# pairlab/SlotFormer

Measured on AMD Instinct MI355X. Metric: rollout frames/sec at B=32, 128x128, 7 slots, 6+50 steps (SAVi-encode + SlotFormer rollout), higher is better.
Workload: dtype f32 storage; matmul/conv on split-bf16 MFMA (bf16x3: hi*hi+hi*lo+lo*hi, f32 accumulate)

## Files before the change

include/slotformer_hip.h:

```cpp
#ifndef SLOTFORMER_HIP_H
#define SLOTFORMER_HIP_H
#include <stddef.h>

#ifdef __cplusplus
extern "C" {
#endif

int sf_version(void);
const char* sf_last_error_string(void);

int sf_get_precision(void);
int sf_set_precision(int mode);

int sf_profile_enable(int class_mask);
int sf_set_seam_fused(int on);
int sf_get_seam_fused(void);
int sf_set_ffn_rows64(int on);
int sf_get_ffn_rows64(void);
int sf_profile_sample(int every);
int sf_profile_read(int kernel_class, double* total_ms, long long* launches, double* work);


int sf_linear_f32(const float* A, int lda, const float* W, const float* bias, const float* ln_gamma,
                  const float* ln_beta, float ln_eps, const float* residual, int ldr, float* C, int ldc,
// ... 137 lines not shown
int sf_slot_update_packed_f32(const float* part_num, const float* part_den, int P, const float* slots_prev,
                              const void* gru_ih_packed, const void* gru_hh_packed, const float* gru_b_ih,
                              const float* gru_b_hh, const float* ln_g, const float* ln_b, const void* mlp_w1_packed,
                              const float* mlp_b1, const void* mlp_w2_packed, const float* mlp_b2, float* slots_out,
                              const float* q_ln_g, const float* q_ln_b, const void* q_w_packed, float* q_out, int B, int N,
                              int D, int H, float ln_eps, void* stream);
int sf_slot_update_packed_next_f32(const float* part_num, const float* part_den, int P, const float* slots_prev,
                                   const void* gru_ih_packed, const void* gru_hh_packed, const float* gru_b_ih,
                                   const float* gru_b_hh, const float* ln_g, const float* ln_b, const void* mlp_w1_packed,
                                   const float* mlp_b1, const void* mlp_w2_packed, const float* mlp_b2, float* slots_out,
                                   const float* q_ln_g, const float* q_ln_b, const void* q_w_packed, float* q_out, int B, int N,
                                   int D, int H, float ln_eps, float* out2, long long out2_bs, int p_step, const float* pm_ln_g,
                                   const float* pm_ln_b, const void* pm_w0_packed, const float* pm_b0, const void* pm_w2_packed,
                                   const float* pm_b2, int norm_first, const void* kd_w_packed, const float* kd_b, const float* noise,
                                   long long noise_bs, float* kdist_out, long long kdist_bs, float* next_slots, void* stream);

int sf_mha_f32(const float* qkv, float* out, int B, int L, int Lq, int d_model, int num_heads, void* stream);

int sf_qkv_attention_f32(const float* x, const float* ln_gamma, const float* ln_beta, float ln_eps,
                         const float* in_proj_w, const float* in_proj_b, float* out, int B, int L, int Lq, int d_model,
                         int num_heads, void* stream);

int sf_lstm_pointwise_f32(const float* gates, const float* c_prev, float* h_out, float* c_out, int R, int H,
                          void* stream);

int sf_sample_dist_f32(const float* dist, const float* noise, float* out, int R, int D, void* stream);

int sf_bilinear_resize_f32(const float* in, float* out, long long R, int Hi, int Wi, int Ho, int Wo,
                           void* stream);

size_t sf_groupnorm1_workspace_bytes(int F);
int sf_groupnorm1_nhwc_f32(const float* x, const float* gamma, const float* beta, float* y, int F, int H, int W, int C,
                           float eps, int relu, int pixel_shuffle, void* ws, size_t ws_bytes, void* stream);
size_t sf_groupnorm1_bwd_workspace_bytes(int F, int H, int W, int C);
int sf_groupnorm1_nhwc_bwd_f32(const float* x, const float* gamma, const float* beta, const float* dy, float* dx, float* dgamma,
                               float* dbeta, int F, int H, int W, int C, float eps, int relu, int pixel_shuffle, void* ws,
                               size_t ws_bytes, void* stream);

int sf_slate_attention_f32(const float* q, const float* k, const float* v, float* out, int ldq, int ldk, int ldv, int ldo,
                           int B, int Lq, int Lk, int num_heads, int head_dim, int causal, void* stream);
size_t sf_slate_attention_bwd_workspace_bytes(int B, int Lq, int num_heads);
int sf_slate_attention_train_fwd_f32(const float* q, const float* k, const float* v, float* out, float* lse, int ldq, int ldk,
                                     int ldv, int ldo, long long q_bs, long long k_bs, long long v_bs, long long o_bs, int B,
                                     int Lq, int Lk, int num_heads, int head_dim, int causal, float dropout_p,
                                     unsigned long long seed, void* stream);
int sf_slate_attention_train_bwd_f32(const float* q, const float* k, const float* v, const float* out, const float* d_out,
                                     const float* lse, float* dq, float* dk, float* dv, int ldq, int ldk, int ldv, int ldo,
                                     long long q_bs, long long k_bs, long long v_bs, long long o_bs, int B, int Lq, int Lk,
                                     int num_heads, int head_dim, int causal, float dropout_p, unsigned long long seed, void* ws,
                                     size_t ws_bytes, void* stream);
int sf_slate_attention_bwd_f32(const float* q, const float* k, const float* v, const float* out, const float* d_out, float* dq,
                               float* dk, float* dv, int ldq, int ldk, int ldv, int ldo, long long q_bs, long long k_bs,
                               long long v_bs, long long o_bs, int B, int Lq, int Lk, int num_heads, int head_dim, int causal,
                               void* ws, size_t ws_bytes, void* stream);
int sf_slate_attention_strided_f32(const float* q, const float* k, const float* v, float* out, int ldq, int ldk, int ldv,
                                   int ldo, long long q_bs, long long k_bs, long long v_bs, long long o_bs, int B, int Lq,
                                   int Lk, int num_heads, int head_dim, int causal, void* stream);
int sf_embed_tokens_f32(const long long* idx, const float* tok_emb, const float* pos, float* out, int B, int L, int d,
                        void* stream);
int sf_argmax_rows_f32(const float* x, long long ld, long long* out, long long R, int V, void* stream);
int sf_cross_entropy_f32(const float* x, const long long* target, float* loss_rows, float* mean_out, long long R, int V,
                         void* stream);
int sf_softmax_rows_f32(const float* x, const float* add, float scale, float* y, long long R, int V, void* stream);
int sf_cross_entropy_bwd_f32(const float* x, const long long* target, const float* g, float* dx, long long R, int V, void* stream);
int sf_log_softmax_rows_f32(const float* x, float* y, long long R, int V, void* stream);
int sf_gumbel_softmax_rows_f32(const float* x, unsigned long long seed, float scale, float* y, long long R, int V, void* stream);
int sf_softmax_rows_bwd_f32(const float* y, const float* dy, float scale, float* dx, long long R, int V, void* stream);

typedef struct {
  const float *ln1_g, *ln1_b, *wqkv, *wo;
  const float *ln2_g, *ln2_b, *wq_c, *wkv_c, *wo_c;
  const float *ln3_g, *ln3_b, *w1, *b1, *w2, *b2;
  int is_first;
} sf_slate_block;

typedef struct {
  int d_model, num_heads, num_layers, vocab_size, num_slots, max_len;
  const float *in_proj_w, *in_proj_b, *tok_emb , *pos_emb , *lnf_g, *lnf_b, *head_w ;
  const sf_slate_block* blocks;
} sf_slate_decoder;

size_t sf_slate_generate_workspace_bytes(const sf_slate_decoder* m, int B, int steps);
int sf_slate_generate_f32(const sf_slate_decoder* m, const float* slots, int B, int steps, long long* tokens_out,
                          float* logits_out, void* ws, size_t ws_bytes, void* stream);

int sf_slate_step_ok(const sf_slate_decoder* m);
size_t sf_slate_generate_tok_workspace_bytes(const sf_slate_decoder* m, int B, int steps);
int sf_slate_generate_tok_f32(const sf_slate_decoder* m, const float* slots, int B, int steps, long long* tokens_out,
                              float* logits_out, int frames_per_wg, void* ws, size_t ws_bytes, void* stream,
                              int* frames_per_wg_ran);
int sf_gather_rows_f32(const float* table, const long long* ids, float* out, long long R, int d, long long table_rows,
                       void* stream);

int sf_dvae_tokens_ok(int V, int K, int C, int H, int W);
size_t sf_dvae_head_packed_bytes(int V, int K);
int sf_dvae_pack_head_weights(const float* w, void* packed, int V, int K, void* stream);
int sf_dvae_pack_head_weights_host(const float* w, void* packed, int V, int K);
int sf_dvae_patch_embed_f32(const float* img, const float* w, float* y, int F, int C, int H, int W, void* stream);
int sf_dvae_head_argmax_f32(const float* x, long long ld, const void* w_packed, const float* bias, long long* ids_i64, short* ids_i16, long long R,
                            int V, int K, void* stream);

int sf_head_ce_ok(int V, int K);
size_t sf_head_ce_packed_bytes(int V, int K);
size_t sf_head_ce_workspace_bytes(long long R);
int sf_head_ce_pack_weights(const float* w, void* packed, int V, int K, void* stream);
int sf_head_ce_pack_weights_host(const float* w, void* packed, int V, int K);
int sf_head_ce_fwd_f32(const float* x, long long ld, const void* w_packed, const long long* target_i64, const short* target_i16,
                       const float* group_w, int group, float* lse, float* loss_rows, double* stats, long long R, int V, int K, void* ws,
                       size_t ws_bytes, void* stream);
int sf_head_ce_bwd_f32(const float* x, long long ld, const void* w_packed, const long long* target_i64, const short* target_i16,
                       const float* group_w, int group, const float* lse, const float* g, float* dx, long long ldx, long long R, int V, int K,
                       void* stream);

int sf_physion_readout_ok(int N, int C, int F);
int sf_physion_readout_fwd_f32(const float* slots, long long stride_v, long long stride_t, int V, const int* video_index, const float* W1,
                               const float* b1, const float* w2, const float* b2, float* logits, int* t_star, float* step_logits,
                               unsigned char* pair_star, int K, int B, int T, int N, int C, int F, int agg, void* stream);
size_t sf_physion_readout_bwd_workspace_bytes(int B, int N, int F);
int sf_physion_readout_bwd_f32(const float* slots, long long stride_v, long long stride_t, int V, const int* video_index, const float* W1,
                               const float* b1, const float* w2, const float* g, const int* t_star, const unsigned char* pair_star, float* dW1,
                               float* db1, float* dw2, float* db2, int B, int T, int N, int C, int F, int agg, void* workspace,
                               size_t workspace_bytes, void* stream);
int sf_physion_readout_score_f32(const float* logits, const float* labels, const int* task_idx, const float* thresholds, int n_thresh, int n_tasks,
                                 float* loss, float* g, int* counts, int* task_counts, int K, int B, void* stream);


typedef struct {
  const float *norm1_g, *norm1_b, *in_proj_w, *in_proj_b, *out_proj_w, *out_proj_b;
  const float *norm2_g, *norm2_b, *lin1_w, *lin1_b, *lin2_w, *lin2_b;
  const void *lin1_packed, *lin2_packed;
  const void *attn_in_packed, *attn_out_packed;
  const void* tok_packed;
} sf_tfm_layer;

size_t sf_attn_packed_bytes(int d_model, int which);
int sf_pack_attn_weights(const float* in_proj_w, const float* out_proj_w, void* in_packed, void* out_packed, int d_model,
                         int num_heads, void* stream);

size_t sf_ffn_packed_bytes(int d_model, int ffn);
int sf_pack_ffn_weights(const float* lin1_w, const float* lin2_w, void* lin1_packed, void* lin2_packed, int d_model,
                        int ffn, void* stream);

int sf_ffn_chunk_partials_f32(const sf_tfm_layer* w, const float* ap, long long ap_stride, float* xp, long long xp_stride, int M,
                              int ffn, int rows_per_wg, void* stream);

int sf_attn_block_f32(const sf_tfm_layer* w, const float* x, float* out, int B, int L, int Lq, int heads_per_wg, void* stream);
int sf_ffn_block_rows_f32(const sf_tfm_layer* w, const float* x2, float* y, int M, int ffn, void* stream);
size_t sf_layer_tok_packed_bytes(void);
size_t sf_layer_tok_packed_bytes_ex(int d_model, int num_heads, int ffn);
int sf_pack_layer_tok_weights(const sf_tfm_layer* w, void* packed, int d_model, int num_heads, int ffn, void* stream);
int sf_layer_tok_block_f32(const sf_tfm_layer* w, int nl, const float* x, float* y, int B, int L, void* stream);
int sf_layer_tok_block_ex_f32(const sf_tfm_layer* w, int nl, int d_model, int num_heads, int ffn, const float* x, float* y, int B, int L, void* stream);
int sf_debug_read_ts_layer_tok(long long* out16);
size_t sf_attn_rows_planes_bytes(int B);
int sf_attn_block_rows_f32(const sf_tfm_layer* w, const float* x, float* out, void* planes, int B, int L, int Lq, void* stream);

int sf_phyre_readout_ok(int num_slots, int slot_size, int T, int d_model, int num_heads, int ffn, int num_layers);
size_t sf_phyre_readout_workspace_bytes(int B, int num_slots, int T);
int sf_phyre_readout_fwd_f32(const float* slots, long long stride_v, long long stride_t, int V, int T_all, const int* video_index, const int* sel,
                             const float* in_proj_w, const float* in_proj_b, const float* enc_t_pe, const float* cls, const sf_tfm_layer* layers,
                             int num_layers, int d_model, int num_heads, int ffn, const float* mlp_w1, const float* mlp_b1, const float* mlp_w2,
                             const float* mlp_b2, float* logits, float* conf, const int* scatter_index, float* scatter_table, long long scatter_len,
                             int B, int T, int N, int C, void* workspace, size_t workspace_bytes, void* stream);
int sf_phyre_auccess_f32(const float* conf, const int* status, int* first_rank, int tasks, int actions, void* stream);

typedef struct {
  int num_slots, slot_size, T, text_len;
  int question_len;
  int d_model, num_heads, ffn_dim, num_layers;
  int vocab, emb_dim;
  const float* cls;
  const float* pos;
  const float *vision_w, *vision_b;
  const float* q_in_proj_w;
  const float* text_table;
  const sf_tfm_layer* layers;
} sf_aloe;
int sf_aloe_ok(int num_slots, int slot_size, int T, int text_len, int d_model, int num_heads, int ffn, int num_layers);
size_t sf_aloe_workspace_bytes(int B, int num_slots, int T, int text_len, int d_model, int ffn);
int sf_aloe_text_table_f32(const float* q_embedding, const float* q_in_proj_w, const float* q_in_proj_b, float* table, int vocab, int emb_dim, int d_model,
                           void* stream);
int sf_aloe_fwd_f32(const sf_aloe* m, const float* slots, long long stride_v, long long stride_t, int V, int T_all, const int* video_index, const int* start,
                    int frame_offset, const int* tokens, const unsigned char* pad_mask, int multiple_choice, const float* head_w1, const float* head_b1,
                    const float* head_w2, const float* head_b2, int mlp_hidden, int num_outputs, float* logits, int* answers, int B, void* workspace,
                    size_t workspace_bytes, void* stream);
int sf_aloe_score_f32(const float* cls_logits, const int* cls_labels, int B1, int num_answers, const float* mc_logits, const float* mc_labels,
                      const int* mc_flag, int Bn, const int* mc_subtype, int Q, float* losses, int* ques_correct, int* counts, void* stream);

typedef struct {
  int num_slots, slot_size, d_model, num_layers, num_heads, ffn_dim, norm_first;
  int window_len;
  int single_step;
  const float *in_proj_w, *in_proj_b, *out_proj_w, *out_proj_b;
  const float* pe_tok;
  const sf_tfm_layer* layers;
  const void *in_proj_packed, *out_proj_packed;
} sf_rollouter;

size_t sf_packed_linear_bytes(int N, int K);
int sf_pack_linear_weights(const float* w, void* packed, int N, int K, void* stream);

size_t sf_rollout_workspace_bytes(const sf_rollouter* m, int B);
int sf_rollout_f32(const sf_rollouter* m, float* slots, int B, int T_total, int pred_len, void* ws,
                   size_t ws_bytes, void* stream);

typedef struct {
  int precision;
  int seam_fused;
  int ffn_rows;
  int attn_heads_per_wg;
  int attn_qkv_rows;
  int ffn_tile;
  int cus_available;
  int layer_tok;
} sf_rollout_opts;
int sf_set_layer_tok(int on);
int sf_get_layer_tok(void);
int sf_rollout_opts_f32(const sf_rollouter* m, float* slots, int B, int T_total, int pred_len, void* ws, size_t ws_bytes,
                        void* stream, const sf_rollout_opts* opts);
size_t sf_rollout_phases_workspace_bytes(const sf_rollouter* m, int B, int frame_offset);
int sf_rollout_phases_f32(const sf_rollouter* m, float* slots, int B, int T_total, int obs, int frame_offset, int pred_len, void* ws,
                          size_t ws_bytes, void* stream, const sf_rollout_opts* opts);
int sf_rollout_is_fused(const sf_rollouter* m);
int sf_rollout_tok_ok(const sf_rollouter* m);
int sf_rollout_tok_layers(const sf_rollouter* m, int B, const sf_rollout_opts* opts);
int sf_rollout_uses_seam(const sf_rollouter* m, int B);
int sf_rollout_uses_seam_opts(const sf_rollouter* m, int B, const sf_rollout_opts* opts);

size_t sf_linear_bwd_workspace_bytes(long long M, int N, int K);
int sf_linear_bwd_f32(const float* x, const float* W, const float* y, float* dy, float* dx, float* dW, float* db, long long M,
                      int N, int K, int relu, void* ws, size_t ws_bytes, void* stream);
int sf_mha_train_fwd_f32(const float* qkv, float* ctx, int B, int L, int d_model, int num_heads, float dropout_p,
                         unsigned long long seed, void* stream);
int sf_mha_train_bwd_f32(const float* qkv, const float* d_ctx, float* d_qkv, int B, int L, int d_model, int num_heads,
                         float dropout_p, unsigned long long seed, void* stream);
int sf_dropout_f32(const float* x, const float* res, float* y, long long n, float dropout_p, unsigned long long seed,
                   void* stream);
int sf_adam_flat_f32(float* param, const float* grad, float* exp_avg, float* exp_avg_sq, long long n, int step, float lr,
                     float beta1, float beta2, float eps, void* stream);
size_t sf_grad_norm_workspace_bytes(long long n);
int sf_grad_clip_coef_f32(const float* grad, long long n, float max_norm, float* out3, void* ws, size_t ws_bytes,
                          void* stream);
#define SF_ADAM_MAX_GROUPS 8
typedef struct {
  long long begin;
  float lr;
} sf_adam_group;
int sf_adam_flat_groups_f32(float* param, const float* grad, float* exp_avg, float* exp_avg_sq, long long n, int step,
                            const sf_adam_group* groups, int num_groups, float beta1, float beta2, float eps,
                            const float* grad_scale, void* stream);
size_t sf_layernorm_bwd_workspace_bytes(int D);
int sf_layernorm_bwd_f32(const float* x, const float* dy, const float* gamma, float* dx, float* dgamma, float* dbeta,
                         long long rows, int D, float eps, void* ws, size_t ws_bytes, void* stream);

typedef struct {
  int resolution, layers, channels, ks, hidden, out_channels;
  const float* conv_w[8];
  const float* conv_b[8];
  const float *pos_grid, *pos_w, *pos_b;
  const float *ln_g, *ln_b, *fc1_w, *fc1_b, *fc2_w, *fc2_b;
} sf_savi_features;

typedef struct {
  float* conv_w[8];
  float* conv_b[8];
  float *pos_w, *pos_b, *ln_g, *ln_b, *fc1_w, *fc1_b, *fc2_w, *fc2_b;
} sf_savi_features_grads;

size_t sf_savi_features_train_workspace_bytes(const sf_savi_features* m, int F);
int sf_savi_features_train_fwd_f32(const sf_savi_features* m, const float* img, long long frame_stride, int F, float* out,
                                   void* ws, size_t ws_bytes, void* stream);
int sf_savi_features_train_bwd_f32(const sf_savi_features* m, const float* img, long long frame_stride, const float* d_out,
                                   const sf_savi_features_grads* g, int F, void* ws, size_t ws_bytes, void* stream);

typedef struct {
  int in_features, slot_size, mlp_hidden, num_slots;
  const float *norm_in_g, *norm_in_b, *wk, *wv;
  const float *q_ln_g, *q_ln_b, *wq;
  const float *gru_w_ih, *gru_w_hh, *gru_b_ih, *gru_b_hh;
  const float *mlp_ln_g, *mlp_ln_b, *mlp_w1, *mlp_b1, *mlp_w2, *mlp_b2;
  float eps;
} sf_slot_attention;

typedef struct {
  float *norm_in_g, *norm_in_b, *wk, *wv, *q_ln_g, *q_ln_b, *wq, *gru_w_ih, *gru_w_hh, *gru_b_ih, *gru_b_hh;
  float *mlp_ln_g, *mlp_ln_b, *mlp_w1, *mlp_b1, *mlp_w2, *mlp_b2;
} sf_slot_attention_grads;

size_t sf_slot_attention_train_workspace_bytes(const sf_slot_attention* m, int B, int HW, int iters);
int sf_slot_attention_train_fwd_f32(const sf_slot_attention* m, const float* inputs, const float* slots_in, int B, int HW,
                                    int iters, float* slots_out, void* ws, size_t ws_bytes, void* stream);
int sf_slot_attention_train_bwd_f32(const sf_slot_attention* m, const float* inputs, const float* d_slots_out, float* d_inputs,
                                    float* d_slots_in, const sf_slot_attention_grads* g, int B, int HW, int iters, void* ws,
                                    size_t ws_bytes, void* stream);

typedef struct {
  float *norm1_g, *norm1_b, *in_proj_w, *in_proj_b, *out_proj_w, *out_proj_b;
  float *norm2_g, *norm2_b, *lin1_w, *lin1_b, *lin2_w, *lin2_b;
} sf_tfm_layer_grads;

typedef struct {
  float *in_proj_w, *in_proj_b, *out_proj_w, *out_proj_b;
  const sf_tfm_layer_grads* layers;
  float* pe_tok;
} sf_rollouter_grads;

size_t sf_rollout_train_workspace_bytes(const sf_rollouter* m, int B, int pred_len);
int sf_rollout_train_fwd_f32(const sf_rollouter* m, const float* x, float* pred, int B, int pred_len, float dropout_p,
                             unsigned long long seed, void* ws, size_t ws_bytes, void* stream);
int sf_rollout_train_bwd_f32(const sf_rollouter* m, const float* d_pred, float* d_x, const sf_rollouter_grads* g, int B,
                             int pred_len, float dropout_p, unsigned long long seed, void* ws, size_t ws_bytes,
                             void* stream);

typedef struct {
  int num_slots, slot_size, d_model, num_heads, ffn_dim, num_layers;
  const float *in_proj_w, *in_proj_b;
  const float *enc_t_pe, *cls;
  const sf_tfm_layer* layers;
  const float *mlp_w1, *mlp_b1, *mlp_w2, *mlp_b2;
} sf_phyre_readout_model;

typedef struct {
  float *in_proj_w, *in_proj_b;
  float *enc_t_pe, *cls;
  const sf_tfm_layer_grads* layers;
  float *mlp_w1, *mlp_b1, *mlp_w2, *mlp_b2;
} sf_phyre_readout_grads;

size_t sf_phyre_readout_train_workspace_bytes(const sf_phyre_readout_model* m, int B, int T);
int sf_phyre_readout_train_fwd_f32(const sf_phyre_readout_model* m, const float* slots, long long stride_v, long long stride_t, int V, int T_all,
                                   const int* video_index, const int* sel, int B, int T, float dropout_p, unsigned long long seed, float* logits,
                                   unsigned char* gates, unsigned char* head_gates, void* ws, size_t ws_bytes, void* stream);
int sf_phyre_readout_train_bwd_f32(const sf_phyre_readout_model* m, const float* slots, long long stride_v, long long stride_t, int V, int T_all,
                                   const int* video_index, const int* sel, int B, int T, const float* g, const sf_phyre_readout_grads* grads,
                                   float dropout_p, unsigned long long seed, void* ws, size_t ws_bytes, void* stream);

int sf_rollout_train_clips_fwd_f32(const sf_rollouter* m, const float* table, int T_total, const int* clip_video, const int* clip_start,
                                   int frame_offset, float* pred, int B, int pred_len, float dropout_p, unsigned long long seed, void* ws,
                                   size_t ws_bytes, void* stream);
size_t sf_clip_mse_workspace_bytes(int B, int S, long long E);
int sf_clip_mse_f32(const float* pred, const float* target, const int* clip_video, const int* clip_start, int T_total, int first_frame,
                    int frame_step, const float* step_w, const int* clip_len, int hist, float scale, float* d_pred, double* stats, int B, int S,
                    long long E, void* ws, size_t ws_bytes, void* stream);
int sf_clip_frames_f32(const unsigned char* table, int T_total, const int* clip_video, const int* clip_start, int first_frame, int frame_step,
                       const float* mean3, const float* std3, float* out, int B, int S, int H, int W, void* stream);

typedef struct {
  int resolution;
  int enc_layers;
// ... 149 lines not shown
```

slotformer_amd/_lib.py:

```python
import ctypes as C
import os

_HERE = os.path.dirname(os.path.abspath(__file__))
LIB_PATH = os.environ.get('SF_LIB_PATH') or os.path.join(_HERE, 'libslotformer_hip.so')

FP = C.c_void_p


class sf_tfm_layer(C.Structure):
    _fields_ = [(n, FP) for n in (
        'norm1_g', 'norm1_b', 'in_proj_w', 'in_proj_b', 'out_proj_w', 'out_proj_b',
        'norm2_g', 'norm2_b', 'lin1_w', 'lin1_b', 'lin2_w', 'lin2_b', 'lin1_packed', 'lin2_packed', 'attn_in_packed', 'attn_out_packed', 'tok_packed')]


class sf_rollouter(C.Structure):
    _fields_ = [(n, C.c_int) for n in (
        'num_slots', 'slot_size', 'd_model', 'num_layers', 'num_heads', 'ffn_dim', 'norm_first',
        'window_len', 'single_step')] + [(n, FP) for n in (
            'in_proj_w', 'in_proj_b', 'out_proj_w', 'out_proj_b', 'pe_tok')] + [
                ('layers', C.POINTER(sf_tfm_layer)), ('in_proj_packed', C.c_void_p), ('out_proj_packed', C.c_void_p)]


class sf_aloe(C.Structure):
    _fields_ = [(n, C.c_int) for n in ('num_slots', 'slot_size', 'T', 'text_len', 'question_len', 'd_model', 'num_heads', 'ffn_dim', 'num_layers',
                                       'vocab', 'emb_dim')] + [(n, FP) for n in ('cls', 'pos', 'vision_w', 'vision_b', 'q_in_proj_w', 'text_table')] + [
                                           ('layers', C.POINTER(sf_tfm_layer))]


class sf_rollout_opts(C.Structure):
    _fields_ = [(n, C.c_int) for n in ('precision', 'seam_fused', 'ffn_rows', 'attn_heads_per_wg', 'attn_qkv_rows', 'ffn_tile', 'cus_available', 'layer_tok')]


class sf_tfm_layer_grads(C.Structure):
    _fields_ = [(n, FP) for n in (
        'norm1_g', 'norm1_b', 'in_proj_w', 'in_proj_b', 'out_proj_w', 'out_proj_b',
        'norm2_g', 'norm2_b', 'lin1_w', 'lin1_b', 'lin2_w', 'lin2_b')]


class sf_phyre_readout_model(C.Structure):
    _fields_ = [(n, C.c_int) for n in ('num_slots', 'slot_size', 'd_model', 'num_heads', 'ffn_dim', 'num_layers')] + [
        (n, FP) for n in ('in_proj_w', 'in_proj_b', 'enc_t_pe', 'cls')] + [('layers', C.POINTER(sf_tfm_layer))] + [
            (n, FP) for n in ('mlp_w1', 'mlp_b1', 'mlp_w2', 'mlp_b2')]


class sf_phyre_readout_grads(C.Structure):
    _fields_ = [(n, FP) for n in ('in_proj_w', 'in_proj_b', 'enc_t_pe', 'cls')] + [('layers', C.POINTER(sf_tfm_layer_grads))] + [
        (n, FP) for n in ('mlp_w1', 'mlp_b1', 'mlp_w2', 'mlp_b2')]


class sf_rollouter_grads(C.Structure):
    _fields_ = [(n, FP) for n in ('in_proj_w', 'in_proj_b', 'out_proj_w', 'out_proj_b')] + [
        ('layers', C.POINTER(sf_tfm_layer_grads)), ('pe_tok', FP)]


_SA_LEAVES = ('norm_in_g', 'norm_in_b', 'wk', 'wv', 'q_ln_g', 'q_ln_b', 'wq', 'gru_w_ih', 'gru_w_hh', 'gru_b_ih', 'gru_b_hh',
              'mlp_ln_g', 'mlp_ln_b', 'mlp_w1', 'mlp_b1', 'mlp_w2', 'mlp_b2')


class sf_slot_attention(C.Structure):
    _fields_ = [(n, C.c_int) for n in ('in_features', 'slot_size', 'mlp_hidden', 'num_slots')] + [
        (n, FP) for n in _SA_LEAVES] + [('eps', C.c_float)]


class sf_slot_attention_grads(C.Structure):
    _fields_ = [(n, FP) for n in _SA_LEAVES]


class sf_adam_group(C.Structure):
    _fields_ = [('begin', C.c_longlong), ('lr', C.c_float)]


class sf_savi_decoder_grads(C.Structure):
    _fields_ = [('deconv_w', FP * 8), ('deconv_b', FP * 8)] + [(n, FP) for n in ('out_w', 'out_b', 'pos_w', 'pos_b')]


class sf_savi_features(C.Structure):
    _fields_ = [(n, C.c_int) for n in ('resolution', 'layers', 'channels', 'ks', 'hidden', 'out_channels')] + [
        ('conv_w', FP * 8), ('conv_b', FP * 8)] + [(n, FP) for n in ('pos_grid', 'pos_w', 'pos_b', 'ln_g', 'ln_b', 'fc1_w', 'fc1_b',
                                                                      'fc2_w', 'fc2_b')]


class sf_savi_features_grads(C.Structure):
    _fields_ = [('conv_w', FP * 8), ('conv_b', FP * 8)] + [(n, FP) for n in ('pos_w', 'pos_b', 'ln_g', 'ln_b', 'fc1_w', 'fc1_b',
                                                                              'fc2_w', 'fc2_b')]


class sf_savi_encoder(C.Structure):
    _fields_ = (
        [('resolution', C.c_int), ('enc_layers', C.c_int), ('enc_channels', C.c_int * 9),
         ('enc_ks', C.c_int)] +
        [(n, C.c_int) for n in ('enc_out_channels', 'num_slots', 'slot_size', 'slot_mlp_size',
                                'num_iterations')] +
        [('conv_w', FP * 8), ('conv_b', FP * 8), ('pos_table', FP)] +
        [(n, FP) for n in ('enc_ln_g', 'enc_ln_b', 'enc_fc1_w', 'enc_fc1_b', 'enc_fc2_w', 'enc_fc2_b',
                           'sa_norm_in_g', 'sa_norm_in_b', 'sa_q_ln_g', 'sa_q_ln_b', 'sa_q_w', 'sa_kv_w',
                           'gru_w_ih', 'gru_w_hh', 'gru_b_ih', 'gru_b_hh',
                           'mlp_ln_g', 'mlp_ln_b', 'mlp_w1', 'mlp_b1', 'mlp_w2', 'mlp_b2',
                           'init_latents')] +
        [('kd_mode', C.c_int)] +
        [(n, FP) for n in ('kd_w0', 'kd_b0', 'kd_ln_g', 'kd_ln_b', 'kd_w3', 'kd_b3')] +
        [(n, C.c_int) for n in ('pred_type', 'pred_rnn', 'pred_norm_first', 'pred_num_layers',
                                'pred_num_heads', 'pred_ffn_dim', 'pred_hidden')] +
        [(n, FP) for n in ('pm_ln_g', 'pm_ln_b', 'pm_w0', 'pm_b0', 'pm_w2', 'pm_b2')] +
        [('pred_layers', C.POINTER(sf_tfm_layer))] +
        [(n, FP) for n in ('lstm_w_ih', 'lstm_w_hh', 'lstm_b_ih', 'lstm_b_hh', 'proj_w', 'proj_b')] +
        [('sa_eps', C.c_float), ('sa_q_w_t', FP), ('pm_w0_t', FP), ('pm_w2_t', FP), ('kd_w0_t', FP),
         ('sa_gru_ih_p', C.c_void_p), ('sa_gru_hh_p', C.c_void_p), ('sa_mlp_w1_p', C.c_void_p), ('sa_mlp_w2_p', C.c_void_p),
         ('sa_q_w_p', C.c_void_p), ('sa_fold_q_w', FP), ('sa_fold_q_w_t', FP), ('sa_fold_gru_ih_t', FP), ('sa_fold_q_w_p', C.c_void_p),
         ('sa_fold_gru_ih_p', C.c_void_p), ('pred_packed', C.POINTER(C.c_void_p)), ('enc_fc1_p', C.c_void_p), ('enc_fc2_p', C.c_void_p),
         ('conv_w_frag', C.c_void_p * 8), ('pm_w0_p', C.c_void_p), ('pm_w2_p', C.c_void_p), ('kd_w0_p', C.c_void_p)])


class sf_slate_block(C.Structure):
    _fields_ = [(n, FP) for n in ('ln1_g', 'ln1_b', 'wqkv', 'wo', 'ln2_g', 'ln2_b', 'wq_c', 'wkv_c', 'wo_c', 'ln3_g', 'ln3_b',
                                  'w1', 'b1', 'w2', 'b2')] + [('is_first', C.c_int)]


class sf_slate_decoder(C.Structure):
    _fields_ = [(n, C.c_int) for n in ('d_model', 'num_heads', 'num_layers', 'vocab_size', 'num_slots', 'max_len')] + [
        (n, FP) for n in ('in_proj_w', 'in_proj_b', 'tok_emb', 'pos_emb', 'lnf_g', 'lnf_b', 'head_w')] + [
            ('blocks', C.POINTER(sf_slate_block))]


class sf_savi_decoder(C.Structure):
    _fields_ = ([('resolution', C.c_int), ('dec_layers', C.c_int), ('dec_channels', C.c_int * 9),
                 ('dec_strides', C.c_int * 8), ('dec_ks', C.c_int), ('dec_res', C.c_int), ('num_slots', C.c_int),
                 ('slot_size', C.c_int), ('deconv_w', FP * 8), ('deconv_b', FP * 8), ('out_w', FP), ('out_b', FP),
                 ('pos_table', FP), ('deconv_w_flipped', FP * 8), ('deconv_w_frag', C.c_void_p * 8), ('l0_weff', FP), ('l0_posterm', FP)])


class sf_egress_tile(C.Structure):
    _fields_ = [('kind', C.c_int), ('N', C.c_int), ('a', C.c_void_p), ('b', C.c_void_p), ('scale', C.c_float), ('ids_i64', C.c_int), ('P', C.c_int),
                ('history_len', C.c_int)]


class sf_lpips_model(C.Structure):
    _fields_ = [('conv_w', C.c_void_p * 13), ('conv_b', FP * 13), ('lin_w', FP * 5), ('shift', FP), ('scale', FP)]


I, LL, F32, SZ, VP = C.c_int, C.c_longlong, C.c_float, C.c_size_t, C.c_void_p

SIGNATURES = {
    'sf_version': (I, []),
    'sf_last_error_string': (C.c_char_p, []),
    'sf_get_precision': (I, []),
    'sf_set_precision': (I, [I]),
    'sf_profile_enable': (I, [I]),
    'sf_profile_sample': (I, [I]),
    'sf_set_seam_fused': (I, [I]),
    'sf_get_seam_fused': (I, []),
    'sf_set_ffn_rows64': (I, [I]),
    'sf_get_ffn_rows64': (I, []),
    'sf_profile_read': (I, [I, C.POINTER(C.c_double), C.POINTER(C.c_longlong), C.POINTER(C.c_double)]),
    'sf_linear_f32': (I, [FP, I, FP, FP, FP, FP, F32, FP, I, FP, I, I, I, I, I, VP]),
    'sf_layernorm_f32': (I, [FP, FP, FP, FP, I, I, F32, VP]),
    'sf_conv2d_nchw_in_f32': (I, [FP, LL, FP, FP, FP, FP, I, I, I, I, I, I, I, I, VP]),
    'sf_conv2d_nchw_in_grouped_f32': (I, [FP, LL, I, LL, FP, FP, FP, FP, I, I, I, I, I, I, I, I, VP]),
    'sf_conv2d_nhwc_f32': (I, [FP, FP, FP, FP, FP, I, I, I, I, I, I, I, VP]),
    'sf_pack_conv_weight_f32': (I, [FP, FP, I, I, I, VP]),
    'sf_pixel_feat_f32': (I, [FP] * 10 + [I, F32, I, VP]),
    'sf_conv_frag_bytes': (SZ, [I, I, I]),
    'sf_set_conv_fp16x2': (I, [I]),
    'sf_get_conv_fp16x2': (I, []),
    'sf_pack_conv_frag_weights': (I, [FP, VP, I, I, I, VP]),
    'sf_conv5x5_frag_f32': (I, [FP, VP, FP, FP, FP, I, I, I, I, VP]),
    'sf_conv5x5_ws_f32': (I, [FP, VP, FP, FP, FP, I, I, I, I, I, VP]),
    'sf_deconv_frag_bytes': (SZ, [I, I, I, I]),
    'sf_pack_deconv_frag_weights': (I, [FP, VP, I, I, I, I, VP]),
    'sf_deconv5x5s2_frag_f32': (I, [FP, VP, FP, FP, I, I, I, I, VP]),
    'sf_deconv5x5s2_head_frag_f32': (I, [FP, VP, FP, FP, FP, FP, I, I, I, VP]),
    'sf_decode_l0_expand_f32': (I, [FP, FP, FP, I, I, I, VP]),
    'sf_conv_transpose2d_nhwc_f32': (I, [FP, FP, FP, FP, I, I, I, I, I, I, I, I, VP]),
    'sf_pack_deconv_weight_f32': (I, [FP, FP, I, I, I, VP]),
    'sf_slot_broadcast_f32': (I, [FP, FP, FP, I, I, I, VP]),
    'sf_decode_combine_f32': (I, [FP, FP, FP, FP, I, I, I, VP]),
    'sf_savi_decode_workspace_bytes': (SZ, [C.POINTER(sf_savi_decoder), I]),
    'sf_savi_decode_f32': (I, [C.POINTER(sf_savi_decoder), FP, FP, FP, FP, I, VP, SZ, VP]),
    'sf_savi_decode_seg_f32': (I, [C.POINTER(sf_savi_decoder), FP, FP, FP, FP, VP, VP, F32, I, VP, SZ, VP]),
    'sf_decode_combine_seg_f32': (I, [FP, FP, FP, FP, VP, VP, F32, VP, I, I, I, VP]),
    'sf_postproc_mask_f32': (I, [FP, VP, VP, F32, VP, I, I, I, VP]),
    'sf_vp_metrics_workspace_bytes': (SZ, [I, I, I]),
    'sf_vp_image_metrics_f32': (I, [FP, FP, VP, VP, VP, I, I, I, I, VP, SZ, VP]),
    'sf_vp_mask_metrics': (I, [VP, VP, I, VP, FP, VP, VP, VP, VP, I, I, I, I, VP, SZ, VP]),
    'sf_vp_bbox_pr_f32': (I, [FP, VP, FP, VP, VP, I, I, I, F32, VP]),
    'sf_masks_to_boxes': (I, [VP, I, FP, VP, I, I, I, I, VP]),
    'sf_vp_mean_over_videos_f64': (I, [VP, VP, I, I, I, VP]),
    'sf_lpips_pack_conv_weights': (I, [FP, VP, I, I, VP]),
    'sf_lpips_pack_conv_weights_host': (I, [VP, VP, I, I]),
    'sf_lpips_workspace_bytes': (SZ, [I, I, I]),
    'sf_lpips_f32': (I, [C.POINTER(sf_lpips_model), FP, FP, FP, I, I, I, I, I, VP, SZ, VP]),
    'sf_lpips_mean_over_videos_f32': (I, [FP, VP, VP, I, I, VP]),
    'sf_ingest_tables_bytes': (SZ, [I, I, I, I, I]),
    'sf_ingest_tables_host': (I, [VP, SZ, I, I, I, I, I]),
    'sf_ingest_frames_u8': (I, [VP, VP, I, VP, FP, FP, FP, I, I, I, I, I, I, I, VP]),
    'sf_resize_masks_nearest': (I, [VP, I, VP, VP, VP, I, I, I, I, I, VP]),
    'sf_rle_label_maps': (I, [VP, VP, VP, VP, VP, VP, VP, I, I, I, I, I, I, I, VP]),
    'sf_rle_boxes_pad': (I, [VP, FP, VP, VP, I, I, VP]),
    'sf_egress_frames_u8': (I, [FP, VP, LL, I, I, I, I, I, VP]),
    'sf_egress_grid_shape': (I, [I, I, I, I, I, I, C.POINTER(I), C.POINTER(I)]),
    'sf_egress_grid': (I, [C.POINTER(sf_egress_tile), I, VP, I, I, I, I, I, I, F32, I, VP]),
    'sf_egress_draw_boxes': (I, [VP, FP, VP, VP, I, I, I, I, I, I, VP]),
    'sf_pos_embed_table_f32': (I, [FP, FP, FP, FP, I, I, VP]),
    'sf_slot_attn_num_partials': (I, [I]),
    'sf_slot_attn_iter_f32': (I, [FP, FP, I, LL, FP, FP, FP, FP, I, I, I, I, F32, F32, VP]),
    'sf_slot_update_f32': (I, [FP, FP, I, FP] + [FP] * 10 + [FP, I, I, I, I, F32, VP]),
    'sf_slot_update_packed_f32': (I, [FP, FP, I, FP, VP, VP, FP, FP, FP, FP, VP, FP, VP, FP, FP, FP, FP, VP, FP, I, I, I, I, F32, VP]),
    'sf_slot_attn_iter_planes_f32': (I, [VP, LL, FP, FP, FP, FP, LL, I, I, I, F32, F32, VP]),
    'sf_slot_prologue_f32': (I, [FP] * 8 + [I, FP, FP, FP, LL, FP, LL, FP, FP, FP, FP, FP, I, I, I, F32, VP]),
    'sf_slot_update_packed_next_f32': (I, [FP, FP, I, FP, VP, VP, FP, FP, FP, FP, VP, FP, VP, FP, FP, FP, FP, VP, FP, I, I, I, I, F32,
                                           FP, LL, I, FP, FP, VP, FP, VP, FP, I, VP, FP, FP, LL, FP, LL, FP, VP]),
    'sf_mha_f32': (I, [FP, FP, I, I, I, I, I, VP]),
    'sf_qkv_attention_f32': (I, [FP, FP, FP, F32, FP, FP, FP, I, I, I, I, I, VP]),
    'sf_lstm_pointwise_f32': (I, [FP, FP, FP, FP, I, I, VP]),
    'sf_sample_dist_f32': (I, [FP, FP, FP, I, I, VP]),
    'sf_bilinear_resize_f32': (I, [FP, FP, LL, I, I, I, I, VP]),
    'sf_rollout_workspace_bytes': (SZ, [C.POINTER(sf_rollouter), I]),
    'sf_rollout_f32': (I, [C.POINTER(sf_rollouter), FP, I, I, I, VP, SZ, VP]),
    'sf_rollout_opts_f32': (I, [C.POINTER(sf_rollouter), FP, I, I, I, VP, SZ, VP, C.POINTER(sf_rollout_opts)]),
    'sf_rollout_phases_workspace_bytes': (SZ, [C.POINTER(sf_rollouter), I, I]),
    'sf_rollout_phases_f32': (I, [C.POINTER(sf_rollouter), FP, I, I, I, I, I, VP, SZ, VP, C.POINTER(sf_rollout_opts)]),
    'sf_rollout_uses_seam': (I, [C.POINTER(sf_rollouter), I]),
    'sf_rollout_uses_seam_opts': (I, [C.POINTER(sf_rollouter), I, C.POINTER(sf_rollout_opts)]),
    'sf_rollout_is_fused': (I, [C.POINTER(sf_rollouter)]),
    'sf_rollout_tok_ok': (I, [C.POINTER(sf_rollouter)]),
    'sf_rollout_tok_layers': (I, [C.POINTER(sf_rollouter), I, C.POINTER(sf_rollout_opts)]),
    'sf_ffn_chunk_partials_f32': (I, [C.POINTER(sf_tfm_layer), FP, LL, FP, LL, I, I, I, VP]),
    'sf_attn_block_f32': (I, [C.POINTER(sf_tfm_layer), FP, FP, I, I, I, I, VP]),
    'sf_ffn_block_rows_f32': (I, [C.POINTER(sf_tfm_layer), FP, FP, I, I, VP]),
    'sf_set_layer_tok': (I, [I]),
    'sf_get_layer_tok': (I, []),
    'sf_layer_tok_packed_bytes': (SZ, []),
    'sf_layer_tok_packed_bytes_ex': (SZ, [I, I, I]),
    'sf_pack_layer_tok_weights': (I, [C.POINTER(sf_tfm_layer), VP, I, I, I, VP]),
    'sf_layer_tok_block_f32': (I, [C.POINTER(sf_tfm_layer), I, FP, FP, I, I, VP]),
    'sf_layer_tok_block_ex_f32': (I, [C.POINTER(sf_tfm_layer), I, I, I, I, FP, FP, I, I, VP]),
    'sf_debug_read_ts_layer_tok': (I, [C.POINTER(C.c_longlong)]),
    'sf_attn_rows_planes_bytes': (SZ, [I]),
    'sf_attn_block_rows_f32': (I, [C.POINTER(sf_tfm_layer), FP, FP, VP, I, I, I, VP]),
    'sf_slot_attn_iter_bwd_workspace_bytes': (SZ, [I, I, I, I]),
    'sf_slot_attn_iter_bwd_f32': (I, [FP, FP, I, LL, FP, FP, FP, I, FP, FP, FP, I, FP, I, I, I, I, F32, F32, VP, SZ, VP]),
    'sf_slot_attn_iter_bwd16_workspace_bytes': (SZ, [I, I, I, I]),
    'sf_slot_attn_iter_bwd16_f32': (I, [FP, FP, I, LL, FP, FP, FP, I, FP, FP, FP, I, FP, I, I, I, I, F32, F32, VP, SZ, VP]),
    'sf_set_slot_attn_tile16': (I, [I]),
    'sf_get_slot_attn_tile16': (I, []),
    'sf_slot_attention_train_workspace_bytes': (SZ, [C.POINTER(sf_slot_attention), I, I, I]),
    'sf_slot_attention_train_fwd_f32': (I, [C.POINTER(sf_slot_attention), FP, FP, I, I, I, FP, VP, SZ, VP]),
    'sf_slot_attention_train_bwd_f32': (I, [C.POINTER(sf_slot_attention), FP, FP, FP, FP, C.POINTER(sf_slot_attention_grads), I, I, I,
                                            VP, SZ, VP]),
    'sf_savi_decode_train_workspace_bytes': (SZ, [C.POINTER(sf_savi_decoder), I]),
    'sf_savi_decode_train_fwd_f32': (I, [C.POINTER(sf_savi_decoder), FP, FP, FP, FP, I, VP, SZ, VP]),
    'sf_savi_decode_train_bwd_f32': (I, [C.POINTER(sf_savi_decoder), C.POINTER(C.c_void_p), FP, FP, FP, C.POINTER(sf_savi_decoder_grads),
                                         I, VP, SZ, VP]),
    'sf_savi_features_train_workspace_bytes': (SZ, [C.POINTER(sf_savi_features), I]),
    'sf_savi_features_train_fwd_f32': (I, [C.POINTER(sf_savi_features), FP, LL, I, FP, VP, SZ, VP]),
    'sf_savi_features_train_bwd_f32': (I, [C.POINTER(sf_savi_features), FP, LL, FP, C.POINTER(sf_savi_features_grads), I, VP, SZ, VP]),
    'sf_linear_bwd_workspace_bytes': (SZ, [LL, I, I]),
    'sf_linear_bwd_f32': (I, [FP, FP, FP, FP, FP, FP, FP, LL, I, I, I, VP, SZ, VP]),
    'sf_mha_train_fwd_f32': (I, [FP, FP, I, I, I, I, F32, C.c_ulonglong, VP]),
    'sf_mha_train_bwd_f32': (I, [FP, FP, FP, I, I, I, I, F32, C.c_ulonglong, VP]),
    'sf_dropout_f32': (I, [FP, FP, FP, LL, F32, C.c_ulonglong, VP]),
    'sf_adam_flat_f32': (I, [FP, FP, FP, FP, LL, I, F32, F32, F32, F32, VP]),
    'sf_grad_norm_workspace_bytes': (SZ, [LL]),
    'sf_grad_clip_coef_f32': (I, [FP, LL, F32, FP, VP, SZ, VP]),
    'sf_adam_flat_groups_f32': (I, [FP, FP, FP, FP, LL, I, C.POINTER(sf_adam_group), I, F32, F32, F32, FP, VP]),
    'sf_layernorm_bwd_workspace_bytes': (SZ, [I]),
    'sf_layernorm_bwd_f32': (I, [FP, FP, FP, FP, FP, FP, LL, I, F32, VP, SZ, VP]),
    'sf_rollout_train_workspace_bytes': (SZ, [C.POINTER(sf_rollouter), I, I]),
    'sf_rollout_train_fwd_f32': (I, [C.POINTER(sf_rollouter), FP, FP, I, I, F32, C.c_ulonglong, VP, SZ, VP]),
    'sf_rollout_train_bwd_f32': (I, [C.POINTER(sf_rollouter), FP, FP, C.POINTER(sf_rollouter_grads), I, I, F32,
                                     C.c_ulonglong, VP, SZ, VP]),
    'sf_rollout_train_clips_fwd_f32': (I, [C.POINTER(sf_rollouter), FP, I, VP, VP, I, FP, I, I, F32, C.c_ulonglong, VP, SZ, VP]),
    'sf_clip_mse_workspace_bytes': (SZ, [I, I, LL]),
    'sf_clip_mse_f32': (I, [FP, FP, VP, VP, I, I, I, FP, VP, I, F32, FP, VP, I, I, LL, VP, SZ, VP]),
    'sf_clip_frames_f32': (I, [VP, I, VP, VP, I, I, FP, FP, FP, I, I, I, I, VP]),
    'sf_savi_encode_workspace_bytes': (SZ, [C.POINTER(sf_savi_encoder), I]),
    'sf_savi_encode_f32': (I, [C.POINTER(sf_savi_encoder), FP, FP, FP, FP, FP, I, FP, FP, FP, I, I, VP, SZ,
                               VP]),
    'sf_groupnorm1_workspace_bytes': (SZ, [I]),
    'sf_groupnorm1_nhwc_f32': (I, [FP, FP, FP, FP, I, I, I, I, F32, I, I, VP, SZ, VP]),
    'sf_groupnorm1_bwd_workspace_bytes': (SZ, [I, I, I, I]),
    'sf_groupnorm1_nhwc_bwd_f32': (I, [FP, FP, FP, FP, FP, FP, FP, I, I, I, I, F32, I, I, VP, SZ, VP]),
    'sf_slate_attention_f32': (I, [FP, FP, FP, FP, I, I, I, I, I, I, I, I, I, I, VP]),
    'sf_slate_attention_strided_f32': (I, [FP, FP, FP, FP, I, I, I, I, LL, LL, LL, LL, I, I, I, I, I, I, VP]),
    'sf_slate_attention_bwd_workspace_bytes': (SZ, [I, I, I]),
    'sf_slate_attention_bwd_f32': (I, [FP, FP, FP, FP, FP, FP, FP, FP, I, I, I, I, LL, LL, LL, LL, I, I, I, I, I, I, VP, SZ, VP]),
    'sf_slate_attention_train_fwd_f32': (I, [FP, FP, FP, FP, FP, I, I, I, I, LL, LL, LL, LL, I, I, I, I, I, I, F32, C.c_ulonglong, VP]),
    'sf_slate_attention_train_bwd_f32': (I, [FP, FP, FP, FP, FP, FP, FP, FP, FP, I, I, I, I, LL, LL, LL, LL, I, I, I, I, I, I, F32,
                                             C.c_ulonglong, VP, SZ, VP]),
    'sf_embed_tokens_f32': (I, [VP, FP, FP, FP, I, I, I, VP]),
    'sf_argmax_rows_f32': (I, [FP, LL, VP, LL, I, VP]),
    'sf_cross_entropy_f32': (I, [FP, VP, FP, FP, LL, I, VP]),
    'sf_softmax_rows_f32': (I, [FP, FP, F32, FP, LL, I, VP]),
    'sf_softmax_rows_bwd_f32': (I, [FP, FP, F32, FP, LL, I, VP]),
    'sf_log_softmax_rows_f32': (I, [FP, FP, LL, I, VP]),
    'sf_cross_entropy_bwd_f32': (I, [FP, VP, FP, FP, LL, I, VP]),
    'sf_gumbel_softmax_rows_f32': (I, [FP, C.c_ulonglong, F32, FP, LL, I, VP]),
    'sf_slate_generate_workspace_bytes': (SZ, [C.POINTER(sf_slate_decoder), I, I]),
    'sf_slate_generate_f32': (I, [C.POINTER(sf_slate_decoder), FP, I, I, VP, FP, VP, SZ, VP]),
    'sf_slate_step_ok': (I, [C.POINTER(sf_slate_decoder)]),
    'sf_slate_generate_tok_workspace_bytes': (SZ, [C.POINTER(sf_slate_decoder), I, I]),
    'sf_slate_generate_tok_f32': (I, [C.POINTER(sf_slate_decoder), FP, I, I, VP, FP, I, VP, SZ, VP, C.POINTER(I)]),
    'sf_gather_rows_f32': (I, [FP, VP, FP, LL, I, LL, VP]),
    'sf_dvae_tokens_ok': (I, [I, I, I, I, I]),
    'sf_dvae_head_packed_bytes': (SZ, [I, I]),
    'sf_dvae_pack_head_weights': (I, [FP, VP, I, I, VP]),
    'sf_dvae_pack_head_weights_host': (I, [VP, VP, I, I]),
    'sf_dvae_patch_embed_f32': (I, [FP, FP, FP, I, I, I, I, VP]),
    'sf_dvae_head_argmax_f32': (I, [FP, LL, VP, FP, VP, VP, LL, I, I, VP]),
    'sf_head_ce_ok': (I, [I, I]),
    'sf_head_ce_packed_bytes': (SZ, [I, I]),
    'sf_head_ce_workspace_bytes': (SZ, [LL]),
    'sf_head_ce_pack_weights': (I, [FP, VP, I, I, VP]),
    'sf_head_ce_pack_weights_host': (I, [VP, VP, I, I]),
    'sf_head_ce_fwd_f32': (I, [FP, LL, VP, VP, VP, FP, I, FP, FP, VP, LL, I, I, VP, SZ, VP]),
    'sf_head_ce_bwd_f32': (I, [FP, LL, VP, VP, VP, FP, I, FP, FP, FP, LL, LL, I, I, VP]),
    'sf_physion_readout_ok': (I, [I, I, I]),
    'sf_physion_readout_fwd_f32': (I, [FP, LL, LL, I, VP, FP, FP, FP, FP, FP, VP, FP, VP, I, I, I, I, I, I, I, VP]),
    'sf_physion_readout_bwd_workspace_bytes': (SZ, [I, I, I]),
    'sf_physion_readout_bwd_f32': (I, [FP, LL, LL, I, VP, FP, FP, FP, FP, VP, VP, FP, FP, FP, FP, I, I, I, I, I, I, VP, SZ, VP]),
    'sf_physion_readout_score_f32': (I, [FP, FP, VP, C.POINTER(F32), I, I, FP, FP, VP, VP, I, I, VP]),
    'sf_phyre_readout_ok': (I, [I, I, I, I, I, I, I]),
    'sf_phyre_readout_workspace_bytes': (SZ, [I, I, I]),
    'sf_phyre_readout_fwd_f32': (I, [FP, LL, LL, I, I, VP, C.POINTER(C.c_int), FP, FP, FP, FP, C.POINTER(sf_tfm_layer), I, I, I, I, FP, FP, FP, FP, FP,
                                     FP, VP, FP, LL, I, I, I, I, VP, SZ, VP]),
    'sf_phyre_auccess_f32': (I, [FP, VP, VP, I, I, VP]),
    'sf_phyre_readout_train_workspace_bytes': (SZ, [C.POINTER(sf_phyre_readout_model), I, I]),
    'sf_phyre_readout_train_fwd_f32': (I, [C.POINTER(sf_phyre_readout_model), FP, LL, LL, I, I, VP, C.POINTER(C.c_int), I, I, F32, C.c_ulonglong, FP,
                                           VP, VP, VP, SZ, VP]),
    'sf_phyre_readout_train_bwd_f32': (I, [C.POINTER(sf_phyre_readout_model), FP, LL, LL, I, I, VP, C.POINTER(C.c_int), I, I, FP,
                                           C.POINTER(sf_phyre_readout_grads), F32, C.c_ulonglong, VP, SZ, VP]),
    'sf_aloe_ok': (I, [I, I, I, I, I, I, I, I]),
    'sf_aloe_workspace_bytes': (SZ, [I, I, I, I, I, I]),
    'sf_aloe_text_table_f32': (I, [FP, FP, FP, FP, I, I, I, VP]),
    'sf_aloe_fwd_f32': (I, [C.POINTER(sf_aloe), FP, LL, LL, I, I, VP, VP, I, VP, VP, I, FP, FP, FP, FP, I, I, FP, VP, I, VP, SZ, VP]),
    'sf_aloe_score_f32': (I, [FP, VP, I, I, FP, FP, VP, I, VP, I, FP, VP, VP, VP]),
    'sf_packed_linear_bytes': (SZ, [I, I]),
    'sf_pack_linear_weights': (I, [FP, VP, I, I, VP]),
    'sf_attn_packed_bytes': (SZ, [I, I]),
    'sf_pack_attn_weights': (I, [FP, FP, VP, VP, I, I, VP]),
    'sf_ffn_packed_bytes': (SZ, [I, I]),
    'sf_pack_ffn_weights': (I, [FP, FP, VP, VP, I, I, VP]),
    'sf_savi_cnn_workspace_bytes': (SZ, [C.POINTER(sf_savi_encoder), I]),
    'sf_savi_cnn_f32': (I, [C.POINTER(sf_savi_encoder), FP, I, I, I, I, FP, VP, SZ, VP]),
    'sf_savi_encode_pre_f32': (I, [C.POINTER(sf_savi_encoder), FP, FP, I, FP, FP, FP, FP, I, FP, FP, FP, I, I, VP, SZ,
                                   VP]),
    'sf_savi_encode_fork_workspace_bytes': (SZ, [C.POINTER(sf_savi_encoder), I, I]),
    'sf_savi_encode_batched_workspace_bytes': (SZ, [C.POINTER(sf_savi_encoder), I, I]),
    'sf_set_encode_fuse_next': (I, [I]),
    'sf_get_encode_fuse_next': (I, []),
    'sf_set_slot_chain': (I, [I]),
    'sf_get_slot_chain': (I, []),
    'sf_set_slot_attn_planes': (I, [I]),
    'sf_get_slot_attn_planes': (I, []),
    'sf_set_pixel_tok': (I, [I]),
    'sf_get_pixel_tok': (I, []),
    'sf_savi_chain_ok': (I, [C.POINTER(sf_savi_encoder), I, I]),
    'sf_savi_planes_bytes': (SZ, [C.POINTER(sf_savi_encoder), I, I]),
    'sf_savi_features_workspace_bytes': (SZ, [C.POINTER(sf_savi_encoder), I, I]),
    'sf_savi_features_planes_f32': (I, [C.POINTER(sf_savi_encoder), FP, I, I, VP, VP, SZ, VP]),
    'sf_savi_slots_chain_workspace_bytes': (SZ, [C.POINTER(sf_savi_encoder), I]),
    'sf_savi_slots_chain_f32': (I, [C.POINTER(sf_savi_encoder), VP, FP, FP, FP, LL, FP, FP, I, I, I, VP, SZ, VP]),
    'sf_savi_encode_fork_f32': (I, [C.POINTER(sf_savi_encoder), FP, FP, I, FP, FP, FP, FP, I, FP, FP, FP, I, I, VP, SZ,
                                    VP, VP]),
    'sf_kv_producer_workspace_bytes': (SZ, [I, I]),
    'sf_kv_producer_f32': (I, [FP] * 11 + [I, I, I, I, F32, VP, SZ, VP]),
    'sf_device_alloc': (I, [C.POINTER(VP), SZ]),
    'sf_device_free': (I, [VP]),
    'sf_device_upload': (I, [VP, VP, SZ]),
    'sf_device_download': (I, [VP, VP, SZ]),
    'sf_device_synchronize': (I, []),
    'sf_stream_create_cu_mask': (I, [C.POINTER(VP), C.POINTER(C.c_uint), I]),
    'sf_stream_cus': (I, [VP]),
    'sf_stream_set_cus': (I, [VP, I]),
    'sf_debug_spin': (I, [I, VP]),
    'sf_debug_clock_probe': (I, [I, VP, VP]),
    'sf_stream_destroy': (I, [VP]),
    'sf_slot_attn_iter_f32_host': (I, [FP, FP, I, LL, FP, FP, FP, FP, I, I, I, I, F32, F32, VP]),
    'sf_rollout_f32_host': (I, [C.POINTER(sf_rollouter), FP, I, I, I, VP, SZ, VP]),
    'sf_savi_encode_f32_host': (I, [C.POINTER(sf_savi_encoder), FP, FP, FP, FP, FP, I, FP, FP, FP, I, I, VP, SZ,
                                    VP]),
    'sf_savi_decode_f32_host': (I, [C.POINTER(sf_savi_decoder), FP, FP, FP, FP, I, VP, SZ, VP]),
    'sf_seam_timeouts': (I, []),
    'sf_slot_attn_iter_bf16': (I, [VP, VP, I, LL, FP, FP, FP, FP, I, I, I, I, F32, F32, VP]),
    'sf_rollout_bf16': (I, [C.POINTER(sf_rollouter), FP, I, I, I, VP, SZ, VP]),
    'sf_rollout_bf16_host': (I, [C.POINTER(sf_rollouter), FP, I, I, I, VP, SZ, VP]),
    'sf_slot_update_f32_host': (I, [FP, FP, I, FP] + [FP] * 10 + [FP, I, I, I, I, F32, VP]),
    'sf_kv_producer_f32_host': (I, [FP] * 11 + [I, I, I, I, F32, VP, SZ, VP]),
}

_lib = None

# ... 96 lines not shown
```

slotformer_amd/csrc/attn_rows.hip:

```cpp
#include "../../include/slotformer_hip.h"
#include "sf_internal.h"
#include "layer_fused.h"
#include "qkv_heads.h"
#include <stdlib.h>

namespace {
constexpr int NT = 512;
constexpr int D = 256, HD = 32, NH = 8;
constexpr int AP = D + 8;
constexpr int TRMAX = 128;
constexpr int KC = 64, NK = D / KC;
constexpr int PL = 2048;
constexpr size_t K1_PLANES = (size_t)2 * TRMAX * AP * 2;
constexpr size_t K1_LDS = K1_PLANES + 2 * D * 4;
constexpr size_t K2_LDS = (size_t)2 * 64 * AP * 2;
static_assert(K1_LDS <= 160 * 1024 && K2_LDS <= 160 * 1024, "LDS budget");

struct RowsArgs {
  const float* xin;
  long long x_batch_stride, xparts_stride;
  const float* pe;
  int f0, ring_frames, nslots;
  const float *ln_g, *ln_b;
  float ln_eps;
// ... 352 lines not shown
  f32x4 s[2][4], xr[2][4], bv[4];
#pragma unroll
  for (int g = 0; g < 4; ++g) bv[g] = *(const f32x4*)(A.bo + wave * 32 + 8 * g + 4 * (lane >> 5));
#pragma unroll
  for (int rbk = 0; rbk < 2; ++rbk) {
    if (rbk >= nrb || rbk * 32 + 32 <= nq0) continue;
    const int row = rbk * 32 + (lane & 31);
    const float* o = A.x2 + ((long long)b * Lq + (min(max(row, nq0), L - 1) - nq0)) * D + wave * 32 + 4 * (lane >> 5);
#pragma unroll
    for (int g = 0; g < 4; ++g) xr[rbk][g] = *(const f32x4*)(o + 8 * g);
  }
#pragma unroll
  for (int half = 0; half < 2; ++half) {
#pragma unroll
    for (int rbk = 0; rbk < 2; ++rbk) {
      if (rbk >= nrb || rbk * 32 + 32 <= nq0) continue;
      const int row = rbk * 32 + (lane & 31);
      const int ao = row * AP + 8 * (lane >> 5);
#pragma unroll
      for (int hh = 0; hh < 2; ++hh) {
        const int hp = 2 * half + hh;
        f32x16 pacc;
#pragma unroll
        for (int r = 0; r < 16; ++r) pacc[r] = 0.f;
#pragma unroll
        for (int ks = 0; ks < 4; ++ks) {
          const bf16x8 xh = *(const bf16x8*)(Oh + ao + hp * 64 + ks * 16), xl = *(const bf16x8*)(Ol + ao + hp * 64 + ks * 16);
          pacc = __builtin_amdgcn_mfma_f32_32x32x16_bf16(wof[hp][ks][0], xl, pacc, 0, 0, 0);
          pacc = __builtin_amdgcn_mfma_f32_32x32x16_bf16(wof[hp][ks][1], xh, pacc, 0, 0, 0);
          pacc = __builtin_amdgcn_mfma_f32_32x32x16_bf16(wof[hp][ks][0], xh, pacc, 0, 0, 0);
        }
        const bool mine = (wave >> 1) == hp;
#pragma unroll
        for (int g = 0; g < 4; ++g) {
          const f32x4 p = {pacc[4 * g], pacc[4 * g + 1], pacc[4 * g + 2], pacc[4 * g + 3]};
          const f32x4 pm = p + (xr[rbk][g] + bv[g]);
          f32x4 v;
#pragma unroll
          for (int q = 0; q < 4; ++q) v[q] = mine ? pm[q] : p[q];
          s[rbk][g] = hp == 0 ? v : s[rbk][g] + v;
        }
      }
    }
  }
#pragma unroll
  for (int rbk = 0; rbk < 2; ++rbk) {
    if (rbk >= nrb || rbk * 32 + 32 <= nq0) continue;
    const int row = rbk * 32 + (lane & 31);
    if (row >= nq0 && row < L) {
      float* o = A.x2 + ((long long)b * Lq + (row - nq0)) * D + wave * 32 + 4 * (lane >> 5);
#pragma unroll
      for (int g = 0; g < 4; ++g) *(f32x4*)(o + 8 * g) = s[rbk][g];
    }
  }
  if ((A.dbg & 16) && b == 0 && t == 0) ar_ts[10] = wall_clock64();
}

size_t sf_attn_rows_plane_bytes(int B) { return (size_t)B * NH * 6 * PL * 2; }

static int ar_dbg() {
  static const int v = sf_dbg("lf");
  return v;
}

static int launch_core(const sf_tfm_layer& w, float* x2, void* planes, int B, int L, int Lq, hipStream_t st) {
  CoreArgs C;
  C.planes = (const __bf16*)planes; C.wo_p = (const uint4*)w.attn_out_packed; C.bo = w.out_proj_b; C.x2 = x2; C.L = L; C.Lq = Lq;
  C.dbg = ar_dbg();
  SF_TRY(sf_ensure_dyn_lds((const void*)attn_core_kernel, K2_LDS));
  hipLaunchKernelGGL(attn_core_kernel, dim3(B), dim3(NT), K2_LDS, st, C);
  SF_CHECK_LAUNCH();
  return 0;
}

int sf_attn_rows_ex(int mode, const float* xin, long long x_batch_stride, long long xparts_stride, const float* pe, int f0,
                    int ring_frames, int nslots, const sf_tfm_layer& w, float eps, float* x2, void* planes, int B, int L, int Lq,
                    hipStream_t st) {
  if (!w.attn_in_packed || !w.attn_out_packed)
    return sf_set_err(-1, "invalid argument: fused attention needs packed weights (sf_pack_attn_weights)", __FILE__, __LINE__);
  if (!planes || L < 1 || L > 64 || Lq < 1 || Lq > L || (long long)B * L >= (1 << 22))
    return sf_set_err(-1, "invalid argument: row-tile attention needs planes, 1 <= Lq <= L <= 64 and B * L < 2^22", __FILE__, __LINE__);
  RowsArgs A;
  A.xin = xin; A.x_batch_stride = x_batch_stride; A.xparts_stride = xparts_stride; A.pe = pe; A.f0 = f0;
  A.ring_frames = ring_frames; A.nslots = nslots; A.ln_g = w.norm1_g; A.ln_b = w.norm1_b; A.ln_eps = eps;
  A.wqkv_p = (const uint4*)w.attn_in_packed; A.bias = w.in_proj_b; A.planes = (__bf16*)planes; A.x2 = x2;
  A.B = B; A.L = L; A.Lq = Lq; A.dbg = ar_dbg();
  const int TRr = 64;
  A.nt = (B * L + TRr - 1) / TRr;
  const int ntq = (B * Lq + TRr - 1) / TRr;
  int extra = 0;
  if (Lq == L) {
    A.ng = 3;
  } else {
    A.ng = 2;
    extra = ntq;
  }
  A.main_blocks = A.nt;
  const int blocks = A.nt + extra;
  const size_t lds = (size_t)2 * TRr * AP * 2 + 2 * D * 4;
  sf_prof_begin(SF_K_MHA, st, 6.0 * B * L * (double)D * D + 4.0 * (double)B * NH * Lq * L * HD + 2.0 * B * Lq * (double)D * D);
#define SF_QKV_TRY(x)                 \
  do {                                \
    const int rc_ = (x);              \
    if (rc_) {                        \
      sf_prof_end(SF_K_MHA, st);      \
      return rc_;                     \
    }                                 \
  } while (0)
#define SF_QKV_LAUNCH(RING_, PART_)                                                                                         \
  do {                                                                                                                      \
    if (TRr == 128) {                                                                                                       \
      SF_QKV_TRY(sf_ensure_dyn_lds((const void*)qkv_rows_kernel<RING_, PART_, 128>, lds));                                  \
      hipLaunchKernelGGL((qkv_rows_kernel<RING_, PART_, 128>), dim3(blocks), dim3(NT), lds, st, A);                         \
    } else {                                                                                                                \
      SF_QKV_TRY(sf_ensure_dyn_lds((const void*)qkv_rows_kernel<RING_, PART_, 64>, lds));                                   \
      hipLaunchKernelGGL((qkv_rows_kernel<RING_, PART_, 64>), dim3(blocks), dim3(NT), lds, st, A);                          \
    }                                                                                                                       \
  } while (0)
  if (mode == 2)
    SF_QKV_LAUNCH(true, false);
  else if (mode == 1)
    SF_QKV_LAUNCH(false, true);
  else
    SF_QKV_LAUNCH(false, false);
#undef SF_QKV_LAUNCH
#undef SF_QKV_TRY
  SF_CHECK_LAUNCH();
  const int rc = launch_core(w, x2, planes, B, L, Lq, st);
  sf_prof_end(SF_K_MHA, st);
  return rc;
}

int sf_attn_core_ex(const sf_tfm_layer& w, float* x2, void* planes, int B, int L, int Lq, hipStream_t st) {
  if (!w.attn_out_packed || !planes || !x2 || L < 1 || L > 64 || Lq < 1 || Lq > L)
    return sf_set_err(-1, "invalid argument: attention core needs packed out-projection weights, planes and 1 <= Lq <= L <= 64", __FILE__, __LINE__);
  sf_prof_begin(SF_K_MHA, st, 4.0 * (double)B * NH * Lq * L * HD + 2.0 * B * Lq * (double)D * D);
  const int rc = launch_core(w, x2, planes, B, L, Lq, st);
  sf_prof_end(SF_K_MHA, st);
  return rc;
}

extern "C" size_t sf_attn_rows_planes_bytes(int B) { return B > 0 ? sf_attn_rows_plane_bytes(B) : 0; }

extern "C" int sf_attn_block_rows_f32(const sf_tfm_layer* w, const float* x, float* out, void* planes, int B, int L, int Lq, void* stream) {
  SF_REQUIRE(w && x && out && planes && B > 0, "sf_attn_block_rows_f32: null pointer / empty problem");
  SF_REQUIRE(L >= 1 && L <= 64 && Lq >= 1 && Lq <= L, "sf_attn_block_rows_f32: needs 1 <= Lq <= L <= 64");
  SF_REQUIRE(w->norm1_g && w->norm1_b && w->in_proj_b && w->out_proj_b && w->attn_in_packed && w->attn_out_packed,
             "sf_attn_block_rows_f32: null weight (packed attention weights needed)");
  hipError_t e = hipMemsetAsync(planes, 0, sf_attn_rows_plane_bytes(B), (hipStream_t)stream);
  if (e != hipSuccess) return sf_set_err((int)e, hipGetErrorString(e), __FILE__, __LINE__);
  return sf_attn_rows_ex(0, x, (long long)L * D, 0, nullptr, 0, 1, 1, *w, 1e-5f, out, planes, B, L, Lq, (hipStream_t)stream);
}

extern "C" int sf_debug_read_ts_rows(long long* out32) {
  hipError_t e = hipMemcpyFromSymbol(out32, HIP_SYMBOL(ar_ts), sizeof(long long) * 32);
  return e == hipSuccess ? 0 : (int)e;
}
```

slotformer_amd/csrc/engine.hip:

```cpp
#include "../../include/slotformer_hip.h"
#include "sf_internal.h"
#include <map>
#include <vector>
#include "layer_fused.h"
#include "slot_chain.h"
#include <stdlib.h>

namespace {

inline size_t pad256(size_t nfloat) { return ((nfloat * sizeof(float)) + 255) & ~(size_t)255; }

struct Bump {
  char* p;
  size_t left;
  bool ok = true;
  size_t used = 0;
  float* take(size_t nfloat) {
    const size_t bytes = pad256(nfloat);
    if (bytes > left) {
      ok = false;
      return nullptr;
    }
    float* r = p ? (float*)(p + used) : nullptr;
    used += bytes;
    left -= bytes;
    return r;
  }
};

inline bool plain_gemms(const SfThreadOpts& o) { return o.precision == 2 || o.precision == 3; }

struct TfmWs {
  float *x2, *qkv, *att, *hid, *y;
};

size_t tfm_ws_bytes(int M, int d, int ffn) {
  return pad256((size_t)M * d) * 3 + pad256((size_t)M * 3 * d) + pad256((size_t)M * ffn);
}

bool tfm_ws_take(Bump& bp, TfmWs& w, int M, int d, int ffn) {
  w.x2 = bp.take((size_t)M * d);
  w.qkv = bp.take((size_t)M * 3 * d);
  w.att = bp.take((size_t)M * d);
  w.hid = bp.take((size_t)M * ffn);
  w.y = bp.take((size_t)M * d);
  return bp.ok;
}

int tfm_layer(const sf_tfm_layer& w, float* x, TfmWs& ws, int B, int L, int Lq, int d, int heads, int ffn,
              int norm_first, hipStream_t st, float** out, float* xp = nullptr, int* counters = nullptr) {
  const int M = B * L, Mq = B * Lq;
  const float eps = 1e-5f;
  const SfRowMap rd = sf_rows(d);
  if (norm_first) {
    int fused = 1;
    if (sf_get_precision() >= 1 && !plain_gemms(sf_thread_opts()))
      fused = sf_qkv_attn_ex(x, w.norm1_g, w.norm1_b, eps, w.in_proj_w, w.in_proj_b, ws.att, B, L, Lq, d, heads, st);
    if (fused < 0 || fused > 1) return fused;
    if (fused == 1) {
      SF_TRY(sf_linear_ex(x, rd, w.in_proj_w, w.in_proj_b, w.norm1_g, w.norm1_b, eps, nullptr, rd, 0, ws.qkv,
                          sf_rows(3 * d), M, 3 * d, d, 0, st));
      SF_TRY(sf_mha_ex(ws.qkv, ws.att, B, L, Lq, d, heads, st));
    }
    const SfRowMap xr = (Lq == L) ? rd : sf_rows_batched(d, Lq, (long long)L * d, (long long)(L - Lq) * d);
    SF_TRY(sf_linear_ex(ws.att, rd, w.out_proj_w, w.out_proj_b, nullptr, nullptr, eps, x, xr, 0, ws.x2, rd, Mq,
                        d, d, 0, st));
    float* dst = (Lq == L) ? x : ws.y;
    if (xp && counters) {
      SF_TRY(sf_ffn_partial_ex(ws.x2, (long long)Mq * d, w, eps, xp, (long long)Mq * d, dst, counters, Mq, ffn, st, 1));
    } else {
      SF_TRY(sf_linear_ex(ws.x2, rd, w.lin1_w, w.lin1_b, w.norm2_g, w.norm2_b, eps, nullptr, rd, 0, ws.hid,
                          sf_rows(ffn), Mq, ffn, d, 1, st));
      SF_TRY(sf_linear_ex(ws.hid, sf_rows(ffn), w.lin2_w, w.lin2_b, nullptr, nullptr, eps, ws.x2, rd, 0, dst, rd,
                          Mq, d, ffn, 0, st));
    }
    *out = dst;
  } else {
    if (Lq != L) return sf_set_err(-1, "row pruning requires norm_first", __FILE__, __LINE__);
    int fused = 1;
    if (sf_get_precision() >= 1 && !plain_gemms(sf_thread_opts()))
      fused = sf_qkv_attn_ex(x, nullptr, nullptr, eps, w.in_proj_w, w.in_proj_b, ws.att, B, L, L, d, heads, st);
    if (fused < 0 || fused > 1) return fused;
    if (fused == 1) {
      SF_TRY(sf_linear_ex(x, rd, w.in_proj_w, w.in_proj_b, nullptr, nullptr, eps, nullptr, rd, 0, ws.qkv,
                          sf_rows(3 * d), M, 3 * d, d, 0, st));
      SF_TRY(sf_mha_ex(ws.qkv, ws.att, B, L, L, d, heads, st));
    }
    SF_TRY(sf_linear_ex(ws.att, rd, w.out_proj_w, w.out_proj_b, nullptr, nullptr, eps, x, rd, 0, ws.y, rd, M, d,
                        d, 0, st));
    SF_TRY(sf_layernorm_ex(ws.y, rd, w.norm1_g, w.norm1_b, ws.x2, rd, M, d, eps, st));
    SF_TRY(sf_linear_ex(ws.x2, rd, w.lin1_w, w.lin1_b, nullptr, nullptr, eps, nullptr, rd, 0, ws.hid,
                        sf_rows(ffn), M, ffn, d, 1, st));
    SF_TRY(sf_linear_ex(ws.hid, sf_rows(ffn), w.lin2_w, w.lin2_b, nullptr, nullptr, eps, ws.x2, rd, 0, ws.y, rd,
                        M, d, ffn, 0, st));
    SF_TRY(sf_layernorm_ex(ws.y, rd, w.norm2_g, w.norm2_b, x, rd, M, d, eps, st));
    *out = x;
  }
  return 0;
}

int check_layers(const sf_tfm_layer* l, int n) {
  if (n > 0 && !l) return -1;
  for (int i = 0; i < n; ++i) {
    const sf_tfm_layer& w = l[i];
    if (!w.norm1_g || !w.norm1_b || !w.in_proj_w || !w.in_proj_b || !w.out_proj_w || !w.out_proj_b ||
        !w.norm2_g || !w.norm2_b || !w.lin1_w || !w.lin1_b || !w.lin2_w || !w.lin2_b)
      return -1;
  }
  return 0;
}

void step_window(const sf_rollouter* m, int s, int& nf, int& f0) {
  nf = (m->single_step && s + 1 < m->window_len) ? s + 1 : m->window_len;
  f0 = m->single_step ? s + 1 - nf : s;
}

struct RolloutPlan {
  enum Path { GENERIC, LONG_WINDOW, FUSED_ROWS, FUSED_RING } path = GENERIC;
  int tok_layers = 0;
  enum Attn { HEAD_PAIRS, ALL_HEADS, ROW_TILES } attn = HEAD_PAIRS;
  enum Ffn { CHUNK_PARTS, TILE, TILE_QKV } ffn = CHUNK_PARTS;
  bool seam = false;
  bool fused() const { return path == FUSED_ROWS || path == FUSED_RING; }
};

RolloutPlan plan_rollout(const sf_rollouter* m, int B, const SfThreadOpts& o) {
  RolloutPlan p;
  if (!m || !m->layers) return p;
  const int N = m->num_slots, W = m->window_len, Lmax = W * N, nl = m->num_layers, d = m->d_model;
  bool packed = true, tok_packed = nl >= 2;
  for (int l = 0; l < nl; ++l) {
    const sf_tfm_layer& w = m->layers[l];
    packed = packed && w.lin1_packed && w.lin2_packed && w.attn_in_packed && w.attn_out_packed;
    if (l + 1 < nl) tok_packed = tok_packed && w.tok_packed;
  }
  const int precision = sf_precision(o);
  const bool fusable = packed && !plain_gemms(o) && precision >= 1 && m->norm_first;
  const bool tok_on = tok_packed && sf_layer_tok_on(o);
  if (fusable && sf_layer_fused_ok(d, m->num_heads, m->ffn_dim, Lmax)) {
    p.path = (m->in_proj_packed && m->out_proj_packed && sf_step_boundary_ok(d, m->slot_size)) ? RolloutPlan::FUSED_RING
                                                                                               : RolloutPlan::FUSED_ROWS;
    bool tok = tok_on;
    for (int nf = m->single_step ? 1 : W; nf <= W && tok; ++nf) tok = sf_layer_tok_ok(nf * N);
    p.tok_layers = tok ? nl - 1 : 0;
    p.attn = (o.attn_rows == 128 || tok) ? RolloutPlan::ROW_TILES : (o.attn_heads == 8 ? RolloutPlan::ALL_HEADS : RolloutPlan::HEAD_PAIRS);
    if (p.attn != RolloutPlan::HEAD_PAIRS && o.ffn_tile >= 1)
      p.ffn = (p.attn == RolloutPlan::ROW_TILES && o.ffn_tile == 2) ? RolloutPlan::TILE_QKV : RolloutPlan::TILE;
    const int cus = o.cus > 0 && o.cus < 160 ? o.cus : 160;
    p.seam = p.path == RolloutPlan::FUSED_RING && p.attn == RolloutPlan::HEAD_PAIRS &&
             sf_seam_on(o) && sf_seam_blocks(B, N) <= cus;
  } else if (fusable && sf_layer_fused_ok(d, m->num_heads, m->ffn_dim, 1) && Lmax > 64 && sf_ffn_tiles(B * Lmax) <= 1024) {
    p.path = RolloutPlan::LONG_WINDOW;
    if (tok_on && Lmax <= 96 && !m->single_step && sf_layer_tok_ok(Lmax)) p.tok_layers = nl - 1;
  } else if (tok_on && !plain_gemms(o) && precision >= 1 && m->norm_first && sf_layer_tok128_shape(d, m->num_heads, m->ffn_dim) && !m->single_step &&
             sf_layer_tok_ok(Lmax)) {
    p.tok_layers = nl - 1;
  }
  return p;
}

struct RolloutWs {
  float* x;
  TfmWs tw;
  float* apb;
  float* xpb;
  float *xa, *xb2;
  int* counters;
  unsigned* seam_flags;
  float* ring;
  float* planes;
};

bool rollout_ws_take(Bump& bp, RolloutWs& w, const sf_rollouter* m, int B) {
  const size_t M = (size_t)B * m->window_len * m->num_slots, d = m->d_model;
  w.x = bp.take(M * d);
  tfm_ws_take(bp, w.tw, (int)M, (int)d, m->ffn_dim);
  w.apb = bp.take(8 * M * d);
  w.xpb = bp.take(4 * M * d);
  w.xa = bp.take(M * d);
  w.xb2 = bp.take(M * d);
  w.counters = (int*)bp.take(1024);
  w.seam_flags = (unsigned*)bp.take(1024);
  w.ring = bp.take((size_t)B * (m->window_len + 1) * m->num_slots * d);
  w.planes = bp.take(sf_attn_rows_plane_bytes(B) / 4);
  return bp.ok;
}

}

extern "C" {

size_t sf_rollout_workspace_bytes(const sf_rollouter* m, int B) {
  if (!m || B <= 0) return 0;
  Bump bp{nullptr, ~(size_t)0};
  RolloutWs w;
  rollout_ws_take(bp, w, m, B);
  return bp.used;
}

__global__ void spin_kernel(long long ticks) {
  const long long t0 = wall_clock64();
  while (wall_clock64() - t0 < ticks) __builtin_amdgcn_s_sleep(16);
}
extern "C" int sf_debug_spin(int us, void* stream) {
  SF_REQUIRE(us > 0 && us <= 100000, "sf_debug_spin: 1..100000 microseconds");
  hipLaunchKernelGGL(spin_kernel, dim3(1), dim3(64), 0, (hipStream_t)stream, (long long)us * 100);
  SF_CHECK_LAUNCH();
  return 0;
}

__global__ void clock_probe_kernel(long long ticks, long long* out) {
  const long long w0 = wall_clock64(), c0 = __builtin_readcyclecounter();
  long long w1 = w0;
  while (w1 - w0 < ticks) {
    __builtin_amdgcn_s_sleep(8);
    w1 = wall_clock64();
  }
  const long long c1 = __builtin_readcyclecounter();
  if (threadIdx.x == 0) {
    out[0] = c1 - c0;
    out[1] = w1 - w0;
  }
}
extern "C" int sf_debug_clock_probe(int us, long long* out2, void* stream) {
  SF_REQUIRE(us > 0 && us <= 100000 && out2, "sf_debug_clock_probe: 1..100000 microseconds, a device buffer of two int64");
  hipLaunchKernelGGL(clock_probe_kernel, dim3(1), dim3(64), 0, (hipStream_t)stream, (long long)us * 100, out2);
  SF_CHECK_LAUNCH();
  return 0;
}

__global__ void zero_f32_kernel(float* a, float* b, long long n) {
  const long long i = 4 * ((long long)blockIdx.x * blockDim.x + threadIdx.x);
  if (i >= n) return;
  const bool vec = i + 4 <= n && ((((unsigned long long)(a + i)) | ((unsigned long long)(b + i))) & 15ull) == 0;
  if (vec) {
    *(float4*)(a + i) = float4{0.f, 0.f, 0.f, 0.f};
    *(float4*)(b + i) = float4{0.f, 0.f, 0.f, 0.f};
  } else {
    for (long long j = i; j < n && j < i + 4; ++j) {
      a[j] = 0.f;
      b[j] = 0.f;
    }
  }
}

__global__ void zero_words_kernel(unsigned* a, unsigned* b) {
  unsigned* p = blockIdx.x == 0 ? a : b;
  if (p) p[threadIdx.x] = 0u;
}

__global__ void gather_phase_window_kernel(const float* __restrict__ slots, long long bs, int f, long long fe, int f0, int nf,
                                           float* __restrict__ dst, long long n4) {
  const long long i = (long long)blockIdx.x * blockDim.x + threadIdx.x;
  if (i >= n4) return;
  const long long e = 4 * i, pv = (long long)nf * fe, v = e / pv, r = e - v * pv, j = r / fe, o = r - j * fe;
  const long long b = v / f, p = v - b * f;
  *(float4*)(dst + e) = *(const float4*)(slots + b * bs + ((f0 + j) * f + p) * fe + o);
}

}

namespace {
int rollout_run(const sf_rollouter* m, float* slots, int Bvid, int T_total, int first, int f, int pred_len, void* ws,
                size_t ws_bytes, void* stream) {
  SF_REQUIRE(m && slots && ws, "null pointer");
  SF_REQUIRE(Bvid >= 1 && pred_len >= 0 && f >= 1 && first >= 0, "bad batch / pred_len");
  SF_REQUIRE(m->num_slots >= 1 && m->slot_size > 0 && (m->slot_size % 4) == 0 && m->d_model > 0 &&
                 (m->d_model % 4) == 0 && m->ffn_dim > 0 && (m->ffn_dim % 4) == 0 && m->num_layers >= 1 &&
                 m->window_len >= 1, "bad rollouter shape");
  SF_REQUIRE(m->in_proj_w && m->in_proj_b && m->out_proj_w && m->out_proj_b && m->pe_tok, "null weight");
  SF_REQUIRE(check_layers(m->layers, m->num_layers) == 0, "null transformer-layer weight");
  const int n_in = m->single_step ? 1 : m->window_len;
  SF_REQUIRE(!(m->single_step && f > 1), "sf_rollout_phases_f32: a single-step rollouter takes frame_offset 1 only");
  SF_REQUIRE((long long)T_total >= first + (long long)(n_in + pred_len) * f, "slots buffer shorter than burn-in + pred_len");
  SF_REQUIRE((long long)Bvid * f <= 0x7fffffffLL / ((long long)m->window_len * m->num_slots), "batch too large");
  const int B = Bvid * f;
  SF_REQUIRE(ws_bytes >= sf_rollout_workspace_bytes(m, B), "workspace too small");
  hipStream_t st = (hipStream_t)stream;
  const int N = m->num_slots, C = m->slot_size, d = m->d_model, W = m->window_len, nl = m->num_layers;
  const float eps = 1e-5f;
  Bump bp{(char*)ws, ws_bytes};
  RolloutWs w;
  if (!rollout_ws_take(bp, w, m, B)) return sf_set_err(-1, "workspace too small", __FILE__, __LINE__);
  const RolloutPlan p = plan_rollout(m, B, sf_thread_opts());
  const bool ring_in = p.path == RolloutPlan::FUSED_RING;
  const bool long_ffn = p.path == RolloutPlan::LONG_WINDOW;
  const int np = p.attn == RolloutPlan::HEAD_PAIRS ? 4 : 1;
  const int RF = W + 1;
  const long long bs = (long long)T_total * N * C;
  slots += (long long)first * N * C;
  float* stage = nullptr;
  if (f > 1 && !ring_in) {
    const bool in_apb = !p.fused();
    stage = in_apb ? w.apb : w.ring;
    SF_REQUIRE(in_apb ? C <= 8 * d : (long long)W * C <= (long long)(W + 1) * d,
               "sf_rollout_phases_f32: slot_size too wide for this model's idle workspace (the staged window)");
  }
  if (ring_in) {
    SF_TRY(sf_ring_init_ex(m->out_proj_packed, m->out_proj_b, m->in_proj_packed, m->in_proj_b, slots, bs, n_in, w.ring, RF, N, B, st, f));
  }
  if (p.fused() || long_ffn) {
    SF_REQUIRE(sf_ffn_tiles(B * W * N) <= 1024, "batch too large for the fused-layer tile counters");
    hipLaunchKernelGGL(zero_words_kernel, dim3(2), dim3(1024), 0, st, (unsigned*)w.counters, p.seam ? w.seam_flags : nullptr);
    SF_CHECK_LAUNCH();
    if (p.attn == RolloutPlan::ROW_TILES) {
      const long long nfl = (long long)(sf_attn_rows_plane_bytes(B) / 4), half = nfl / 2;
      hipLaunchKernelGGL(zero_f32_kernel, dim3((unsigned)(((half + 3) / 4 + 255) / 256)), dim3(256), 0, st, w.planes, w.planes + half, half);
      SF_CHECK_LAUNCH();
    }
  }
  float* apb2 = w.apb + (size_t)4 * B * W * N * d;
  float* ap0 = w.apb;
  bool attn0_done = false;
  for (int s = 0; s < pred_len; ++s) {
    int nf, f0;
    step_window(m, s, nf, f0);
    const int L = nf * N, pe_off = (W - nf) * N;
    const float* pe = m->pe_tok + (long long)pe_off * d;
    float* cin = nullptr;
    if (!ring_in) {
      SfRowMap pmap = sf_rows(d);
      pmap.base = (long long)pe_off * d;
      if (stage) {
        const long long n4 = (long long)B * L * C / 4;
        hipLaunchKernelGGL(gather_phase_window_kernel, dim3((unsigned)((n4 + 255) / 256)), dim3(256), 0, st, slots, bs, f, (long long)N * C, f0, nf,
                           stage, n4);
        SF_CHECK_LAUNCH();
      }
      SF_TRY(sf_linear_ex(stage ? stage : slots, stage ? sf_rows(C) : sf_rows_batched(C, L, bs, (long long)f0 * N * C), m->in_proj_w, m->in_proj_b,
                          nullptr, nullptr, 0.f, m->pe_tok, pmap, L, w.x, sf_rows(d), B * L, d, C, 0, st));
      cin = w.x;
    }
    int l = 0;
    while (l < p.tok_layers) {
      const int nlt = (p.tok_layers - l) < 8 ? (p.tok_layers - l) : 8;
      float* xo = (cin == w.xa) ? w.xb2 : w.xa;
      if (ring_in)
        SF_TRY(sf_layer_tok_ex(l == 0 ? 1 : 0, cin, w.ring, RF, N, f0, pe, m->layers + l, nlt, eps, xo, B, L, st));
      else if (sf_layer_tok128_shape(d, m->num_heads, m->ffn_dim))
        SF_TRY(sf_layer_tok128_ex(cin, m->layers + l, nlt, eps, xo, B, L, st));
      else
        SF_TRY(sf_layer_tok_ex(0, cin, nullptr, 1, 1, 0, nullptr, m->layers + l, nlt, eps, xo, B, L, st));
      cin = xo;
      l += nlt;
    }
    if (!p.fused()) {
      int Lc = L;
      for (; l < nl; ++l) {
        const int Lq = (l == nl - 1 && m->norm_first) ? N : Lc;
        SF_TRY(tfm_layer(m->layers[l], cin, w.tw, B, Lc, Lq, d, m->num_heads, m->ffn_dim, m->norm_first, st, &cin,
                         long_ffn ? w.xpb : nullptr, long_ffn ? w.counters : nullptr));
        Lc = Lq;
      }
      const SfRowMap lastmap = (Lc == N) ? sf_rows(d) : sf_rows_batched(d, N, (long long)Lc * d, (long long)(Lc - N) * d);
      SF_TRY(sf_linear_ex(cin, lastmap, m->out_proj_w, m->out_proj_b, nullptr, nullptr, 0.f, nullptr, sf_rows(C), 0,
                          slots, sf_rows_batched(C, f * N, bs, (long long)(n_in + s) * f * N * C), B * N, C, d, 0, st));
      continue;
    }
    bool parts_in = false;
    float* parked = nullptr;
    for (; l < nl; ++l) {
      const sf_tfm_layer& lw = m->layers[l];
      const bool lastl = (l == nl - 1);
      const int Lq = lastl ? N : L;
      const long long pst = (long long)B * Lq * d;
      float* xo = (cin == w.xa) ? w.xb2 : w.xa;
      float* ap = (l == 0) ? ap0 : w.apb;
      if (parked) {
        ap = parked;
        SF_TRY(sf_attn_core_ex(lw, ap, w.planes, B, L, Lq, st));
      } else if (p.attn == RolloutPlan::ROW_TILES) {
        if (l == 0 && ring_in)
          SF_TRY(sf_attn_rows_ex(2, w.ring, (long long)RF * N * d, 0, pe, f0, RF, N, lw, eps, ap, w.planes, B, L, Lq, st));
        else if (parts_in)
          SF_TRY(sf_attn_rows_ex(1, w.xpb, (long long)L * d, (long long)B * L * d, nullptr, 0, 1, 1, lw, eps, ap, w.planes, B, L, Lq, st));
        else
          SF_TRY(sf_attn_rows_ex(0, cin, (long long)L * d, 0, nullptr, 0, 1, 1, lw, eps, ap, w.planes, B, L, Lq, st));
      } else if (p.attn == RolloutPlan::ALL_HEADS) {
        if (l == 0 && ring_in)
          SF_TRY(sf_attn_all_ring_ex(w.ring, RF, N, f0, pe, lw, eps, ap, B, L, Lq, st));
        else if (parts_in)
          SF_TRY(sf_attn_all_parts_ex(w.xpb, (long long)B * L * d, lw, eps, ap, B, L, Lq, st));
        else
          SF_TRY(sf_attn_all_ex(cin, lw, eps, ap, B, L, Lq, st));
      } else if (l == 0 && ring_in) {
        if (!attn0_done) SF_TRY(sf_attn_oproj_ring_ex(w.ring, RF, N, f0, pe, lw, eps, ap, pst, B, L, Lq, st));
      } else if (parts_in) {
        SF_TRY(sf_attn_oproj_parts_ex(w.xpb, (long long)B * L * d, lw, eps, ap, pst, B, L, Lq, st));
      } else {
        SF_TRY(sf_attn_oproj_ex(cin, lw, eps, ap, pst, B, L, Lq, st));
      }
      if (!lastl) {
        if (p.ffn == RolloutPlan::TILE_QKV) {
          float* park = (ap == w.apb) ? apb2 : w.apb;
          SF_TRY(sf_ffn_qkv_tile_ex(ap, lw, m->layers[l + 1], eps, park, w.planes, B, L, (l + 1 == nl - 1) ? N : L, m->ffn_dim, st));
          parked = park;
          cin = nullptr;
        } else if (p.ffn == RolloutPlan::TILE) {
          SF_TRY(sf_ffn_tile_ex(ap, lw, eps, xo, B * Lq, m->ffn_dim, st));
          cin = xo;
        } else {
          SF_TRY(sf_ffn_parts_ex(ap, pst, lw, eps, w.xpb, pst, B * Lq, m->ffn_dim, st, np));
          cin = nullptr;
        }
        parts_in = p.ffn == RolloutPlan::CHUNK_PARTS;
      } else if (ring_in) {
        int nf1 = 0, f01 = 0;
        if (s + 1 < pred_len) step_window(m, s + 1, nf1, f01);
        if (p.seam && s + 1 < pred_len && sf_seam_window_ok(nf1 * N, N)) {
          const int L1 = nf1 * N, Lq1 = (nl == 1) ? N : L1;
          float* ap_next = (ap == w.apb) ? apb2 : w.apb;
          SF_TRY(sf_seam_ex(ap, pst, lw, eps, w.xpb, pst, w.counters, m->ffn_dim, m->out_proj_packed, m->out_proj_b,
                            m->in_proj_packed, m->in_proj_b, slots, bs, n_in + s, w.ring, RF, N, B, m->layers[0], f01,
                            m->pe_tok + (long long)((W - nf1) * N) * d, ap_next, (long long)B * Lq1 * d, L1, Lq1, w.seam_flags,
                            (unsigned)(s + 1), st, f));
          ap0 = ap_next;
          attn0_done = true;
        } else {
          SF_TRY(sf_ffn_boundary_ex(ap, pst, lw, eps, w.xpb, pst, w.counters, m->ffn_dim, m->out_proj_packed, m->out_proj_b,
                                    m->in_proj_packed, m->in_proj_b, slots, bs, n_in + s, w.ring, RF, N, B, st, np, f));
          ap0 = w.apb;
          attn0_done = false;
        }
      } else {
        SF_TRY(sf_ffn_partial_ex(ap, pst, lw, eps, w.xpb, pst, xo, w.counters, B * Lq, m->ffn_dim, st, np));
        SF_TRY(sf_linear_ex(xo, sf_rows(d), m->out_proj_w, m->out_proj_b, nullptr, nullptr, 0.f, nullptr, sf_rows(C), 0,
                            slots, sf_rows_batched(C, f * N, bs, (long long)(n_in + s) * f * N * C), B * N, C, d, 0, st));
      }
    }
  }
  return 0;
}
}

extern "C" {

int sf_rollout_f32(const sf_rollouter* m, float* slots, int B, int T_total, int pred_len, void* ws,
                   size_t ws_bytes, void* stream) {
  return rollout_run(m, slots, B, T_total, 0, 1, pred_len, ws, ws_bytes, stream);
}

namespace {
struct OptsScope {
  SfThreadOpts saved;
  explicit OptsScope(const SfThreadOpts& o) : saved(sf_thread_opts()) { sf_thread_opts() = o; }
  ~OptsScope() { sf_thread_opts() = saved; }
};

SfThreadOpts rollout_thread_opts(const sf_rollout_opts* opts) {
  SfThreadOpts o = sf_thread_opts();
  if (!opts) return o;
  if (opts->precision >= 0) o.precision = opts->precision;
  if (opts->seam_fused >= 0) o.seam = opts->seam_fused ? 1 : 0;
  if (opts->ffn_rows > 0) o.ffn_rows = opts->ffn_rows;
  if (opts->attn_heads_per_wg > 0) o.attn_heads = opts->attn_heads_per_wg;
  if (opts->attn_qkv_rows > 0) o.attn_rows = opts->attn_qkv_rows;
  if (opts->ffn_tile > 0) o.ffn_tile = opts->ffn_tile;
  if (opts->cus_available > 0) o.cus = opts->cus_available;
  if (opts->layer_tok != 0) o.layer_tok = opts->layer_tok > 0 ? 1 : -1;
  return o;
}

int check_rollout_opts(const sf_rollout_opts* opts) {
  SF_REQUIRE(opts->precision >= -1 && opts->precision <= 3, "sf_rollout_opts: precision must be -1 (default), 0, 1, 2 or 3");
  SF_REQUIRE(opts->ffn_rows == 0 || opts->ffn_rows == 32 || opts->ffn_rows == 64 || opts->ffn_rows == 128,
             "sf_rollout_opts: ffn_rows must be 0 (default), 32, 64 or 128");
  SF_REQUIRE(opts->attn_heads_per_wg == 0 || opts->attn_heads_per_wg == 2 || opts->attn_heads_per_wg == 8,
             "sf_rollout_opts: attn_heads_per_wg must be 0 (default), 2 or 8");
  SF_REQUIRE(opts->attn_qkv_rows == 0 || opts->attn_qkv_rows == 128, "sf_rollout_opts: attn_qkv_rows must be 0 (off) or 128");
  SF_REQUIRE(opts->ffn_tile >= 0 && opts->ffn_tile <= 2, "sf_rollout_opts: ffn_tile must be 0, 1 or 2");
  SF_REQUIRE(opts->cus_available >= 0 && opts->cus_available <= 256, "sf_rollout_opts: cus_available must be 0 (whole chip) .. 256");
  return 0;
}
}

int sf_rollout_opts_f32(const sf_rollouter* m, float* slots, int B, int T_total, int pred_len, void* ws, size_t ws_bytes,
                        void* stream, const sf_rollout_opts* opts) {
  if (!opts) return sf_rollout_f32(m, slots, B, T_total, pred_len, ws, ws_bytes, stream);
  SF_TRY(check_rollout_opts(opts));
  OptsScope scope(rollout_thread_opts(opts));
  return sf_rollout_f32(m, slots, B, T_total, pred_len, ws, ws_bytes, stream);
}

size_t sf_rollout_phases_workspace_bytes(const sf_rollouter* m, int B, int frame_offset) {
  if (!m || B <= 0 || frame_offset <= 0 || (long long)B * frame_offset > 0x7fffffffLL) return 0;
  return sf_rollout_workspace_bytes(m, B * frame_offset);
}

int sf_rollout_phases_f32(const sf_rollouter* m, float* slots, int B, int T_total, int obs, int frame_offset, int pred_len, void* ws,
                          size_t ws_bytes, void* stream, const sf_rollout_opts* opts) {
  SF_REQUIRE(m && slots && ws, "null pointer");
  SF_REQUIRE(B >= 1 && pred_len >= 0, "bad batch / pred_len");
  SF_REQUIRE(frame_offset >= 1, "sf_rollout_phases_f32: frame_offset >= 1");
  SF_REQUIRE(!(m->single_step && frame_offset > 1), "sf_rollout_phases_f32: a single-step rollouter takes frame_offset 1 only");
  SF_REQUIRE(m->window_len >= 1, "bad rollouter shape");
  const int f = frame_offset, hist = m->single_step ? 1 : m->window_len;
  SF_REQUIRE((long long)obs >= (long long)hist * f, "sf_rollout_phases_f32: fewer observed frames than burn-in * frame_offset");
  const long long S = ((long long)pred_len + f - 1) / f;
  SF_REQUIRE((long long)T_total >= obs + S * f, "slots buffer shorter than obs + ceil(pred_len / frame_offset) * frame_offset");
  const int first = obs - hist * f;
  if (!opts) return rollout_run(m, slots, B, T_total, first, f, (int)S, ws, ws_bytes, stream);
  SF_TRY(check_rollout_opts(opts));
  OptsScope scope(rollout_thread_opts(opts));
  return rollout_run(m, slots, B, T_total, first, f, (int)S, ws, ws_bytes, stream);
}

int sf_rollout_is_fused(const sf_rollouter* m) { return plan_rollout(m, 1, sf_thread_opts()).fused(); }

int sf_rollout_tok_ok(const sf_rollouter* m) {
  SfThreadOpts o = sf_thread_opts();
  o.layer_tok = 1;
  const RolloutPlan p = plan_rollout(m, 1, o);
  return p.fused() && p.tok_layers > 0;
// ... 680 lines not shown
```

slotformer_amd/csrc/layer_fused.h:

```cpp
#pragma once
#include "../../include/slotformer_hip.h"
#include "sf_internal.h"

int sf_pred_step_ex(const float* prev, const sf_tfm_layer* layers, int nlayers, int heads, int ffn, int norm_first, const void* const* packed,
                    const float* lstm_b_ih, const float* lstm_b_hh, const float* proj_b, int hidden, float* lstm_h, float* lstm_c,
                    float* out, int B, int N, int D, float eps, hipStream_t st);

int sf_attn_oproj_ex(const float* xin, const sf_tfm_layer& w, float eps, float* ap, long long ap_stride, int B, int L,
                     int Lq, hipStream_t st);
int sf_attn_oproj_parts_ex(const float* xparts, long long xparts_stride, const sf_tfm_layer& w, float eps, float* ap,
                           long long ap_stride, int B, int L, int Lq, hipStream_t st);
int sf_ffn_parts_ex(const float* ap, long long ap_stride, const sf_tfm_layer& w, float eps, float* xp, long long xp_stride, int M,
                    int ffn, hipStream_t st, int np = 4);
int sf_attn_all_ex(const float* xin, const sf_tfm_layer& w, float eps, float* x2, int B, int L, int Lq, hipStream_t st);
int sf_attn_all_parts_ex(const float* xparts, long long xparts_stride, const sf_tfm_layer& w, float eps, float* x2, int B, int L,
                         int Lq, hipStream_t st);
int sf_attn_all_ring_ex(const float* ring, int ring_frames, int nslots, int f0, const float* pe, const sf_tfm_layer& w, float eps,
                        float* x2, int B, int L, int Lq, hipStream_t st);
int sf_attn_core_ex(const sf_tfm_layer& w, float* x2, void* planes, int B, int L, int Lq, hipStream_t st);
int sf_ffn_qkv_tile_ex(const float* x2, const sf_tfm_layer& w, const sf_tfm_layer& wn, float eps, float* xpark, void* planes, int B, int L, int Lq,
                       int ffn, hipStream_t st);
int sf_ffn_tile_ex(const float* x2, const sf_tfm_layer& w, float eps, float* y, int M, int ffn, hipStream_t st);
bool sf_layer_tok_ok(int L);
int sf_layer_tok_vpw(int L);
bool sf_layer_tok128_shape(int d_model, int num_heads, int ffn);
size_t sf_layer_tok128_packed_bytes();
int sf_pack_layer_tok128(const sf_tfm_layer* w, void* packed, hipStream_t st);
int sf_layer_tok128_ex(const float* xin, const sf_tfm_layer* layers, int nl, float eps, float* y, int B, int L, hipStream_t st);
int sf_layer_tok_ex(int mode, const float* xin, const float* ring, int ring_frames, int nslots, int f0, const float* pe, const sf_tfm_layer* layers, int nl,
                    float eps, float* y, int B, int L, hipStream_t st);
size_t sf_attn_rows_plane_bytes(int B);
int sf_attn_rows_ex(int mode, const float* xin, long long x_batch_stride, long long xparts_stride, const float* pe, int f0,
                    int ring_frames, int nslots, const sf_tfm_layer& w, float eps, float* x2, void* planes, int B, int L, int Lq,
                    hipStream_t st);
int sf_attn_oproj_ring_ex(const float* ring, int ring_frames, int nslots, int f0, const float* pe, const sf_tfm_layer& w,
                          float eps, float* ap, long long ap_stride, int B, int L, int Lq, hipStream_t st);
bool sf_step_boundary_ok(int d, int slot_size);
int sf_ffn_partial_ex(const float* ap, long long ap_stride, const sf_tfm_layer& w, float eps, float* xp,
                      long long xp_stride, float* xout, int* counters, int M, int ffn, hipStream_t st, int np = 4);
int sf_ffn_tiles(int M);
int sf_ring_init_ex(const void* wout_packed, const float* b_out, const void* win_packed, const float* b_in, float* slots,
                    long long slots_bs, int n_frames, float* ring, int ring_frames, int nslots, int B, hipStream_t st, int phases = 1);
int sf_ffn_boundary_ex(const float* ap, long long ap_stride, const sf_tfm_layer& w, float eps, float* xp, long long xp_stride,
                       int* counters, int ffn, const void* wout_packed, const float* b_out, const void* win_packed,
                       const float* b_in, float* slots, long long slots_bs, int frame, float* ring, int ring_frames, int nslots,
                       int B, hipStream_t st, int np = 4, int phases = 1);
int sf_seam_ex(const float* ap_ffn, long long pst_ffn, const sf_tfm_layer& wl, float eps, float* xp, long long xp_stride,
               int* counters, int ffn, const void* wout_packed, const float* b_out, const void* win_packed, const float* b_in,
               float* slots, long long slots_bs, int frame, float* ring, int ring_frames, int nslots, int B,
               const sf_tfm_layer& w0, int f0_next, const float* pe, float* ap_attn, long long pst_attn, int L, int Lq,
               unsigned* seam_flags, unsigned epoch, hipStream_t st, int phases = 1);
int sf_seam_blocks(int B, int nslots);
bool sf_seam_window_ok(int L, int nslots);
```

slotformer_amd/csrc/layer_tok.hip:

```cpp
#include "../../include/slotformer_hip.h"
#include "sf_internal.h"
#include "layer_fused.h"
#include "layer_tok_common.h"
#include <stdlib.h>

namespace {
constexpr int LT_NT = 256, LT_D = 256, LT_F = 1024, LT_NH = 8, LT_TOK = 128, LT_MAXL = 8;
constexpr int LT_STAGE = 32 * 1024, LT_RING = 3;
constexpr int LT_NST_ATT = 4 * LT_NH, LT_NST = LT_NST_ATT + 2 * (LT_F / 32);
constexpr int LT_KV = LT_RING * LT_STAGE;
constexpr int LT_VT = LT_KV + 16 * 1024;
constexpr int LT_PAR = LT_KV + 32 * 1024;
constexpr int P_LN1G = 0, P_LN1B = 256, P_BQKV = 512, P_BO = 1280, P_LN2G = 1536, P_LN2B = 1792, P_B1 = 2048, P_B2 = 3072, P_N = 3328;
constexpr size_t LT_LDS = (size_t)LT_PAR + (size_t)P_N * 4;
constexpr size_t LT_BLOB = (size_t)LT_NST * LT_STAGE + (size_t)P_N * 4;
static_assert(LT_LDS <= 160 * 1024, "LDS budget");

struct LtArgs {
  const float* x;
  const float* ring;
  const float* pe;
  float* y;
  const char* blob[LT_MAXL];
  float eps;
  int nl, B, L, vpw, RF, N, f0, dbg_ts;
};
}

__device__ long long lt_ts[16];
#define LTS(i) do { if (A.dbg_ts && blockIdx.x == 0 && threadIdx.x == 0) lt_ts[i] = wall_clock64(); } while (0)

template <int MODE>
__global__ __launch_bounds__(LT_NT) void layer_tok_kernel(LtArgs A) {
  extern __shared__ __attribute__((aligned(16))) char smem[];
  float* P = (float*)(smem + LT_PAR);
  const int t = threadIdx.x, lane = t & 63;
  const int wave = __builtin_amdgcn_readfirstlane(t >> 6);
  const int n = lane & 31, h = lane >> 5;
  const int L = A.L;
  const int v0 = blockIdx.x * A.vpw;
  const int nvalid = min(A.vpw, A.B - v0) * L;
  const int tl = wave * 32 + n;
  const int te = min(tl, nvalid - 1);
  const int vl = te / L, tok = te - vl * L;
  const long long row = (long long)(v0 + vl) * L + tok;
  LTS(0);
  f32x16 X[8];
  if constexpr (MODE == 0) {
    const float* xr = A.x + row * LT_D + 4 * h;
#pragma unroll
    for (int ob = 0; ob < 8; ++ob)
#pragma unroll
      for (int g = 0; g < 4; ++g) {
        const f32x4 v = *(const f32x4*)(xr + 32 * ob + 8 * g);
#pragma unroll
        for (int q = 0; q < 4; ++q) X[ob][4 * g + q] = v[q];
      }
  } else {
    const int fr = tok / A.N, sl = tok - fr * A.N;
    const float* rr = A.ring + (((long long)(v0 + vl) * A.RF + (A.f0 + fr) % A.RF) * A.N + sl) * LT_D + 4 * h;
    const float* pr = A.pe + (long long)tok * LT_D + 4 * h;
#pragma unroll
    for (int ob = 0; ob < 8; ++ob)
#pragma unroll
      for (int g = 0; g < 4; ++g) {
        const f32x4 v = *(const f32x4*)(rr + 32 * ob + 8 * g);
#pragma unroll
        for (int q = 0; q < 4; ++q) X[ob][4 * g + q] = v[q];
      }
    __builtin_amdgcn_sched_barrier(0);
#pragma unroll
    for (int ob = 0; ob < 8; ++ob) {
#pragma unroll
      for (int g = 0; g < 4; ++g) {
        const f32x4 v = *(const f32x4*)(pr + 32 * ob + 8 * g);
#pragma unroll
        for (int q = 0; q < 4; ++q) X[ob][4 * g + q] += v[q];
      }
      __builtin_amdgcn_sched_barrier(0);
    }
  }
  const unsigned wlane = (unsigned)(wave * 8 * 1024 + lane * 16);
  char* const wdst = smem + (wave * 8) * 1024;
  int cur = 0;
  int cs = -2;
  const char* base_cur = A.blob[0];
  const char* base_nxt = A.blob[0];
  bool last_layer = false;
  auto stage_src = [&]() -> const char* {
    const int t2 = cs + 2;
    const bool wrap = t2 >= LT_NST;
    const char* b = wrap ? base_nxt : base_cur;
    const int so = wrap ? (last_layer ? LT_NST - 1 : t2 - LT_NST) : t2;
    ++cs;
    return b + (size_t)so * LT_STAGE + wlane;
  };
  {
    const char* s0 = stage_src();
    const char* s1 = stage_src();
    LtRing R0{nullptr, s0, wdst}, R1{nullptr, s1, wdst + LT_STAGE};
#pragma unroll
    for (int f = 0; f < 8; ++f) lt_dma(R0, f);
#pragma unroll
    for (int f = 0; f < 8; ++f) lt_dma(R1, f);
  }
#ifdef LT_STAMPS
  long long c_wait = 0, c_bar = 0, c_last = 0, c_work = 0;
#endif
  auto stage_begin = [&]() -> LtRing {
#ifdef LT_STAMPS
    const long long c0 = __builtin_readcyclecounter();
    if (c_last) c_work += c0 - c_last;
#endif
#ifdef LT_NODMA
    asm volatile("s_waitcnt vmcnt(0)" ::: "memory");
#else
    asm volatile("s_waitcnt vmcnt(8)" ::: "memory");
#endif
    asm volatile("s_waitcnt lgkmcnt(0)" ::: "memory");
#ifdef LT_STAMPS
    const long long c1 = __builtin_readcyclecounter();
#endif
#ifndef LT_NOBAR
    __builtin_amdgcn_s_barrier();
#endif
    asm volatile("" ::: "memory");
#ifdef LT_STAMPS
    c_last = __builtin_readcyclecounter();
    c_wait += c1 - c0;
    c_bar += c_last - c1;
#endif
    const int nb = cur == 0 ? 2 : cur - 1;
    LtRing R{smem + cur * LT_STAGE + lane * 16, stage_src(), wdst + nb * LT_STAGE};
#ifdef LT_BURST
#pragma unroll
    for (int f = 0; f < 8; ++f) lt_dma_now(R, f);
#endif
    cur = cur == 2 ? 0 : cur + 1;
    return R;
  };
  const int wf = min(wave * 32, nvalid - 1);
  const int kb0 = ((wf / L) * L) >> 5;
  const int d0 = 32 * kb0 + 4 * h - vl * L;
  const char* pb;
  {
    unsigned pbo = (unsigned)(LT_PAR + 16 * h);
    asm volatile("" : "+v"(pbo));
    pb = smem + pbo;
  }
  const int g16 = lane >> 4;
  const char *px, *pg;
  {
    unsigned pxo = (unsigned)(LT_PAR + 4 * LT16_FEAT(g16)), pgo = (unsigned)(LT_PAR + 16 * g16);
    asm volatile("" : "+v"(pxo), "+v"(pgo));
    px = smem + pxo;
    pg = smem + pgo;
  }
  char* const kwr = smem + LT_KV + wave * 1024 + lane * 16;
  char* const vwr = smem + LT_VT + wave * 4096 + lane * 16;
  const char* krd[3];
  const char* vrd[3];
#pragma unroll
  for (int kbi = 0; kbi < 3; ++kbi) {
    const int kb = min(kb0 + kbi, 3);
    krd[kbi] = smem + LT_KV + kb * 1024 + lane * 16;
    vrd[kbi] = smem + LT_VT + kb * 4096 + lane * 16;
  }
  const float qscale = 0.2550348616841918f;
  constexpr float NEG = -3.0e38f;
  LTS(1);

#pragma unroll 1
  for (int l = 0; l < A.nl; ++l) {
    cs = 0;
    base_cur = A.blob[l];
    last_layer = l + 1 >= A.nl;
    base_nxt = A.blob[last_layer ? l : l + 1];
    __syncthreads();
    {
      const float* vsrc = (const float*)(A.blob[l] + (size_t)LT_NST * LT_STAGE);
      for (int i = t; i < P_N / 4; i += LT_NT) *(f32x4*)(P + 4 * i) = *(const f32x4*)(vsrc + 4 * i);
    }
    __syncthreads();
    if (l == 0) LTS(2);
    bf16x8 xh[16], xl[16];
    lt_layernorm<P_LN1G, P_LN1B>(X, pb, h, A.eps, xh, xl);
    lt_add_vec<P_BO>(X, pb);
    if (l == 0) LTS(3);
    f32x16 qa, ka, va, S[3], O;
    bf16x8 qh[2], ql[2], ph[3][2], pl[3][2], oh[2], ol[2];
    float mx0 = NEG, mx1 = NEG, mx = 0.f, sm = 0.f, rinv = 0.f;
    auto zero16 = [](f32x16& a) {
#pragma unroll
      for (int r = 0; r < 16; ++r) a[r] = 0.f;
    };
    int hq = 0;
    auto mask_chunk = [&](int c) {
      const int kbi = c >> 1;
#pragma unroll
      for (int rr = 0; rr < 8; ++rr) {
        const int r = 8 * (c & 1) + rr;
        const bool ok = (unsigned)(d0 + 32 * kbi + 8 * (r >> 2) + (r & 3)) < (unsigned)L;
        const float v = ok ? S[kbi][r] : NEG;
        S[kbi][r] = v;
        if (rr & 1) mx1 = fmaxf(mx1, v); else mx0 = fmaxf(mx0, v);
      }
    };
    auto exp_chunk = [&](int c) {
      const int kbi = c >> 1;
      float s0 = 0.f, s1 = 0.f;
#pragma unroll
      for (int rr = 0; rr < 8; ++rr) {
        const int r = 8 * (c & 1) + rr;
#ifdef LT_EXPF
        const float e = __expf((S[kbi][r] - mx) * 0.6931471805599453f);
#else
        const float e = __builtin_amdgcn_exp2f(S[kbi][r] - mx);
#endif
        S[kbi][r] = e;
        if (rr & 1) s1 += e; else s0 += e;
      }
      sm += s0 + s1;
    };
    auto psplit_chunk = [&](int c) { sf_split8(quad(S[c >> 1], 2 * (c & 1)), quad(S[c >> 1], 2 * (c & 1) + 1), ph[c >> 1][c & 1], pl[c >> 1][c & 1]); };
    auto kconv = [&](int s) {
      const float* bk = (const float*)pb + P_BQKV + 256 + 32 * hq;
      bf16x8 fh, fl;
      sf_split8(quad(ka, 2 * s) + *(const f32x4*)(bk + 16 * s), quad(ka, 2 * s + 1) + *(const f32x4*)(bk + 16 * s + 8), fh, fl);
      *(bf16x8*)(kwr + (s * 2) * 4096) = fh;
      *(bf16x8*)(kwr + (s * 2 + 1) * 4096) = fl;
    };
    auto qconv = [&](int s) {
      const float* bq = (const float*)pb + P_BQKV + 32 * hq;
      sf_split8((quad(qa, 2 * s) + *(const f32x4*)(bq + 16 * s)) * qscale, (quad(qa, 2 * s + 1) + *(const f32x4*)(bq + 16 * s + 8)) * qscale, qh[s], ql[s]);
    };
    auto vconv = [&](int s) {
      const float bv = P[P_BQKV + 512 + 32 * hq + n];
      bf16x8 fh, fl;
      sf_split8(quad(va, 2 * s) + bv, quad(va, 2 * s + 1) + bv, fh, fl);
      *(bf16x8*)(vwr + (s * 2) * 1024) = fh;
      *(bf16x8*)(vwr + (s * 2 + 1) * 1024) = fl;
    };
    auto oconv = [&](int s) { sf_split8(quad(O, 2 * s) * rinv, quad(O, 2 * s + 1) * rinv, oh[s], ol[s]); };
    auto scores = [&]() {
      bf16x8 kh[3][2], kl[3][2];
#pragma unroll
      for (int kbi = 0; kbi < 3; ++kbi)
#pragma unroll
        for (int s = 0; s < 2; ++s) {
          kh[kbi][s] = *(const bf16x8*)(krd[kbi] + (s * 2) * 4096);
          kl[kbi][s] = *(const bf16x8*)(krd[kbi] + (s * 2 + 1) * 4096);
        }
#pragma unroll
      for (int kbi = 0; kbi < 3; ++kbi) zero16(S[kbi]);
#pragma unroll
      for (int s = 0; s < 2; ++s) {
#pragma unroll
        for (int kbi = 0; kbi < 3; ++kbi) { S[kbi] = LT_MFMA(kh[kbi][s], ql[s], S[kbi]); LT_PIN(); }
#pragma unroll
        for (int kbi = 0; kbi < 3; ++kbi) { S[kbi] = LT_MFMA(kl[kbi][s], qh[s], S[kbi]); LT_PIN(); }
#pragma unroll
        for (int kbi = 0; kbi < 3; ++kbi) { S[kbi] = LT_MFMA(kh[kbi][s], qh[s], S[kbi]); LT_PIN(); }
      }
      mx0 = mx1 = NEG;
      sm = 0.f;
    };
    auto pv = [&]() {
      f32x16 Op[3];
      bf16x8 vh[3][2], vlo[3][2];
#pragma unroll
      for (int kbi = 0; kbi < 3; ++kbi)
#pragma unroll
        for (int s = 0; s < 2; ++s) {
          vh[kbi][s] = *(const bf16x8*)(vrd[kbi] + (s * 2) * 1024);
          vlo[kbi][s] = *(const bf16x8*)(vrd[kbi] + (s * 2 + 1) * 1024);
        }
#pragma unroll
      for (int kbi = 0; kbi < 3; ++kbi) zero16(Op[kbi]);
#pragma unroll
      for (int s = 0; s < 2; ++s) {
#pragma unroll
        for (int kbi = 0; kbi < 3; ++kbi) { Op[kbi] = LT_MFMA(vh[kbi][s], pl[kbi][s], Op[kbi]); LT_PIN(); }
#pragma unroll
        for (int kbi = 0; kbi < 3; ++kbi) { Op[kbi] = LT_MFMA(vlo[kbi][s], ph[kbi][s], Op[kbi]); LT_PIN(); }
#pragma unroll
        for (int kbi = 0; kbi < 3; ++kbi) { Op[kbi] = LT_MFMA(vh[kbi][s], ph[kbi][s], Op[kbi]); LT_PIN(); }
      }
#pragma unroll
      for (int r = 0; r < 16; ++r) O[r] = (Op[0][r] + Op[1][r]) + Op[2][r];
    };
    auto sideD = [&](int g) {
      if (g < 6) mask_chunk(g);
      if (g == 6) mx = lt_xmax(fmaxf(mx0, mx1), h);
      if (g == 7) exp_chunk(0);
    };
    auto sideA = [&](int g) {
      if (g == 0) { exp_chunk(1); exp_chunk(2); }
      if (g == 1) { exp_chunk(3); exp_chunk(4); }
      if (g == 2) { exp_chunk(5); rinv = 1.0f / lt_xsum(sm, h); psplit_chunk(0); }
      if (g == 3) { psplit_chunk(1); psplit_chunk(2); }
      if (g == 4) { psplit_chunk(3); psplit_chunk(4); }
      if (g == 5) psplit_chunk(5);
    };
    {
      const LtRing R = stage_begin();
      lt_row_product<false, 0>(R, xh, xl, qa, LtNoSide{});
    }
    {
      const LtRing R = stage_begin();
      lt_row_product<false, 0>(R, xh, xl, ka, LtNoSide{});
    }
    {
      const LtRing R = stage_begin();
      lt_row_product<true, 5>(R, xh, xl, va, [&](int g) {
        if (g < 2) kconv(g);
        else if (g < 4) qconv(g - 2);
      });
      vconv(0);
      vconv(1);
    }
#pragma unroll 1
    for (hq = 1; hq < LT_NH; ++hq) {
      {
        const LtRing R = stage_begin();
        scores();
          lt_row_product<false, 6>(R, xh, xl, qa, sideD);
      }
      {
        const LtRing R = stage_begin();
          lt_row_product<false, 6>(R, xh, xl, ka, sideA);
        pv();
      }
      {
        const LtRing R = stage_begin();
          lt_row_product<true, 5>(R, xh, xl, va, [&](int g) {
          if (g < 2) kconv(g);
          else if (g < 4) qconv(g - 2);
          else if (g < 6) oconv(g - 4);
        });
      }
      {
        const LtRing R = stage_begin();
        lt_kslice_product<5>(R, oh, ol, X, [&](int g) {
          if (g < 2) vconv(g);
        });
      }
    }
    asm volatile("s_waitcnt lgkmcnt(0)" ::: "memory");
    __builtin_amdgcn_s_barrier();
    asm volatile("" ::: "memory");
    scores();
#pragma unroll
    for (int g = 0; g < 8; ++g) sideD(g);
#pragma unroll
    for (int g = 0; g < 6; ++g) sideA(g);
    pv();
    oconv(0);
    oconv(1);
    {
      const LtRing R = stage_begin();
      lt_kslice_product<0>(R, oh, ol, X, LtNoSide{});
    }
    if (l == 0) LTS(4);
#ifdef LT_STAMPS
    if (l == 0 && blockIdx.x == 0 && threadIdx.x == 0) { lt_ts[8] = c_wait; lt_ts[9] = c_bar; lt_ts[10] = c_work; }
#endif
    lt16_swap_layout(X);
    lt16_layernorm<P_LN2G, P_LN2B>(X, px, g16, A.eps, xh, xl);
    lt16_add_vec<P_B2>(X, px);
    if (l == 0) LTS(5);
    f32x4 Ha[2][2], Hb[2][2];
    bf16x8 hh[2], hl[2];
    f32x4 b1q[2];
    auto b1_load = [&](int blk) {
      const float* b1 = (const float*)pg + P_B1 + 32 * blk;
#pragma unroll
      for (int r = 0; r < 2; ++r) b1q[r] = *(const f32x4*)(b1 + 16 * r);
    };
    typedef unsigned __attribute__((ext_vector_type(4))) lt_u32x4;
    lt_u32x4 hw[2], lw[2];
    auto hconv_piece = [&](const f32x4 (&Hx)[2][2], int k) {
      const int t16 = k >> 2, w = k & 3, r = w >> 1, e = 2 * (w & 1);
      unsigned hi, lo;
      pl_split2(fmaxf(Hx[r][t16][e] + b1q[r][e], 0.f), fmaxf(Hx[r][t16][e + 1] + b1q[r][e + 1], 0.f), hi, lo);
      hw[t16][w] = hi;
      lw[t16][w] = lo;
    };
    auto hconv_done = [&]() {
#pragma unroll
      for (int t16 = 0; t16 < 2; ++t16) {
        hh[t16] = __builtin_bit_cast(bf16x8, hw[t16]);
        hl[t16] = __builtin_bit_cast(bf16x8, lw[t16]);
      }
    };
    auto ffn_step = [&](f32x4 (&Hn)[2][2], const f32x4 (&Hp)[2][2], int j) {
      {
        const LtRing R = stage_begin();
        lt16_row_product<2, 8>(R, xh, xl, Hn, [&](int ks) { hconv_piece(Hp, ks); });
        hconv_done();
        asm volatile("" : "+v"(hh[0]), "+v"(hh[1]), "+v"(hl[0]), "+v"(hl[1]));
      }
      {
        const LtRing R = stage_begin();
        b1_load(j);
        lt16_kslice_product<0>(R, hh, hl, X, LtNoSide{});
      }
    };
    {
      const LtRing R = stage_begin();
      b1_load(0);
      lt16_row_product<0, 8>(R, xh, xl, Ha, LtNoSide{});
    }
    ffn_step(Hb, Ha, 1);
#pragma unroll 1
    for (int j = 2; j < LT_F / 32; j += 2) {
      ffn_step(Ha, Hb, j);
      ffn_step(Hb, Ha, j + 1);
    }
#pragma unroll
    for (int k = 0; k < 8; ++k) hconv_piece(Hb, k);
    hconv_done();
    {
      const LtRing R = stage_begin();
      lt16_kslice_product<0>(R, hh, hl, X, LtNoSide{});
    }
    lt16_swap_layout(X);
    if (l == 0) LTS(6);
#ifdef LT_STAMPS
    if (l == 0 && blockIdx.x == 0 && threadIdx.x == 0) { lt_ts[11] = c_wait; lt_ts[12] = c_bar; lt_ts[13] = c_work; }
#endif
  }
  asm volatile("s_waitcnt vmcnt(0)" ::: "memory");
  if (tl < nvalid) {
    float* yr = A.y + row * LT_D + 4 * h;
#pragma unroll
    for (int ob = 0; ob < 8; ++ob)
#pragma unroll
      for (int g = 0; g < 4; ++g) *(f32x4*)(yr + 32 * ob + 8 * g) = quad(X[ob], g);
  }
  LTS(7);
}

extern "C" int sf_debug_read_ts_layer_tok(long long* out16) {
  hipError_t e = hipMemcpyFromSymbol(out16, HIP_SYMBOL(lt_ts), sizeof(long long) * 16);
  return e == hipSuccess ? 0 : (int)e;
}

extern "C" size_t sf_layer_tok_packed_bytes(void) { return LT_BLOB; }
extern "C" size_t sf_layer_tok_packed_bytes_ex(int d_model, int num_heads, int ffn) {
  if (d_model == LT_D && num_heads == LT_NH && ffn == LT_F) return LT_BLOB;
  return sf_layer_tok128_shape(d_model, num_heads, ffn) ? sf_layer_tok128_packed_bytes() : 0;
}

extern "C" int sf_pack_layer_tok_weights(const sf_tfm_layer* w, void* packed, int d_model, int num_heads, int ffn, void* stream) {
  SF_REQUIRE(w && packed, "sf_pack_layer_tok_weights: null pointer");
  SF_REQUIRE(w->in_proj_w && w->out_proj_w && w->lin1_w && w->lin2_w && w->norm1_g && w->norm1_b && w->in_proj_b && w->out_proj_b && w->norm2_g &&
                 w->norm2_b && w->lin1_b && w->lin2_b, "sf_pack_layer_tok_weights: null weight");
  hipStream_t st = (hipStream_t)stream;
  if (sf_layer_tok128_shape(d_model, num_heads, ffn)) return sf_pack_layer_tok128(w, packed, st);
  SF_REQUIRE(d_model == LT_D && num_heads == LT_NH && ffn == LT_F, "sf_pack_layer_tok_weights: (d_model, heads, ffn) = (256, 8, 1024) or (128, 8, 512) only");
  constexpr int n_att = LT_NST_ATT * 32 * 64, n_ffn = (LT_NST - LT_NST_ATT) * 32 * 64;
  static_assert(n_att % 256 == 0 && n_ffn % 256 == 0, "whole blocks");
  hipLaunchKernelGGL((pack_layer_tok_kernel<LT_D, LT_F>), dim3(n_att / 256), dim3(256), 0, st, w->in_proj_w, w->out_proj_w, w->lin1_w, w->lin2_w, (uint4*)packed);
  SF_CHECK_LAUNCH();
  hipLaunchKernelGGL((pack_layer_tok_ffn16_kernel<LT_D, LT_F>), dim3(n_ffn / 256), dim3(256), 0, st, w->lin1_w, w->lin2_w, (uint4*)packed);
  SF_CHECK_LAUNCH();
  float* vec = (float*)((char*)packed + (size_t)LT_NST * LT_STAGE);
  const struct {
    const float* src;
    int off, n;
  } parts[8] = {{w->norm1_g, P_LN1G, 256}, {w->norm1_b, P_LN1B, 256}, {w->in_proj_b, P_BQKV, 768}, {w->out_proj_b, P_BO, 256},
                {w->norm2_g, P_LN2G, 256}, {w->norm2_b, P_LN2B, 256}, {w->lin1_b, P_B1, 1024},   {w->lin2_b, P_B2, 256}};
  for (const auto& p : parts) {
    const hipError_t e = hipMemcpyAsync(vec + p.off, p.src, (size_t)p.n * 4, hipMemcpyDeviceToDevice, st);
    if (e != hipSuccess) return sf_set_err((int)e, hipGetErrorString(e), __FILE__, __LINE__);
  }
  return 0;
}

int sf_layer_tok_vpw(int L) {
  if (L < 1 || L > 96) return 0;
  for (int vpw = LT_TOK / L; vpw >= 1; --vpw) {
    const int nvalid = vpw * L;
    bool ok = true;
    for (int w = 0; w < 4 && ok; ++w) {
      const int wf = w * 32 < nvalid ? w * 32 : nvalid - 1, wl = w * 32 + 31 < nvalid ? w * 32 + 31 : nvalid - 1;
      const int kb0 = ((wf / L) * L) >> 5, kb1 = (((wl / L) * L) + L - 1) >> 5;
      ok = kb1 - kb0 + 1 <= 3;
    }
    if (ok) return vpw;
  }
  return 0;
}
bool sf_layer_tok_ok(int L) { return sf_layer_tok_vpw(L) > 0; }

int sf_layer_tok_ex(int mode, const float* xin, const float* ring, int ring_frames, int nslots, int f0, const float* pe, const sf_tfm_layer* layers, int nl,
                    float eps, float* y, int B, int L, hipStream_t st) {
  bool ok = layers && nl >= 1 && nl <= LT_MAXL && sf_layer_tok_ok(L) && B >= 1 && y && (mode == 0 ? xin != nullptr : (ring && pe && nslots >= 1 && ring_frames >= 1));
  for (int l = 0; ok && l < nl; ++l) ok = layers[l].tok_packed != nullptr;
  if (!ok)
    return sf_set_err(-1, "invalid argument: the token-stationary layers need sf_pack_layer_tok_weights fragments, 1..8 layers and 1 <= L <= 96 rows per video", __FILE__, __LINE__);
  static const int dbg = sf_dbg("lt");
  LtArgs A;
  A.x = xin; A.ring = ring; A.pe = pe; A.y = y;
  for (int l = 0; l < LT_MAXL; ++l) A.blob[l] = (const char*)layers[l < nl ? l : nl - 1].tok_packed;
  A.eps = eps; A.nl = nl; A.B = B; A.L = L; A.vpw = sf_layer_tok_vpw(L); A.RF = ring_frames; A.N = nslots; A.f0 = f0; A.dbg_ts = dbg;
  const int nwg = (B + A.vpw - 1) / A.vpw;
  const double flops = nl * ((double)B * L * (2.0 * LT_D * (3 * LT_D + LT_D + 2 * LT_F)) + (double)B * LT_NH * 4.0 * L * L * 32);
  if (mode == 0) {
    SF_TRY(sf_ensure_dyn_lds((const void*)layer_tok_kernel<0>, LT_LDS));
    sf_prof_begin(SF_K_LAYER_TOK, st, flops);
    hipLaunchKernelGGL(layer_tok_kernel<0>, dim3(nwg), dim3(LT_NT), LT_LDS, st, A);
  } else {
    SF_TRY(sf_ensure_dyn_lds((const void*)layer_tok_kernel<1>, LT_LDS));
    sf_prof_begin(SF_K_LAYER_TOK, st, flops);
    hipLaunchKernelGGL(layer_tok_kernel<1>, dim3(nwg), dim3(LT_NT), LT_LDS, st, A);
  }
  sf_prof_end(SF_K_LAYER_TOK, st);
  SF_CHECK_LAUNCH();
  return 0;
}

extern "C" int sf_layer_tok_block_f32(const sf_tfm_layer* w, int nl, const float* x, float* y, int B, int L, void* stream) {
  SF_REQUIRE(w && x && y && B > 0 && nl >= 1 && nl <= LT_MAXL, "sf_layer_tok_block_f32: null pointer / empty problem / more than 8 layers");
  SF_REQUIRE(sf_get_precision() == 1, "sf_layer_tok_block_f32: split-bf16 mode only");
  return sf_layer_tok_ex(0, x, nullptr, 1, 1, 0, nullptr, w, nl, 1e-5f, y, B, L, (hipStream_t)stream);
}

extern "C" int sf_layer_tok_block_ex_f32(const sf_tfm_layer* w, int nl, int d_model, int num_heads, int ffn, const float* x, float* y, int B, int L,
                                         void* stream) {
  SF_REQUIRE(w && x && y && B > 0 && nl >= 1 && nl <= LT_MAXL, "sf_layer_tok_block_ex_f32: null pointer / empty problem / more than 8 layers");
  SF_REQUIRE(sf_get_precision() == 1, "sf_layer_tok_block_ex_f32: split-bf16 mode only");
  if (sf_layer_tok128_shape(d_model, num_heads, ffn)) return sf_layer_tok128_ex(x, w, nl, 1e-5f, y, B, L, (hipStream_t)stream);
  SF_REQUIRE(d_model == LT_D && num_heads == LT_NH && ffn == LT_F, "sf_layer_tok_block_ex_f32: (d_model, heads, ffn) = (256, 8, 1024) or (128, 8, 512) only");
  return sf_layer_tok_ex(0, x, nullptr, 1, 1, 0, nullptr, w, nl, 1e-5f, y, B, L, (hipStream_t)stream);
}
```

slotformer_amd/csrc/sf_switches.cpp:

```cpp
#include <stdlib.h>
#include <atomic>

#include "../../include/slotformer_hip.h"
#include "sf_internal.h"

namespace {
enum Parse { NO_ENV, FLAG, PRECISION };
struct Row {
  const char* env;
  int def;
  Parse parse;
};
constexpr Row ROWS[SF_SW_NUM] = {
     {"SF_PRECISION", 1, PRECISION},
     {"SF_LAYER_TOK", 0, FLAG},
     {"SF_SEAM_FUSED", 1, FLAG},
     {nullptr, 0, NO_ENV},
     {"SF_CONV_FP16X2", 0, FLAG},
     {nullptr, 1, NO_ENV},
     {nullptr, 1, NO_ENV},
     {nullptr, 0, NO_ENV},
     {nullptr, 1, NO_ENV},
     {nullptr, 1, NO_ENV},
     {"SF_CONV_WS", 1, FLAG},
};

std::atomic<int> g_slot[SF_SW_NUM];

int initial(const Row& r) {
  const char* e = r.env ? getenv(r.env) : nullptr;
  if (!e) return r.def;
  if (r.parse == PRECISION) return (e[0] == 'f' || e[0] == '0') ? 0 : (strcmp(e, "bf16") == 0 ? 2 : 1);
  return r.def ? e[0] != '0' : e[0] == '1';
}
}

int sf_switch(SfSwitch s) {
  int v = g_slot[s].load(std::memory_order_relaxed);
  if (v == 0) {
    v = initial(ROWS[s]) + 1;
    int seen = 0;
    if (!g_slot[s].compare_exchange_strong(seen, v, std::memory_order_relaxed)) v = seen;
  }
  return v - 1;
}

int sf_switch_set(SfSwitch s, int v) {
  g_slot[s].store(v + 1, std::memory_order_relaxed);
  return 0;
}

extern "C" {
int sf_get_precision(void) { return sf_precision(sf_thread_opts()); }
int sf_set_precision(int mode) {
  if (mode < 0 || mode > 2) return sf_set_err(-1, "invalid argument: precision mode must be 0 (f32), 1 (bf16x3) or 2 (bf16)", __FILE__, __LINE__);
  return sf_switch_set(SF_SW_PRECISION, mode);
}
int sf_get_layer_tok(void) { return sf_switch(SF_SW_LAYER_TOK); }
int sf_set_layer_tok(int on) { return sf_switch_set(SF_SW_LAYER_TOK, on != 0); }
int sf_get_seam_fused(void) { return sf_switch(SF_SW_SEAM_FUSED); }
int sf_set_seam_fused(int on) { return sf_switch_set(SF_SW_SEAM_FUSED, on != 0); }
int sf_get_ffn_rows64(void) { return sf_switch(SF_SW_FFN_ROWS64); }
int sf_set_ffn_rows64(int on) { return sf_switch_set(SF_SW_FFN_ROWS64, on != 0); }
int sf_get_conv_fp16x2(void) { return sf_switch(SF_SW_CONV_FP16X2); }
int sf_set_conv_fp16x2(int on) { return sf_switch_set(SF_SW_CONV_FP16X2, on != 0); }
int sf_get_slot_attn_tile16(void) { return sf_switch(SF_SW_SLOT_ATTN_TILE16); }
int sf_set_slot_attn_tile16(int on) { return sf_switch_set(SF_SW_SLOT_ATTN_TILE16, on != 0); }
int sf_get_encode_fuse_next(void) { return sf_switch(SF_SW_ENCODE_FUSE_NEXT); }
int sf_set_encode_fuse_next(int on) { return sf_switch_set(SF_SW_ENCODE_FUSE_NEXT, on != 0); }
int sf_get_slot_chain(void) { return sf_switch(SF_SW_SLOT_CHAIN); }
int sf_set_slot_chain(int on) { return sf_switch_set(SF_SW_SLOT_CHAIN, on != 0); }
int sf_get_slot_attn_planes(void) { return sf_switch(SF_SW_SLOT_ATTN_PLANES); }
int sf_set_slot_attn_planes(int on) { return sf_switch_set(SF_SW_SLOT_ATTN_PLANES, on != 0); }
int sf_get_pixel_tok(void) { return sf_switch(SF_SW_PIXEL_TOK); }
int sf_set_pixel_tok(int on) { return sf_switch_set(SF_SW_PIXEL_TOK, on != 0); }
}
```

slotformer_amd/csrc/sf_switches.h:

```cpp
#pragma once

enum SfSwitch {
  SF_SW_PRECISION,
  SF_SW_LAYER_TOK,
  SF_SW_SEAM_FUSED,
  SF_SW_FFN_ROWS64,
  SF_SW_CONV_FP16X2,
  SF_SW_SLOT_ATTN_TILE16,
  SF_SW_ENCODE_FUSE_NEXT,
  SF_SW_SLOT_CHAIN,
  SF_SW_SLOT_ATTN_PLANES,
  SF_SW_PIXEL_TOK,
  SF_SW_CONV_WS,
  SF_SW_NUM
};

int sf_switch(SfSwitch s);
int sf_switch_set(SfSwitch s, int v);

extern "C" int sf_get_precision(void);
```

slotformer_amd/engine.py:

```python
import ctypes as C
import os

import torch

from . import _lib
from ._lib import lib, check, sf_tfm_layer, sf_rollouter, sf_savi_encoder, sf_savi_decoder
from . import ops, plans

_WORKSPACES = {}


def workspace(device, nbytes, slot=0):
    key = (device.type, device.index, slot)
    cur = _WORKSPACES.get(key)
    if cur is None or cur.numel() < nbytes:
        cur = torch.empty(int(nbytes), dtype=torch.uint8, device=device)
        _WORKSPACES[key] = cur
    return cur


def release_workspaces(prefix):
    n = len(prefix)
    for key in [k for k in _WORKSPACES if isinstance(k[2], tuple) and len(k[2]) > 1 and isinstance(k[2][1], tuple) and k[2][1][:n] == prefix]:
        del _WORKSPACES[key]


def kernel_noise(m, noise, B, T, device):
    if getattr(m, 'kernel_dist_layer', None) is None or getattr(m, 'kld_method', None) == 'none':
        return None
    if noise is not None:
        return noise
    return torch.randn(B, T, m.num_slots, m.slot_size, device=device)


def _require_inference(module, *tensors):
    if torch.is_grad_enabled() and any(p.requires_grad for p in module.parameters()):
        raise NotImplementedError(
            'slotformer_amd: this call is inference-only on the HIP path (the training nodes of row N1 live in train.py); '
            'wrap the call in torch.no_grad()')
    for t in tensors:
        if t is not None and not t.is_cuda:
            raise RuntimeError('slotformer_amd: inputs must live on a HIP device; there is no CPU fallback')


invalidate = plans.invalidate


def _tfm_layers(plan, encoder, pack_ffn=False):
    n = len(encoder.layers)
    arr = (sf_tfm_layer * n)()
    for i, l in enumerate(encoder.layers):
        a = arr[i]
        d, ffn = l.linear1.in_features, l.linear1.out_features
        if pack_ffn and d == 256 and ffn == 1024 and l.linear1.weight.is_cuda:
            nb = lib().sf_ffn_packed_bytes(d, ffn)
            p1 = torch.empty(nb, dtype=torch.uint8, device=l.linear1.weight.device)
            p2 = torch.empty(nb, dtype=torch.uint8, device=l.linear1.weight.device)
            check(lib().sf_pack_ffn_weights(plan.dp(l.linear1.weight), plan.dp(l.linear2.weight), p1.data_ptr(),
                                            p2.data_ptr(), d, ffn, torch.cuda.current_stream().cuda_stream))
            plan.keep += [p1, p2]
            a.lin1_packed, a.lin2_packed = p1.data_ptr(), p2.data_ptr()
            if l.self_attn.num_heads == 8:
                q1 = torch.empty(lib().sf_attn_packed_bytes(d, 0), dtype=torch.uint8, device=p1.device)
                q2 = torch.empty(lib().sf_attn_packed_bytes(d, 1), dtype=torch.uint8, device=p1.device)
                check(lib().sf_pack_attn_weights(plan.dp(l.self_attn.in_proj_weight), plan.dp(l.self_attn.out_proj.weight),
                                                 q1.data_ptr(), q2.data_ptr(), d, 8, torch.cuda.current_stream().cuda_stream))
                plan.keep += [q1, q2]
                a.attn_in_packed, a.attn_out_packed = q1.data_ptr(), q2.data_ptr()
        a.norm1_g, a.norm1_b = plan.dp(l.norm1.weight), plan.dp(l.norm1.bias)
        a.in_proj_w, a.in_proj_b = plan.dp(l.self_attn.in_proj_weight), plan.dp(l.self_attn.in_proj_bias)
        a.out_proj_w, a.out_proj_b = plan.dp(l.self_attn.out_proj.weight), plan.dp(l.self_attn.out_proj.bias)
        a.norm2_g, a.norm2_b = plan.dp(l.norm2.weight), plan.dp(l.norm2.bias)
        a.lin1_w, a.lin1_b = plan.dp(l.linear1.weight), plan.dp(l.linear1.bias)
        a.lin2_w, a.lin2_b = plan.dp(l.linear2.weight), plan.dp(l.linear2.bias)
        heads = l.self_attn.num_heads
        if a.attn_in_packed or (pack_ffn and (d, heads, ffn) == (128, 8, 512) and l.linear1.weight.is_cuda):
            tp = torch.empty(lib().sf_layer_tok_packed_bytes_ex(d, heads, ffn), dtype=torch.uint8, device=l.linear1.weight.device)
            check(lib().sf_pack_layer_tok_weights(C.byref(a), tp.data_ptr(), d, heads, ffn, torch.cuda.current_stream().cuda_stream))
            plan.keep.append(tp)
            a.tok_packed = tp.data_ptr()
    plan.keep.append(arr)
    return arr


def rollouter_plan(r, packed=True):
    return plans.cached(r, 'rollouter' if packed else 'rollouter_train', plans.signature(r), _rollouter_plan, r, packed)


def _rollouter_plan(r, packed):
    plan = plans.Plan()
    s = sf_rollouter()
    single = hasattr(r, 'cond_len')
    W = r.cond_len if single else r.history_len
    N = r.num_slots
    s.num_slots, s.slot_size, s.d_model = N, r.in_proj.in_features, r.in_proj.out_features
    enc = r.transformer_encoder
    l0 = enc.layers[0]
    s.num_layers, s.num_heads = len(enc.layers), l0.self_attn.num_heads
    s.ffn_dim, s.norm_first = l0.linear1.out_features, int(l0.norm_first)
    s.window_len, s.single_step = W, int(single)
    s.in_proj_w, s.in_proj_b = plan.dp(r.in_proj.weight), plan.dp(r.in_proj.bias)
    s.out_proj_w, s.out_proj_b = plan.dp(r.out_proj.weight), plan.dp(r.out_proj.bias)
    pe = r.enc_t_pe.detach()[0].repeat_interleave(N, dim=0)
    if r.enc_slots_pe is not None:
        pe = pe + r.enc_slots_pe.detach()[0].repeat(W, 1)
    s.pe_tok = plan.dp(pe.contiguous())
    s.layers = C.cast(_tfm_layers(plan, enc, pack_ffn=packed), C.POINTER(sf_tfm_layer))
    if packed and s.d_model == 256 and s.slot_size == 128 and r.in_proj.weight.is_cuda:
        s.in_proj_packed, s.out_proj_packed = plan.packed(r.in_proj.weight), plan.packed(r.out_proj.weight)
    plan.struct = s
    return plan


def phyre_readout_plan(m):
    return plans.cached(m, 'phyre_readout', plans.signature(m), _phyre_readout_plan, m)


def _phyre_readout_plan(m):
    plan = plans.Plan()
    plan.struct = plan.layers = C.cast(_tfm_layers(plan, m.transformer_encoder, pack_ffn=True), C.POINTER(sf_tfm_layer))
    return plan


def aloe_plan(tm):
    return plans.cached(tm, 'aloe', plans.signature(tm), _aloe_plan, tm)


def _aloe_plan(tm):
    plan = plans.Plan()
    s = _lib.sf_aloe()
    enc = tm.transformer_encoder
    l0 = enc.layers[0]
    s.slot_size, s.question_len = tm.vision_in_proj.in_features - 2, tm.question_len
    s.d_model, s.num_heads, s.ffn_dim, s.num_layers = tm.d_model, l0.self_attn.num_heads, l0.linear1.out_features, len(enc.layers)
    s.vocab, s.emb_dim = tm.q_embedding.num_embeddings, tm.q_embedding.embedding_dim
    s.cls, s.pos = plan.dp(tm.CLS.reshape(-1)), plan.dp(enc.pos_enc.reshape(-1, tm.d_model))
    s.vision_w, s.vision_b = plan.dp(tm.vision_in_proj.weight), plan.dp(tm.vision_in_proj.bias)
    s.q_in_proj_w = plan.dp(tm.q_in_proj.weight)
    plan.text_table = ops.aloe_text_table(tm.q_embedding.weight.detach().float().contiguous(), tm.q_in_proj.weight.detach().float().contiguous(),
                                          tm.q_in_proj.bias.detach().float().contiguous())
    s.text_table = plan.dp(plan.text_table)
    s.layers = C.cast(_tfm_layers(plan, enc), C.POINTER(sf_tfm_layer))
    plan.struct = s
    return plan


def rollout_opts(opts):
    if opts is None:
        return None
    if isinstance(opts, _lib.sf_rollout_opts):
        return opts
    unknown = set(opts) - {'precision', 'seam', 'ffn_rows', 'attn_heads', 'attn_rows', 'ffn_tile', 'cus', 'layer_tok'}
    if unknown:
        raise ValueError(f'slotformer_amd: unknown rollout options {sorted(unknown)}')
    prec = opts.get('precision', -1)
    prec = {'f32': 0, 'bf16x3': 1, 'bf16': 2, 'fp16': 3}.get(prec, prec)
    seam = opts.get('seam', None)
    return _lib.sf_rollout_opts(int(prec), -1 if seam is None else int(bool(seam)), int(opts.get('ffn_rows', 0)), int(opts.get('attn_heads', 0)),
                                int(opts.get('attn_rows', 0)), int(opts.get('ffn_tile', 0)), int(opts.get('cus', 0)),
                                {None: 0, True: 1, False: -1}[opts.get('layer_tok', None)])


def burn_in_of(r):
    return 1 if hasattr(r, 'cond_len') else r.history_len


def rollout(r, slots_all, n_in, pred_len, ws_slot=0, opts=None):
    _require_inference(r, slots_all)
    ops._chk(slots_all)
    if n_in != burn_in_of(r):
        raise RuntimeError(f'slotformer_amd: burn-in of {n_in} frames, but this rollouter consumes {burn_in_of(r)} '
                           '(history_len; 1 for SingleStepSlotRollouter)')
    plan = rollouter_plan(r)
    B, T_total = slots_all.shape[:2]
    need = lib().sf_rollout_workspace_bytes(C.byref(plan.struct), B)
    ws = workspace(slots_all.device, need, ('roll', ws_slot))
    o = rollout_opts(opts)
    check(lib().sf_rollout_opts_f32(C.byref(plan.struct), slots_all.data_ptr(), B, T_total, pred_len, ws.data_ptr(),
                                    ws.numel(), torch.cuda.current_stream().cuda_stream, None if o is None else C.byref(o)))
    return slots_all


def rollout_phases(r, slots_all, obs, pred_len, frame_offset, ws_slot=0, opts=None):
    if slots_all.dim() != 4:
        raise ValueError(f'slotformer_amd: rollout slots are [B, T_total, N, C], got {tuple(slots_all.shape)}')
    f, obs, pred_len, hist = int(frame_offset), int(obs), int(pred_len), burn_in_of(r)
    B, T_total = slots_all.shape[:2]
    if f < 1:
        raise ValueError(f'slotformer_amd: frame_offset >= 1, got {frame_offset!r}')
    if f > 1 and hasattr(r, 'cond_len'):
        raise ValueError('slotformer_amd: a SingleStepSlotRollouter rolls out at frame_offset 1 only')
    if B < 1 or pred_len < 0:
        raise ValueError(f'slotformer_amd: rollout of {B} videos for {pred_len} frames')
    if obs < hist * f:
        raise ValueError(f'slotformer_amd: {obs} observed frames, but a burn-in of {hist} frames at frame_offset {f} needs {hist * f}')
    steps = -(-pred_len // f)
    if T_total < obs + steps * f:
        raise ValueError(f'slotformer_amd: every phase runs {steps} steps and frames {obs} .. {obs + steps * f - 1} are written, but the buffer has '
                         f'{T_total} frames (pad it to obs + ceil(pred_len / frame_offset) * frame_offset and slice)')
    _require_inference(r, slots_all)
    ops._chk(slots_all)
    plan = rollouter_plan(r)
    need = lib().sf_rollout_phases_workspace_bytes(C.byref(plan.struct), B, f)
    ws = workspace(slots_all.device, need, ('roll', ws_slot))
    o = rollout_opts(opts)
    check(lib().sf_rollout_phases_f32(C.byref(plan.struct), slots_all.data_ptr(), B, T_total, obs, f, pred_len, ws.data_ptr(), ws.numel(),
                                      torch.cuda.current_stream().cuda_stream, None if o is None else C.byref(o)))
    return slots_all


def encoder_plan(m):
    return plans.cached(m, 'encoder', plans.signature(m), _encoder_plan, m)


def _encoder_plan(m):
    plan = plans.Plan()
    s = sf_savi_encoder()
    if m.resolution[0] != m.resolution[1] or m.resolution[0] not in (64, 128):
        raise NotImplementedError(f'resolution {m.resolution}: the encoder needs 64x64 or 128x128 input '
                                  '(visual_resolution is fixed to 64x64, savi.py:226)')
    s.resolution = m.resolution[0]
    ch = list(m.enc_channels)
    n = len(ch) - 1
    if n > 8:
        raise NotImplementedError('at most 8 encoder convs')
    s.enc_layers, s.enc_ks = n, m.enc_ks
    for i, c in enumerate(ch):
        s.enc_channels[i] = c
    for i in range(n):
        conv = m.encoder[i][0]
        w = conv.weight.detach().float().contiguous()
        wp = w if i == 0 else ops.pack_conv_weight(w)
        s.conv_w[i] = plan.dp(wp)
        s.conv_b[i] = plan.dp(conv.bias)
        if i > 0 and w.is_cuda and tuple(w.shape) == (64, 64, 5, 5):
            frag = ops.pack_conv_frag(wp)
            plan.keep.append(frag)
            s.conv_w_frag[i] = frag.data_ptr()
    pe = m.encoder_pos_embedding
    s.pos_table = plan.dp(ops.pos_embed_table(pe.grid.detach().float(), pe.dense.weight.detach().float().contiguous(),
                                              pe.dense.bias.detach().float().contiguous()))
    eo = m.encoder_out_layer
    s.enc_ln_g, s.enc_ln_b = plan.dp(eo[0].weight), plan.dp(eo[0].bias)
    s.enc_fc1_w, s.enc_fc1_b = plan.dp(eo[1].weight), plan.dp(eo[1].bias)
    s.enc_fc2_w, s.enc_fc2_b = plan.dp(eo[3].weight), plan.dp(eo[3].bias)
    s.enc_out_channels = m.enc_out_channels
    s.num_slots, s.slot_size, s.slot_mlp_size = m.num_slots, m.slot_size, m.slot_mlp_size
    s.num_iterations = m.num_iterations
    sa = m.slot_attention
    s.sa_norm_in_g, s.sa_norm_in_b = plan.dp(sa.norm_inputs.weight), plan.dp(sa.norm_inputs.bias)
    s.sa_q_ln_g, s.sa_q_ln_b = plan.dp(sa.project_q[0].weight), plan.dp(sa.project_q[0].bias)
    s.sa_q_w = plan.dp(sa.project_q[1].weight)
    s.sa_q_w_t = plan.dp(sa.project_q[1].weight.detach().float().t().contiguous())
    s.sa_kv_w = plan.dp(torch.cat([sa.project_k.weight.detach(), sa.project_v.weight.detach()], 0).contiguous())
    tr = lambda w: w.detach().float().t().contiguous()
    s.gru_w_ih, s.gru_w_hh = plan.dp(tr(sa.gru.weight_ih)), plan.dp(tr(sa.gru.weight_hh))
    s.gru_b_ih, s.gru_b_hh = plan.dp(sa.gru.bias_ih), plan.dp(sa.gru.bias_hh)
    s.mlp_ln_g, s.mlp_ln_b = plan.dp(sa.mlp[0].weight), plan.dp(sa.mlp[0].bias)
    s.mlp_w1, s.mlp_b1 = plan.dp(tr(sa.mlp[1].weight)), plan.dp(sa.mlp[1].bias)
    s.mlp_w2, s.mlp_b2 = plan.dp(tr(sa.mlp[3].weight)), plan.dp(sa.mlp[3].bias)
# ... 274 lines not shown
```

slotformer_amd/switches.py:

```python
import os

SWITCHES = {
    'SF_PRECISION': ('product', "process default of the matrix arithmetic: 'bf16x3' (default; split-bf16, fp32-equivalent) | 'f32' (exact-f32 MFMA) | 'bf16' (single pass)"),
    'SF_LAYER_TOK': ('product', "process default of sf_rollout_opts.layer_tok for DIRECT rollout calls (0, default: the row-tile / latency forms; 1: the layers before the last as token-stationary launches -- d_model 256 rollouters on the fused / long-window paths, and the OBJ3D shape (128, 8, 512) on the generic path, where it pays from ~64 videos per call and costs 7 % at 32: `sf_rollout_tok_layers` tells what a call takes). The pipeline passes its own choice per unit"),
    'SF_SEAM_FUSED': ('product', "process default of the seam launches of the latency forms (1; 0: two launches instead)"),
    'SF_CONV_FP16X2': ('product', "OPT-IN two-product fp16 form of the 5x5 convolutions (weights rounded to fp16: 3-6e-5 from the fixtures instead of 1e-5); default 0"),
    'SF_CONV_WS': ('product', "0: the 4-row-tile convolution everywhere (default 1: the weights-stationary kernel on streams with CUs of their own; the same bits)"),
    'SF_ENCODE_FORK': ('product', "direct encode calls as two branches on two streams (1, default) or one stream (0)"),
    'SF_PIPE_TOK': ('product', "0: the pipeline never uses the token-stationary layer launches (every unit bit-identical to the serial module calls)"),
    'SF_PIPE_GROUP': ('product', "batches per rollout unit (default: 6 for token-stationary units of 32-video batches, else 4 / unit_batches_for)"),
    'SF_PIPE_HYBRID': ('product', "every k-th batch behind the fill is encoded on an unmasked stream beside the CU-masked lane (default 8 with token-stationary units, 3 / 5 / 0 otherwise)"),
    'SF_PIPE_FILL': ('product', "batches encoded on the whole chip at the start of a run (default: three units' worth)"),
    'SF_PIPE_CU_SPLIT': ('product', "CU mask of the encode partition, e.g. rows4 (default: sized from the two sides' CU time)"),
    'SF_PIPE_ENCODE_GRAPH': ('product', "replay the encode of a batch from a hipGraph (1, default) or launch it eagerly (0)"),
    'SF_PIPE_TRACE': ('tools', "record the device timeline of a run (tools/pipe_timeline.py)"),
    'SF_LIB_PATH': ('tools', "load another build of libslotformer_hip.so (tools/build_variant.sh: -D variants of a kernel)"),
    'SF_DBG': ('tools', "in-kernel time stamps and tuning overrides of the probes, comma separated: conv, lt, lf=<bits>, deconv, gemm, gemmcfg=<id>, convcfg=<id>, sab1 / flash1 (the packed-word attention backward / exact-f32 flash forward the bf16-plane kernels replaced), sabts (tools/*_probe.py)"),
}

PROCESS = {
    'precision': ('sf_set_precision', 'sf_get_precision', 'SF_PRECISION', 1, "matrix arithmetic: 0 exact-f32 MFMA, 1 split-bf16 (bf16x3), 2 single-pass bf16; the getter answers the calling thread's per-call precision while one is set"),
    'layer_tok': ('sf_set_layer_tok', 'sf_get_layer_tok', 'SF_LAYER_TOK', 0, "sf_rollout_opts.layer_tok == 0: the layers before the last of a rollout as token-stationary launches"),
    'seam_fused': ('sf_set_seam_fused', 'sf_get_seam_fused', 'SF_SEAM_FUSED', 1, "sf_rollout_opts.seam_fused == -1: seam launches of the rollout's latency forms"),
    'ffn_rows64': ('sf_set_ffn_rows64', 'sf_get_ffn_rows64', None, 0, "sf_rollout_opts.ffn_rows == 0: 64 instead of 32 rows per workgroup of the chunk-partial FFN launches (the same bits)"),
    'conv_fp16x2': ('sf_set_conv_fp16x2', 'sf_get_conv_fp16x2', 'SF_CONV_FP16X2', 0, "OPT-IN two-product fp16 arithmetic of the 64 -> 64 5x5 convolutions"),
    'slot_attn_tile16': ('sf_set_slot_attn_tile16', 'sf_get_slot_attn_tile16', None, 1, "9 .. 16 slots, keys == values: the one-pass tile kernel of Slot Attention (0: the two-pass kernel)"),
    'encode_fuse_next': ('sf_set_encode_fuse_next', 'sf_get_encode_fuse_next', None, 1, "the slot prologue of step t + 1 at the tail of step t's last slot update (0: its own launch; split-bf16 rounding apart)"),
    'slot_chain': ('sf_set_slot_chain', 'sf_get_slot_chain', None, 0, "OPT-IN: the slot branch of a batched encode as one video-stationary launch"),
    'slot_attn_planes': ('sf_set_slot_attn_planes', 'sf_get_slot_attn_planes', None, 1, "Slot-Attention iterations of the encode on feature rows kept as two bf16 planes, split-bf16 MFMAs (0: f32 rows, exact-f32 tile kernel)"),
    'pixel_tok': ('sf_set_pixel_tok', 'sf_get_pixel_tok', None, 1, "the per-pixel chain of the encoder in its pixel-stationary form (0: the tile kernels; another summation order)"),
}


def check_environment(environ=None):
    environ = os.environ if environ is None else environ
    seen = {k: v for k, v in environ.items() if k.startswith('SF_')}
    return {k: v for k, v in seen.items() if k in SWITCHES}, sorted(k for k in seen if k not in SWITCHES)


def markdown_table():
    rows = ['| variable | kind | what it does |', '|---|---|---|']
    rows += [f'| `{k}` | {kind} | {text} |' for k, (kind, text) in SWITCHES.items()]
    return '\n'.join(rows)


def process_table():
    rows = ['| switch | setter / getter | environment | default | what it selects |', '|---|---|---|---|---|']
    rows += [f"| {k} | `{s}` / `{g}` | {f'`{env}`' if env else '-'} | {default} | {text} |" for k, (s, g, env, default, text) in PROCESS.items()]
    return '\n'.join(rows)


if __name__ == '__main__':
    print(markdown_table())
    print()
    print(process_table())
```

Measured before the change: 714,300.

## Fuse last layer's LN1 and q|k|v into token-stationary launch tail; prefetch layer vectors by DMA

Adds an opt-in tail mode to the token-stationary layer kernel. After the launch's last layer, it runs LN1 and the q|k|v projection of the following row-pruned layer and writes bf16 planes, so the rollout can skip the separate q|k|v launch of the row-tile form. Independently, each layer's vector parameters (norms, biases) are now prefetched into LDS with asynchronous global-to-LDS loads overlapped with the weight stream, replacing a synchronous copy between two barriers. This adds wait-count bookkeeping and a larger tail weight blob. The tail is off by default.

```diff
diff --git a/include/slotformer_hip.h b/include/slotformer_hip.h
--- a/include/slotformer_hip.h
+++ b/include/slotformer_hip.h
@@ -313,8 +313,15 @@
 int sf_layer_tok_block_f32(const sf_tfm_layer* w, int nl, const float* x, float* y, int B, int L, void* stream);
 int sf_layer_tok_block_ex_f32(const sf_tfm_layer* w, int nl, int d_model, int num_heads, int ffn, const float* x, float* y, int B, int L, void* stream);
 int sf_debug_read_ts_layer_tok(long long* out16);
+size_t sf_layer_tok_tail_packed_bytes(void);
+int sf_pack_layer_tok_tail(const sf_tfm_layer* w, void* packed, void* stream);
+int sf_layer_tok_tail_f32(const sf_tfm_layer* w, int nl, const void* tail_packed, const float* x, float* xpark, void* planes, int B, int L, int Lq,
+                          void* stream);
+int sf_layer_tok_tail_set(int on);
+int sf_layer_tok_tail_get(void);
 size_t sf_attn_rows_planes_bytes(int B);
 int sf_attn_block_rows_f32(const sf_tfm_layer* w, const float* x, float* out, void* planes, int B, int L, int Lq, void* stream);
+int sf_attn_rows_part_f32(const sf_tfm_layer* w, const float* x, float* out, void* planes, int B, int L, int Lq, int part, void* stream);
 
 int sf_phyre_readout_ok(int num_slots, int slot_size, int T, int d_model, int num_heads, int ffn, int num_layers);
 size_t sf_phyre_readout_workspace_bytes(int B, int num_slots, int T);
@@ -356,6 +363,7 @@
   const float* pe_tok;
   const sf_tfm_layer* layers;
   const void *in_proj_packed, *out_proj_packed;
+  const void* tok_tail_packed;
 } sf_rollouter;
 
 size_t sf_packed_linear_bytes(int N, int K);
diff --git a/slotformer_amd/_lib.py b/slotformer_amd/_lib.py
--- a/slotformer_amd/_lib.py
+++ b/slotformer_amd/_lib.py
@@ -18,7 +18,8 @@
         'num_slots', 'slot_size', 'd_model', 'num_layers', 'num_heads', 'ffn_dim', 'norm_first',
         'window_len', 'single_step')] + [(n, FP) for n in (
             'in_proj_w', 'in_proj_b', 'out_proj_w', 'out_proj_b', 'pe_tok')] + [
-                ('layers', C.POINTER(sf_tfm_layer)), ('in_proj_packed', C.c_void_p), ('out_proj_packed', C.c_void_p)]
+                ('layers', C.POINTER(sf_tfm_layer)), ('in_proj_packed', C.c_void_p), ('out_proj_packed', C.c_void_p),
+                ('tok_tail_packed', C.c_void_p)]
 
 
 class sf_aloe(C.Structure):
@@ -235,8 +236,14 @@
     'sf_layer_tok_block_f32': (I, [C.POINTER(sf_tfm_layer), I, FP, FP, I, I, VP]),
     'sf_layer_tok_block_ex_f32': (I, [C.POINTER(sf_tfm_layer), I, I, I, I, FP, FP, I, I, VP]),
     'sf_debug_read_ts_layer_tok': (I, [C.POINTER(C.c_longlong)]),
+    'sf_layer_tok_tail_packed_bytes': (SZ, []),
+    'sf_pack_layer_tok_tail': (I, [C.POINTER(sf_tfm_layer), VP, VP]),
+    'sf_layer_tok_tail_f32': (I, [C.POINTER(sf_tfm_layer), I, VP, FP, FP, VP, I, I, I, VP]),
+    'sf_layer_tok_tail_set': (I, [I]),
+    'sf_layer_tok_tail_get': (I, []),
     'sf_attn_rows_planes_bytes': (SZ, [I]),
     'sf_attn_block_rows_f32': (I, [C.POINTER(sf_tfm_layer), FP, FP, VP, I, I, I, VP]),
+    'sf_attn_rows_part_f32': (I, [C.POINTER(sf_tfm_layer), FP, FP, VP, I, I, I, I, VP]),
     'sf_slot_attn_iter_bwd_workspace_bytes': (SZ, [I, I, I, I]),
     'sf_slot_attn_iter_bwd_f32': (I, [FP, FP, I, LL, FP, FP, FP, I, FP, FP, FP, I, FP, I, I, I, I, F32, F32, VP, SZ, VP]),
     'sf_slot_attn_iter_bwd16_workspace_bytes': (SZ, [I, I, I, I]),
diff --git a/slotformer_amd/csrc/attn_rows.hip b/slotformer_amd/csrc/attn_rows.hip
--- a/slotformer_amd/csrc/attn_rows.hip
+++ b/slotformer_amd/csrc/attn_rows.hip
@@ -528,6 +528,15 @@
   return sf_attn_rows_ex(0, x, (long long)L * D, 0, nullptr, 0, 1, 1, *w, 1e-5f, out, planes, B, L, Lq, (hipStream_t)stream);
 }
 
+extern "C" int sf_attn_rows_part_f32(const sf_tfm_layer* w, const float* x, float* out, void* planes, int B, int L, int Lq, int part, void* stream) {
+  SF_REQUIRE(w && out && planes && B > 0 && (part == 1 || x), "sf_attn_rows_part_f32: null pointer / empty problem");
+  SF_REQUIRE(L >= 1 && L <= 64 && Lq >= 1 && Lq <= L && (part == 0 || part == 1), "sf_attn_rows_part_f32: needs 1 <= Lq <= L <= 64 and part 0 or 1");
+  SF_REQUIRE(w->norm1_g && w->norm1_b && w->in_proj_b && w->out_proj_b && w->attn_in_packed && w->attn_out_packed,
+             "sf_attn_rows_part_f32: null weight (packed attention weights needed)");
+  if (part == 1) return sf_attn_core_ex(*w, out, planes, B, L, Lq, (hipStream_t)stream);
+  return sf_attn_rows_ex(0, x, (long long)L * D, 0, nullptr, 0, 1, 1, *w, 1e-5f, out, planes, B, L, Lq, (hipStream_t)stream);
+}
+
 extern "C" int sf_debug_read_ts_rows(long long* out32) {
   hipError_t e = hipMemcpyFromSymbol(out32, HIP_SYMBOL(ar_ts), sizeof(long long) * 32);
   return e == hipSuccess ? 0 : (int)e;
diff --git a/slotformer_amd/csrc/engine.hip b/slotformer_amd/csrc/engine.hip
--- a/slotformer_amd/csrc/engine.hip
+++ b/slotformer_amd/csrc/engine.hip
@@ -121,6 +121,7 @@
   enum Attn { HEAD_PAIRS, ALL_HEADS, ROW_TILES } attn = HEAD_PAIRS;
   enum Ffn { CHUNK_PARTS, TILE, TILE_QKV } ffn = CHUNK_PARTS;
   bool seam = false;
+  bool tok_tail = false;
   bool fused() const { return path == FUSED_ROWS || path == FUSED_RING; }
 };
 
@@ -143,6 +144,7 @@
     bool tok = tok_on;
     for (int nf = m->single_step ? 1 : W; nf <= W && tok; ++nf) tok = sf_layer_tok_ok(nf * N);
     p.tok_layers = tok ? nl - 1 : 0;
+    p.tok_tail = tok && m->tok_tail_packed && sf_switch(SF_SW_LAYER_TOK_TAIL) && sf_layer_tok_tail_ok(Lmax);
     p.attn = (o.attn_rows == 128 || tok) ? RolloutPlan::ROW_TILES : (o.attn_heads == 8 ? RolloutPlan::ALL_HEADS : RolloutPlan::HEAD_PAIRS);
     if (p.attn != RolloutPlan::HEAD_PAIRS && o.ffn_tile >= 1)
       p.ffn = (p.attn == RolloutPlan::ROW_TILES && o.ffn_tile == 2) ? RolloutPlan::TILE_QKV : RolloutPlan::TILE;
@@ -332,10 +334,14 @@
       cin = w.x;
     }
     int l = 0;
+    float* tail_parked = nullptr;
     while (l < p.tok_layers) {
       const int nlt = (p.tok_layers - l) < 8 ? (p.tok_layers - l) : 8;
       float* xo = (cin == w.xa) ? w.xb2 : w.xa;
-      if (ring_in)
+      if (p.tok_tail && l + nlt == p.tok_layers) {
+        SF_TRY(sf_layer_tok_tail_ex(ring_in && l == 0 ? 1 : 0, cin, w.ring, RF, N, f0, pe, m->layers + l, nlt, m->tok_tail_packed, eps, xo, w.planes, B, L, N, st));
+        tail_parked = xo;
+      } else if (ring_in)
         SF_TRY(sf_layer_tok_ex(l == 0 ? 1 : 0, cin, w.ring, RF, N, f0, pe, m->layers + l, nlt, eps, xo, B, L, st));
       else if (sf_layer_tok128_shape(d, m->num_heads, m->ffn_dim))
         SF_TRY(sf_layer_tok128_ex(cin, m->layers + l, nlt, eps, xo, B, L, st));
@@ -358,7 +364,7 @@
       continue;
     }
     bool parts_in = false;
-    float* parked = nullptr;
+    float* parked = tail_parked;
     for (; l < nl; ++l) {
       const sf_tfm_layer& lw = m->layers[l];
       const bool lastl = (l == nl - 1);
diff --git a/slotformer_amd/csrc/layer_fused.h b/slotformer_amd/csrc/layer_fused.h
--- a/slotformer_amd/csrc/layer_fused.h
+++ b/slotformer_amd/csrc/layer_fused.h
@@ -29,6 +29,9 @@
 int sf_layer_tok128_ex(const float* xin, const sf_tfm_layer* layers, int nl, float eps, float* y, int B, int L, hipStream_t st);
 int sf_layer_tok_ex(int mode, const float* xin, const float* ring, int ring_frames, int nslots, int f0, const float* pe, const sf_tfm_layer* layers, int nl,
                     float eps, float* y, int B, int L, hipStream_t st);
+bool sf_layer_tok_tail_ok(int L);
+int sf_layer_tok_tail_ex(int mode, const float* xin, const float* ring, int ring_frames, int nslots, int f0, const float* pe, const sf_tfm_layer* layers, int nl,
+                         const void* tail, float eps, float* xpark, void* planes, int B, int L, int Lq, hipStream_t st);
 size_t sf_attn_rows_plane_bytes(int B);
 int sf_attn_rows_ex(int mode, const float* xin, long long x_batch_stride, long long xparts_stride, const float* pe, int f0,
                     int ring_frames, int nslots, const sf_tfm_layer& w, float eps, float* x2, void* planes, int B, int L, int Lq,
diff --git a/slotformer_amd/csrc/layer_tok.hip b/slotformer_amd/csrc/layer_tok.hip
--- a/slotformer_amd/csrc/layer_tok.hip
+++ b/slotformer_amd/csrc/layer_tok.hip
@@ -2,6 +2,7 @@
 #include "sf_internal.h"
 #include "layer_fused.h"
 #include "layer_tok_common.h"
+#include "qkv_heads.h"
 #include <stdlib.h>
 
 namespace {
@@ -15,6 +16,11 @@
 constexpr size_t LT_LDS = (size_t)LT_PAR + (size_t)P_N * 4;
 constexpr size_t LT_BLOB = (size_t)LT_NST * LT_STAGE + (size_t)P_N * 4;
 static_assert(LT_LDS <= 160 * 1024, "LDS budget");
+constexpr int LT_VP_ATT = P_LN2G * 4 / 1024, LT_VP_FFN = (P_N - P_LN2G) * 4 / 1024;
+static_assert(LT_VP_ATT * 1024 == P_LN2G * 4 && LT_VP_FFN * 1024 == (P_N - P_LN2G) * 4 && LT_VP_ATT <= 8 && LT_VP_FFN <= 8, "whole pieces, two per wave");
+constexpr int LT_NST_TAIL = 3 * LT_NH;
+constexpr size_t LT_TAIL_BLOB = (size_t)LT_NST_TAIL * LT_STAGE + (size_t)P_LN2G * 4;
+constexpr int LT_PL = 2048;
 
 struct LtArgs {
   const float* x;
@@ -22,16 +28,24 @@
   const float* pe;
   float* y;
   const char* blob[LT_MAXL];
+  const char* tail;
+  __bf16* planes;
   float eps;
-  int nl, B, L, vpw, RF, N, f0, dbg_ts;
+  int nl, B, L, vpw, RF, N, f0, dbg_ts, Lq;
 };
 }
 
 __device__ long long lt_ts[16];
 #define LTS(i) do { if (A.dbg_ts && blockIdx.x == 0 && threadIdx.x == 0) lt_ts[i] = wall_clock64(); } while (0)
 
+template <int E>
+struct LtExtra {
+  static constexpr int value = E;
+};
+
 template <int MODE>
 __global__ __launch_bounds__(LT_NT) void layer_tok_kernel(LtArgs A) {
+  constexpr bool RING = (MODE & 1) != 0, TAIL = (MODE & 2) != 0;
   extern __shared__ __attribute__((aligned(16))) char smem[];
   float* P = (float*)(smem + LT_PAR);
   const int t = threadIdx.x, lane = t & 63;
@@ -45,41 +59,6 @@
   const int vl = te / L, tok = te - vl * L;
   const long long row = (long long)(v0 + vl) * L + tok;
   LTS(0);
-  f32x16 X[8];
-  if constexpr (MODE == 0) {
-    const float* xr = A.x + row * LT_D + 4 * h;
-#pragma unroll
-    for (int ob = 0; ob < 8; ++ob)
-#pragma unroll
-      for (int g = 0; g < 4; ++g) {
-        const f32x4 v = *(const f32x4*)(xr + 32 * ob + 8 * g);
-#pragma unroll
-        for (int q = 0; q < 4; ++q) X[ob][4 * g + q] = v[q];
-      }
-  } else {
-    const int fr = tok / A.N, sl = tok - fr * A.N;
-    const float* rr = A.ring + (((long long)(v0 + vl) * A.RF + (A.f0 + fr) % A.RF) * A.N + sl) * LT_D + 4 * h;
-    const float* pr = A.pe + (long long)tok * LT_D + 4 * h;
-#pragma unroll
-    for (int ob = 0; ob < 8; ++ob)
-#pragma unroll
-      for (int g = 0; g < 4; ++g) {
-        const f32x4 v = *(const f32x4*)(rr + 32 * ob + 8 * g);
-#pragma unroll
-        for (int q = 0; q < 4; ++q) X[ob][4 * g + q] = v[q];
-      }
-    __builtin_amdgcn_sched_barrier(0);
-#pragma unroll
-    for (int ob = 0; ob < 8; ++ob) {
-#pragma unroll
-      for (int g = 0; g < 4; ++g) {
-        const f32x4 v = *(const f32x4*)(pr + 32 * ob + 8 * g);
-#pragma unroll
-        for (int q = 0; q < 4; ++q) X[ob][4 * g + q] += v[q];
-      }
-      __builtin_amdgcn_sched_barrier(0);
-    }
-  }
   const unsigned wlane = (unsigned)(wave * 8 * 1024 + lane * 16);
   char* const wdst = smem + (wave * 8) * 1024;
   int cur = 0;
@@ -87,15 +66,27 @@
   const char* base_cur = A.blob[0];
   const char* base_nxt = A.blob[0];
   bool last_layer = false;
+  int nst_tail = LT_NST;
   auto stage_src = [&]() -> const char* {
+    const int nst = TAIL ? nst_tail : LT_NST;
     const int t2 = cs + 2;
-    const bool wrap = t2 >= LT_NST;
+    const bool wrap = t2 >= nst;
     const char* b = wrap ? base_nxt : base_cur;
-    const int so = wrap ? (last_layer ? LT_NST - 1 : t2 - LT_NST) : t2;
+    const int so = wrap ? (last_layer ? nst - 1 : t2 - nst) : t2;
     ++cs;
     return b + (size_t)so * LT_STAGE + wlane;
   };
+  auto lt_vec_dma = [&](const char* vsrc, auto off, auto np) {
+    constexpr int OFF = decltype(off)::value, NP = decltype(np)::value;
+#pragma unroll
+    for (int i = 0; i < 2; ++i) {
+      const int pc = min(2 * wave + i, NP - 1);
+      __builtin_amdgcn_global_load_lds((const void __attribute__((address_space(1)))*)(vsrc + OFF + pc * 1024 + lane * 16),
+                                       (void __attribute__((address_space(3)))*)(smem + LT_PAR + OFF + pc * 1024), 16, 0, 0);
+    }
+  };
   {
+    lt_vec_dma(A.blob[0] + (size_t)LT_NST * LT_STAGE, LtExtra<0>{}, LtExtra<LT_VP_ATT>{});
     const char* s0 = stage_src();
     const char* s1 = stage_src();
     LtRing R0{nullptr, s0, wdst}, R1{nullptr, s1, wdst + LT_STAGE};
@@ -103,11 +94,48 @@
     for (int f = 0; f < 8; ++f) lt_dma(R0, f);
 #pragma unroll
     for (int f = 0; f < 8; ++f) lt_dma(R1, f);
+    __builtin_amdgcn_sched_barrier(0);
+  }
+  f32x16 X[8];
+  if constexpr (!RING) {
+    const float* xr = A.x + row * LT_D + 4 * h;
+#pragma unroll
+    for (int ob = 0; ob < 8; ++ob)
+#pragma unroll
+      for (int g = 0; g < 4; ++g) {
+        const f32x4 v = *(const f32x4*)(xr + 32 * ob + 8 * g);
+#pragma unroll
+        for (int q = 0; q < 4; ++q) X[ob][4 * g + q] = v[q];
+      }
+  } else {
+    const int fr = tok / A.N, sl = tok - fr * A.N;
+    const float* rr = A.ring + (((long long)(v0 + vl) * A.RF + (A.f0 + fr) % A.RF) * A.N + sl) * LT_D + 4 * h;
+    const float* pr = A.pe + (long long)tok * LT_D + 4 * h;
+#pragma unroll
+    for (int ob = 0; ob < 8; ++ob)
+#pragma unroll
+      for (int g = 0; g < 4; ++g) {
+        const f32x4 v = *(const f32x4*)(rr + 32 * ob + 8 * g);
+#pragma unroll
+        for (int q = 0; q < 4; ++q) X[ob][4 * g + q] = v[q];
+      }
+    __builtin_amdgcn_sched_barrier(0);
+#pragma unroll
+    for (int ob = 0; ob < 8; ++ob) {
+#pragma unroll
+      for (int g = 0; g < 4; ++g) {
+        const f32x4 v = *(const f32x4*)(pr + 32 * ob + 8 * g);
+#pragma unroll
+        for (int q = 0; q < 4; ++q) X[ob][4 * g + q] += v[q];
+      }
+      __builtin_amdgcn_sched_barrier(0);
+    }
   }
 #ifdef LT_STAMPS
   long long c_wait = 0, c_bar = 0, c_last = 0, c_work = 0;
 #endif
-  auto stage_begin = [&]() -> LtRing {
+  auto stage_begin_x = [&](auto extra) -> LtRing {
+    static_assert(decltype(extra)::value == 0 || decltype(extra)::value == 2, "wait counts that exist");
 #ifdef LT_STAMPS
     const long long c0 = __builtin_readcyclecounter();
     if (c_last) c_work += c0 - c_last;
@@ -115,7 +143,10 @@
 #ifdef LT_NODMA
     asm volatile("s_waitcnt vmcnt(0)" ::: "memory");
 #else
-    asm volatile("s_waitcnt vmcnt(8)" ::: "memory");
+    if constexpr (decltype(extra)::value == 2)
+      asm volatile("s_waitcnt vmcnt(10)" ::: "memory");
+    else
+      asm volatile("s_waitcnt vmcnt(8)" ::: "memory");
 #endif
     asm volatile("s_waitcnt lgkmcnt(0)" ::: "memory");
 #ifdef LT_STAMPS
@@ -139,6 +170,7 @@
     cur = cur == 2 ? 0 : cur + 1;
     return R;
   };
+  auto stage_begin = [&]() -> LtRing { return stage_begin_x(LtExtra<0>{}); };
   const int wf = min(wave * 32, nvalid - 1);
   const int kb0 = ((wf / L) * L) >> 5;
   const int d0 = 32 * kb0 + 4 * h - vl * L;
@@ -169,20 +201,19 @@
   const float qscale = 0.2550348616841918f;
   constexpr float NEG = -3.0e38f;
   LTS(1);
+  asm volatile("s_waitcnt vmcnt(0)" ::: "memory");
+  __syncthreads();
+  LTS(2);
 
 #pragma unroll 1
   for (int l = 0; l < A.nl; ++l) {
+    const bool final_l = l + 1 >= A.nl;
     cs = 0;
     base_cur = A.blob[l];
-    last_layer = l + 1 >= A.nl;
-    base_nxt = A.blob[last_layer ? l : l + 1];
-    __syncthreads();
-    {
-      const float* vsrc = (const float*)(A.blob[l] + (size_t)LT_NST * LT_STAGE);
-      for (int i = t; i < P_N / 4; i += LT_NT) *(f32x4*)(P + 4 * i) = *(const f32x4*)(vsrc + 4 * i);
-    }
-    __syncthreads();
-    if (l == 0) LTS(2);
+    last_layer = final_l && !TAIL;
+    base_nxt = final_l ? (TAIL ? A.tail : A.blob[l]) : A.blob[l + 1];
+    const char* const vec_cur = A.blob[l] + (size_t)LT_NST * LT_STAGE;
+    const char* const vec_nxt = final_l ? (TAIL ? A.tail + (size_t)LT_NST_TAIL * LT_STAGE : vec_cur) : A.blob[l + 1] + (size_t)LT_NST * LT_STAGE;
     bf16x8 xh[16], xl[16];
     lt_layernorm<P_LN1G, P_LN1B>(X, pb, h, A.eps, xh, xl);
     lt_add_vec<P_BO>(X, pb);
@@ -308,10 +339,11 @@
     }
     {
       const LtRing R = stage_begin();
+      lt_vec_dma(vec_cur, LtExtra<P_LN2G * 4>{}, LtExtra<LT_VP_FFN>{});
       lt_row_product<false, 0>(R, xh, xl, ka, LtNoSide{});
     }
     {
-      const LtRing R = stage_begin();
+      const LtRing R = stage_begin_x(LtExtra<2>{});
       lt_row_product<true, 5>(R, xh, xl, va, [&](int g) {
         if (g < 2) kconv(g);
         else if (g < 4) qconv(g - 2);
@@ -393,9 +425,9 @@
         hl[t16] = __builtin_bit_cast(bf16x8, lw[t16]);
       }
     };
-    auto ffn_step = [&](f32x4 (&Hn)[2][2], const f32x4 (&Hp)[2][2], int j) {
-      {
-        const LtRing R = stage_begin();
+    auto ffn_step = [&](f32x4 (&Hn)[2][2], const f32x4 (&Hp)[2][2], int j, auto extra) {
+      {
+        const LtRing R = stage_begin_x(extra);
         lt16_row_product<2, 8>(R, xh, xl, Hn, [&](int ks) { hconv_piece(Hp, ks); });
         hconv_done();
         asm volatile("" : "+v"(hh[0]), "+v"(hh[1]), "+v"(hl[0]), "+v"(hl[1]));
@@ -408,14 +440,15 @@
     };
     {
       const LtRing R = stage_begin();
+      lt_vec_dma(vec_nxt, LtExtra<0>{}, LtExtra<LT_VP_ATT>{});
       b1_load(0);
       lt16_row_product<0, 8>(R, xh, xl, Ha, LtNoSide{});
     }
-    ffn_step(Hb, Ha, 1);
+    ffn_step(Hb, Ha, 1, LtExtra<2>{});
 #pragma unroll 1
     for (int j = 2; j < LT_F / 32; j += 2) {
-      ffn_step(Ha, Hb, j);
-      ffn_step(Hb, Ha, j + 1);
+      ffn_step(Ha, Hb, j, LtExtra<0>{});
+      ffn_step(Hb, Ha, j + 1, LtExtra<0>{});
     }
 #pragma unroll
     for (int k = 0; k < 8; ++k) hconv_piece(Hb, k);
@@ -430,13 +463,101 @@
     if (l == 0 && blockIdx.x == 0 && threadIdx.x == 0) { lt_ts[11] = c_wait; lt_ts[12] = c_bar; lt_ts[13] = c_work; }
 #endif
   }
-  asm volatile("s_waitcnt vmcnt(0)" ::: "memory");
-  if (tl < nvalid) {
-    float* yr = A.y + row * LT_D + 4 * h;
-#pragma unroll
-    for (int ob = 0; ob < 8; ++ob)
-#pragma unroll
-      for (int g = 0; g < 4; ++g) *(f32x4*)(yr + 32 * ob + 8 * g) = quad(X[ob], g);
+  if constexpr (TAIL) {
+    const bool ok = tl < nvalid;
+    const int nq0 = L - A.Lq;
+    const bool qrow = ok && tok >= nq0;
+    cs = 0;
+    base_cur = base_nxt = A.tail;
+    last_layer = true;
+    nst_tail = LT_NST_TAIL;
+#ifdef LT_STAMPS
+    const long long t_wait = c_wait, t_bar = c_bar, t_work = c_work;
+#endif
+    bf16x8 xh[16], xl[16];
+    lt_layernorm<P_LN1G, P_LN1B>(X, pb, h, A.eps, xh, xl);
+    __bf16* const pp = A.planes + (long long)(v0 + vl) * (LT_NH * 6 * LT_PL);
+    const int oqk = tok * 32 + 4 * h, ov = vpos(tok);
+    const float scale = 1.0f / sqrtf(32.f);
+    auto store_qk = [&](const f32x16& a, int hd, auto grp) {
+#pragma clang fp contract(off)
+      constexpr int G = decltype(grp)::value;
+      if (G == 0 ? qrow : ok) {
+        const float* bq = (const float*)pb + P_BQKV + 256 * G + 32 * hd;
+        __bf16* ph = pp + (hd * 6 + 2 * G) * LT_PL + oqk;
+#pragma unroll
+        for (int g = 0; g < 4; ++g) {
+          f32x4 v = quad(a, g) + *(const f32x4*)(bq + 8 * g);
+          if (G == 0) v = v * scale;
+          sf_split4(ph, ph + LT_PL, 8 * g, v);
+        }
+      }
+    };
+    auto store_v = [&](const f32x16& a, int hd) {
+#pragma clang fp contract(off)
+      if (ok) {
+        const float* bv = (const float*)pb + P_BQKV + 512 + 32 * hd;
+        __bf16* pv = pp + (hd * 6 + 4) * LT_PL + ov;
+#pragma unroll
+        for (int g = 0; g < 4; ++g) {
+          const f32x4 b4 = *(const f32x4*)(bv + 8 * g);
+#pragma unroll
+          for (int q = 0; q < 4; ++q) {
+            const float v = a[4 * g + q] + b4[q];
+            const __bf16 hi = (__bf16)v;
+            const int dim = 8 * g + 4 * h + q;
+            pv[dim * 64] = hi;
+            pv[LT_PL + dim * 64] = (__bf16)(v - (float)hi);
+          }
+        }
+      }
+    };
+    f32x16 qa, ka, va;
+#pragma unroll 1
+    for (int hd = 0; hd < LT_NH; ++hd) {
+      {
+        const LtRing R = stage_begin();
+        if (hd > 0) store_v(va, hd - 1);
+        __builtin_amdgcn_sched_barrier(0);
+        lt_row_product<false, 0>(R, xh, xl, qa, LtNoSide{});
+      }
+      {
+        const LtRing R = stage_begin();
+        store_qk(qa, hd, LtExtra<0>{});
+        __builtin_amdgcn_sched_barrier(0);
+        lt_row_product<false, 0>(R, xh, xl, ka, LtNoSide{});
+      }
+      {
+        const LtRing R = stage_begin();
+        store_qk(ka, hd, LtExtra<1>{});
+        __builtin_amdgcn_sched_barrier(0);
+        lt_row_product<false, 0>(R, xh, xl, va, LtNoSide{});
+      }
+    }
+    store_v(va, LT_NH - 1);
+#ifdef LT_STAMPS
+    if (blockIdx.x == 0 && threadIdx.x == 0) {
+      lt_ts[14] = (c_wait - t_wait) + (c_bar - t_bar);
+      lt_ts[15] = (c_work - t_work) + (__builtin_readcyclecounter() - c_last);
+    }
+#endif
+    if (qrow) {
+      float* yr = A.y + ((long long)(v0 + vl) * A.Lq + (tok - nq0)) * LT_D + 4 * h;
+#pragma unroll
+      for (int ob = 0; ob < 8; ++ob)
+#pragma unroll
+        for (int g = 0; g < 4; ++g) *(f32x4*)(yr + 32 * ob + 8 * g) = quad(X[ob], g);
+    }
+    asm volatile("s_waitcnt vmcnt(0)" ::: "memory");
+  } else {
+    asm volatile("s_waitcnt vmcnt(0)" ::: "memory");
+    if (tl < nvalid) {
+      float* yr = A.y + row * LT_D + 4 * h;
+#pragma unroll
+      for (int ob = 0; ob < 8; ++ob)
+#pragma unroll
+        for (int g = 0; g < 4; ++g) *(f32x4*)(yr + 32 * ob + 8 * g) = quad(X[ob], g);
+    }
   }
   LTS(7);
 }
@@ -478,6 +599,50 @@
   return 0;
 }
 
+namespace {
+__global__ void pack_layer_tok_tail_kernel(const float* __restrict__ win, uint4* __restrict__ out) {
+  const int idx = blockIdx.x * blockDim.x + threadIdx.x;
+  if (idx >= LT_NST_TAIL * 32 * 64) return;
+  const int lane = idx & 63, f = (idx >> 6) & 31, st = idx >> 11;
+  const int pl = f & 1, h = lane >> 5, i = lane & 31;
+  const int hd = st / 3, kind = st - 3 * hd;
+  const int vk = f >> 1, c0 = 32 * (vk >> 1), s = vk & 1;
+  const float* src = win + (long long)(kind * LT_D + 32 * hd + i) * LT_D + c0 + 4 * h;
+  union {
+    __bf16 b[8];
+    uint4 u;
+  } o;
+#pragma unroll
+  for (int j = 0; j < 8; ++j) {
+    const float v = src[8 * (2 * s + (j >> 2)) + (j & 3)];
+    const __bf16 hi = (__bf16)v;
+    o.b[j] = pl ? (__bf16)(v - (float)hi) : hi;
+  }
+  out[idx] = o.u;
+}
+}
+
+extern "C" size_t sf_layer_tok_tail_packed_bytes(void) { return LT_TAIL_BLOB; }
+extern "C" int sf_pack_layer_tok_tail(const sf_tfm_layer* w, void* packed, void* stream) {
+  SF_REQUIRE(w && packed, "sf_pack_layer_tok_tail: null pointer");
+  SF_REQUIRE(w->in_proj_w && w->norm1_g && w->norm1_b && w->in_proj_b && w->out_proj_b, "sf_pack_layer_tok_tail: null weight");
+  hipStream_t st = (hipStream_t)stream;
+  constexpr int n = LT_NST_TAIL * 32 * 64;
+  static_assert(n % 256 == 0, "whole blocks");
+  hipLaunchKernelGGL(pack_layer_tok_tail_kernel, dim3(n / 256), dim3(256), 0, st, w->in_proj_w, (uint4*)packed);
+  SF_CHECK_LAUNCH();
+  float* vec = (float*)((char*)packed + (size_t)LT_NST_TAIL * LT_STAGE);
+  const struct {
+    const float* src;
+    int off, n;
+  } parts[4] = {{w->norm1_g, P_LN1G, 256}, {w->norm1_b, P_LN1B, 256}, {w->in_proj_b, P_BQKV, 768}, {w->out_proj_b, P_BO, 256}};
+  for (const auto& p : parts) {
+    const hipError_t e = hipMemcpyAsync(vec + p.off, p.src, (size_t)p.n * 4, hipMemcpyDeviceToDevice, st);
+    if (e != hipSuccess) return sf_set_err((int)e, hipGetErrorString(e), __FILE__, __LINE__);
+  }
+  return 0;
+}
+
 int sf_layer_tok_vpw(int L) {
   if (L < 1 || L > 96) return 0;
   for (int vpw = LT_TOK / L; vpw >= 1; --vpw) {
@@ -494,31 +659,58 @@
 }
 bool sf_layer_tok_ok(int L) { return sf_layer_tok_vpw(L) > 0; }
 
-int sf_layer_tok_ex(int mode, const float* xin, const float* ring, int ring_frames, int nslots, int f0, const float* pe, const sf_tfm_layer* layers, int nl,
-                    float eps, float* y, int B, int L, hipStream_t st) {
+static int launch_layer_tok(int mode, const float* xin, const float* ring, int ring_frames, int nslots, int f0, const float* pe, const sf_tfm_layer* layers,
+                            int nl, float eps, float* y, const void* tail, void* planes, int Lq, int B, int L, hipStream_t st) {
   bool ok = layers && nl >= 1 && nl <= LT_MAXL && sf_layer_tok_ok(L) && B >= 1 && y && (mode == 0 ? xin != nullptr : (ring && pe && nslots >= 1 && ring_frames >= 1));
   for (int l = 0; ok && l < nl; ++l) ok = layers[l].tok_packed != nullptr;
   if (!ok)
     return sf_set_err(-1, "invalid argument: the token-stationary layers need sf_pack_layer_tok_weights fragments, 1..8 layers and 1 <= L <= 96 rows per video", __FILE__, __LINE__);
+  if (tail && !(planes && sf_layer_tok_tail_ok(L) && Lq >= 1 && Lq <= L))
+    return sf_set_err(-1, "invalid argument: the q|k|v tail of the token-stationary layers needs planes, 1 <= Lq <= L and L <= 64 rows per video", __FILE__, __LINE__);
   static const int dbg = sf_dbg("lt");
   LtArgs A;
   A.x = xin; A.ring = ring; A.pe = pe; A.y = y;
   for (int l = 0; l < LT_MAXL; ++l) A.blob[l] = (const char*)layers[l < nl ? l : nl - 1].tok_packed;
+  A.tail = (const char*)tail; A.planes = (__bf16*)planes; A.Lq = Lq;
   A.eps = eps; A.nl = nl; A.B = B; A.L = L; A.vpw = sf_layer_tok_vpw(L); A.RF = ring_frames; A.N = nslots; A.f0 = f0; A.dbg_ts = dbg;
   const int nwg = (B + A.vpw - 1) / A.vpw;
-  const double flops = nl * ((double)B * L * (2.0 * LT_D * (3 * LT_D + LT_D + 2 * LT_F)) + (double)B * LT_NH * 4.0 * L * L * 32);
-  if (mode == 0) {
-    SF_TRY(sf_ensure_dyn_lds((const void*)layer_tok_kernel<0>, LT_LDS));
-    sf_prof_begin(SF_K_LAYER_TOK, st, flops);
-    hipLaunchKernelGGL(layer_tok_kernel<0>, dim3(nwg), dim3(LT_NT), LT_LDS, st, A);
-  } else {
-    SF_TRY(sf_ensure_dyn_lds((const void*)layer_tok_kernel<1>, LT_LDS));
-    sf_prof_begin(SF_K_LAYER_TOK, st, flops);
-    hipLaunchKernelGGL(layer_tok_kernel<1>, dim3(nwg), dim3(LT_NT), LT_LDS, st, A);
-  }
+  const double flops = nl * ((double)B * L * (2.0 * LT_D * (3 * LT_D + LT_D + 2 * LT_F)) + (double)B * LT_NH * 4.0 * L * L * 32) +
+                       (tail ? (double)B * L * 2.0 * LT_D * 3 * LT_D : 0.0);
+  const int m = (mode == 0 ? 0 : 1) | (tail ? 2 : 0);
+#define LT_LAUNCH(M_)                                                                          \
+  do {                                                                                         \
+    SF_TRY(sf_ensure_dyn_lds((const void*)layer_tok_kernel<M_>, LT_LDS));                      \
+    sf_prof_begin(SF_K_LAYER_TOK, st, flops);                                                  \
+    hipLaunchKernelGGL(layer_tok_kernel<M_>, dim3(nwg), dim3(LT_NT), LT_LDS, st, A);           \
+  } while (0)
+  if (m == 0) LT_LAUNCH(0);
+  else if (m == 1) LT_LAUNCH(1);
+  else if (m == 2) LT_LAUNCH(2);
+  else LT_LAUNCH(3);
+#undef LT_LAUNCH
   sf_prof_end(SF_K_LAYER_TOK, st);
   SF_CHECK_LAUNCH();
   return 0;
+}
+
+int sf_layer_tok_ex(int mode, const float* xin, const float* ring, int ring_frames, int nslots, int f0, const float* pe, const sf_tfm_layer* layers, int nl,
+                    float eps, float* y, int B, int L, hipStream_t st) {
+  return launch_layer_tok(mode, xin, ring, ring_frames, nslots, f0, pe, layers, nl, eps, y, nullptr, nullptr, 0, B, L, st);
+}
+
+bool sf_layer_tok_tail_ok(int L) { return sf_layer_tok_ok(L) && L <= 64; }
+
+int sf_layer_tok_tail_ex(int mode, const float* xin, const float* ring, int ring_frames, int nslots, int f0, const float* pe, const sf_tfm_layer* layers, int nl,
+                         const void* tail, float eps, float* xpark, void* planes, int B, int L, int Lq, hipStream_t st) {
+  if (!tail) return sf_set_err(-1, "invalid argument: the q|k|v tail needs the sf_pack_layer_tok_tail copy of the layer behind the launch's last", __FILE__, __LINE__);
+  return launch_layer_tok(mode, xin, ring, ring_frames, nslots, f0, pe, layers, nl, eps, xpark, tail, planes, Lq, B, L, st);
+}
+
+extern "C" int sf_layer_tok_tail_f32(const sf_tfm_layer* w, int nl, const void* tail_packed, const float* x, float* xpark, void* planes, int B, int L, int Lq,
+                                     void* stream) {
+  SF_REQUIRE(w && tail_packed && x && xpark && planes && B > 0 && nl >= 1 && nl <= LT_MAXL, "sf_layer_tok_tail_f32: null pointer / empty problem / more than 8 layers");
+  SF_REQUIRE(sf_get_precision() == 1, "sf_layer_tok_tail_f32: split-bf16 mode only");
+  return sf_layer_tok_tail_ex(0, x, nullptr, 1, 1, 0, nullptr, w, nl, tail_packed, 1e-5f, xpark, planes, B, L, Lq, (hipStream_t)stream);
 }
 
 extern "C" int sf_layer_tok_block_f32(const sf_tfm_layer* w, int nl, const float* x, float* y, int B, int L, void* stream) {
diff --git a/slotformer_amd/csrc/sf_switches.cpp b/slotformer_amd/csrc/sf_switches.cpp
--- a/slotformer_amd/csrc/sf_switches.cpp
+++ b/slotformer_amd/csrc/sf_switches.cpp
@@ -23,6 +23,7 @@
      {nullptr, 1, NO_ENV},
      {nullptr, 1, NO_ENV},
      {"SF_CONV_WS", 1, FLAG},
+     {nullptr, 0, NO_ENV},
 };
 
 std::atomic<int> g_slot[SF_SW_NUM];
@@ -74,4 +75,6 @@
 int sf_set_slot_attn_planes(int on) { return sf_switch_set(SF_SW_SLOT_ATTN_PLANES, on != 0); }
 int sf_get_pixel_tok(void) { return sf_switch(SF_SW_PIXEL_TOK); }
 int sf_set_pixel_tok(int on) { return sf_switch_set(SF_SW_PIXEL_TOK, on != 0); }
+int sf_layer_tok_tail_get(void) { return sf_switch(SF_SW_LAYER_TOK_TAIL); }
+int sf_layer_tok_tail_set(int on) { return sf_switch_set(SF_SW_LAYER_TOK_TAIL, on != 0); }
 }
diff --git a/slotformer_amd/csrc/sf_switches.h b/slotformer_amd/csrc/sf_switches.h
--- a/slotformer_amd/csrc/sf_switches.h
+++ b/slotformer_amd/csrc/sf_switches.h
@@ -12,6 +12,7 @@
   SF_SW_SLOT_ATTN_PLANES,
   SF_SW_PIXEL_TOK,
   SF_SW_CONV_WS,
+  SF_SW_LAYER_TOK_TAIL,
   SF_SW_NUM
 };
 
diff --git a/slotformer_amd/engine.py b/slotformer_amd/engine.py
--- a/slotformer_amd/engine.py
+++ b/slotformer_amd/engine.py
@@ -106,6 +106,11 @@
         pe = pe + r.enc_slots_pe.detach()[0].repeat(W, 1)
     s.pe_tok = plan.dp(pe.contiguous())
     s.layers = C.cast(_tfm_layers(plan, enc, pack_ffn=packed), C.POINTER(sf_tfm_layer))
+    if s.num_layers >= 2 and s.layers[s.num_layers - 1].tok_packed and (s.d_model, s.num_heads, s.ffn_dim) == (256, 8, 1024):
+        tt = torch.empty(lib().sf_layer_tok_tail_packed_bytes(), dtype=torch.uint8, device=r.in_proj.weight.device)
+        check(lib().sf_pack_layer_tok_tail(C.byref(s.layers[s.num_layers - 1]), tt.data_ptr(), torch.cuda.current_stream().cuda_stream))
+        plan.keep.append(tt)
+        s.tok_tail_packed = tt.data_ptr()
     if packed and s.d_model == 256 and s.slot_size == 128 and r.in_proj.weight.is_cuda:
         s.in_proj_packed, s.out_proj_packed = plan.packed(r.in_proj.weight), plan.packed(r.out_proj.weight)
     plan.struct = s
diff --git a/slotformer_amd/switches.py b/slotformer_amd/switches.py
--- a/slotformer_amd/switches.py
+++ b/slotformer_amd/switches.py
@@ -32,6 +32,11 @@
 }
 
 
+FORMS = {
+    'layer_tok_tail': ('sf_layer_tok_tail_set', 'sf_layer_tok_tail_get', 0, "OPT-IN: LN1 + q|k|v of a rollout's row-pruned last layer as the tail of the token-stationary launch in front of it (0: the q|k|v launch of the row-tile form; profiles/layer_tok_tail.md)"),
+}
+
+
 def check_environment(environ=None):
     environ = os.environ if environ is None else environ
     seen = {k: v for k, v in environ.items() if k.startswith('SF_')}
```

After: 713,700, median of 2. About the same (-0.1%).
